# Gorilla-Lab-SCUT/DCL-Net

Measured on AMD Instinct MI355X. Metric: frames/sec DCL_Net.forward @ YCB-V bs32, higher is better.
Workload: dtype f32 (exact 3xbf16-split products on the bf16 MFMA, f32 accumulate)

## Files before the change

### dcl-net_amd/csrc/dense.hip

```cpp
#include "common.h"
#include <atomic>
#include <math.h>

namespace {

typedef float f32x16 __attribute__((ext_vector_type(16)));

constexpr int kKPitch = 68;
constexpr float kThr = 20.0f;

__device__ __forceinline__ int rowmap(int e, int h) { return (e & 3) + 8 * (e >> 2) + 4 * h; }

#ifdef DCL_DIAG
template <int NVT>
__global__ __launch_bounds__(256, 1) void k_cross_attn(
    int nq, int nk, const float *__restrict__ Q, int ldq, const float *__restrict__ K, int ldk,
    const float *__restrict__ V1, int dv1, int ldv1, float *__restrict__ O1, int ldo1,
    const float *__restrict__ V2, int dv2, int ldv2, float *__restrict__ O2, int ldo2) {
  constexpr int T = 256;
  constexpr int DV = NVT * 32;
  constexpr int KT = 32 * kKPitch;
  constexpr int TILE = KT + 32 * DV;
  constexpr int NVS = (32 * (DV / 4) + T - 1) / T;
  extern __shared__ float attn_lds[];
// ... 326 lines not shown
  auto load_k = [&](int kb) {
    int key, c4;
    k_slot(0, key, c4);
    knext0 = *reinterpret_cast<const float4 *>(K + (krow0 + min(kb + key, last_key)) * ldk + c4);
    if (KPT > 1) {
      k_slot(1, key, c4);
      knext1 = *reinterpret_cast<const float4 *>(K + (krow0 + min(kb + key, last_key)) * ldk + c4);
    }
  };
  auto store_k = [&]() {
    int key, c4;
    k_slot(0, key, c4);
    *reinterpret_cast<float4 *>(Ks + key * kKPitch + c4) = knext0;
    if (KPT > 1) {
      k_slot(1, key, c4);
      *reinterpret_cast<float4 *>(Ks + key * kKPitch + c4) = knext1;
    }
  };

  f32x16 O[NVT];
#pragma unroll
  for (int t = 0; t < NVT; ++t)
#pragma unroll
    for (int e = 0; e < 16; ++e) O[t][e] = 0.0f;
  float m_ref = -INFINITY, l_part = 0.0f;

  const int ntiles = (nk + 31) >> 5;
  const int kb_begin = (int)((long long)blockIdx.z * ntiles / gridDim.z) * 32;
  const int kb_end = min((int)((long long)(blockIdx.z + 1) * ntiles / gridDim.z) * 32, nk);
  load_k(kb_begin);
  store_k();
  dma_v(kb_begin, 0);
  int cur = 0;
  for (int kb = kb_begin; kb < kb_end; kb += 32) {
    const bool more = kb + 32 < kb_end;
    __builtin_amdgcn_s_waitcnt(0x0F70);
    __syncthreads();
    if (more) dma_v(kb + 32, cur ^ 1);

    f32x16 S;
#pragma unroll
    for (int e = 0; e < 16; ++e) S[e] = 0.0f;
    {
      const float *krow = Ks + r * kKPitch + 32 * h;
      const float *qrow = Qs + r * kKPitch + 32 * h;
#pragma unroll
      for (int i = 0; i < 8; ++i) {
        const float4 a = *reinterpret_cast<const float4 *>(krow + 4 * i);
        const float4 qv = *reinterpret_cast<const float4 *>(qrow + 4 * i);
        S = __builtin_amdgcn_mfma_f32_32x32x2f32(a.x, qv.x, S, 0, 0, 0);
        S = __builtin_amdgcn_mfma_f32_32x32x2f32(a.y, qv.y, S, 0, 0, 0);
        S = __builtin_amdgcn_mfma_f32_32x32x2f32(a.z, qv.z, S, 0, 0, 0);
        S = __builtin_amdgcn_mfma_f32_32x32x2f32(a.w, qv.w, S, 0, 0, 0);
      }
    }
    __builtin_amdgcn_s_waitcnt(0xC07F);
    __builtin_amdgcn_s_barrier();
    if (more) load_k(kb + 32);

    float m_tile = -INFINITY;
#pragma unroll
    for (int e = 0; e < 16; ++e) {
      if (kb + rowmap(e, h) >= nk) S[e] = -INFINITY;
      m_tile = fmaxf(m_tile, S[e]);
    }
    m_tile = fmaxf(m_tile, __shfl_xor(m_tile, 32, 64));
    if (__ballot(m_tile > m_ref + kThr) != 0ull) {
      const float m_new = fmaxf(m_ref, m_tile);
      const float f = __expf(m_ref - m_new);
      l_part *= f;
#pragma unroll
      for (int t = 0; t < NVT; ++t)
#pragma unroll
        for (int e = 0; e < 16; ++e) O[t][e] *= f;
      m_ref = m_new;
    }
#pragma unroll
    for (int e = 0; e < 16; ++e) {
      S[e] = __expf(S[e] - m_ref);
      l_part += S[e];
    }

    const float *v1b = V1s + cur * V1T + 4 * h * 256 + r;
    const float *v2b = V2s + cur * V2T + 4 * h * 64 + r;
#pragma unroll
    for (int t = 0; t < NVT; ++t) {
#pragma unroll
      for (int e = 0; e < 16; ++e) {
        const int krow = (e & 3) + 8 * (e >> 2);
        const float a = t < 8 ? v1b[krow * 256 + t * 32] : v2b[krow * 64 + (t - 8) * 32];
        O[t] = __builtin_amdgcn_mfma_f32_32x32x2f32(a, S[e], O[t], 0, 0, 0);
      }
    }
    if (more) store_k();
    cur ^= 1;
  }

  asm volatile("s_nop 15\n\ts_nop 7" ::: "memory");
  const float l_tot = l_part + __shfl_xor(l_part, 32, 64);
  if (qlive && gridDim.z > 1) {
    const size_t rows = (size_t)gridDim.y * nq;
    float *P = part + ((size_t)blockIdx.z * rows + (size_t)b * nq + q) * kAttnPartPitch;
#pragma unroll
    for (int t = 0; t < NVT; ++t)
#pragma unroll
      for (int g = 0; g < 4; ++g)
        *reinterpret_cast<float4 *>(P + t * 32 + 8 * g + 4 * h) =
            make_float4(O[t][4 * g], O[t][4 * g + 1], O[t][4 * g + 2], O[t][4 * g + 3]);
    if (h == 0) { P[320] = m_ref; P[321] = l_tot; }
  } else if (qlive) {
    const size_t row = (size_t)b * nq + q;
#pragma unroll
    for (int t = 0; t < NVT; ++t)
#pragma unroll
      for (int g = 0; g < 4; ++g) {
        const int c = t * 32 + 8 * g + 4 * h;
        float4 v;
        v.x = O[t][4 * g] / l_tot; v.y = O[t][4 * g + 1] / l_tot;
        v.z = O[t][4 * g + 2] / l_tot; v.w = O[t][4 * g + 3] / l_tot;
        if (c < 256) *reinterpret_cast<float4 *>(O1 + row * ldo1 + c) = v;
        else *reinterpret_cast<float4 *>(O2 + row * ldo2 + (c - 256)) = v;
      }
  }
}

typedef __bf16 at_bf16x2 __attribute__((ext_vector_type(2)));
typedef __bf16 at_bf16x8 __attribute__((ext_vector_type(8)));
typedef float at_f32x2 __attribute__((ext_vector_type(2)));
typedef unsigned at_u32x4 __attribute__((ext_vector_type(4)));
constexpr int kAttnHalfBytes = 3 * 320 * 2 * 16;
constexpr int kAttnKTileBytes = 3 * 32 * 128;
constexpr int kAttnTileBytes = 2 * kAttnHalfBytes + kAttnKTileBytes;

__device__ __forceinline__ unsigned at_cvt2(float a, float b) {
  const at_f32x2 v = {a, b};
  return __builtin_bit_cast(unsigned, __builtin_convertvector(v, at_bf16x2));
}
__device__ __forceinline__ void at_split2(float x0, float x1, unsigned &h, unsigned &m, unsigned &l) {
  h = at_cvt2(x0, x1);
  float r0 = x0 - __uint_as_float(h << 16);
  asm volatile("" : "+v"(r0));
  float r1 = x1 - __uint_as_float(h & 0xffff0000u);
  asm volatile("" : "+v"(r1));
  m = at_cvt2(r0, r1);
  float s0 = r0 - __uint_as_float(m << 16);
  asm volatile("" : "+v"(s0));
  float s1 = r1 - __uint_as_float(m & 0xffff0000u);
  asm volatile("" : "+v"(s1));
  l = at_cvt2(s0, s1);
}
__device__ __forceinline__ at_bf16x8 at_bf(at_u32x4 v) { return __builtin_bit_cast(at_bf16x8, v); }

__global__ __launch_bounds__(256) void k_attn_split_v(int nk, int nht, const float *__restrict__ V1, int ldv1, const float *__restrict__ V2,
                                                      int ldv2, unsigned *__restrict__ planes, long long total, int c_begin) {
  const int nc = 320 - c_begin;
  for (long long i = blockIdx.x * 256ll + threadIdx.x; i < total; i += (long long)gridDim.x * 256) {
    const int hs = (int)(i & 1);
    const long long q = i >> 1;
    const int c = c_begin + (int)(q % nc);
    const long long cht = q / nc;
    const int ht = (int)(cht % nht), crop = (int)(cht / nht);
    const int h = hs ^ ((c >> 3) & 1);
    const float *col = c < 256 ? V1 + c : V2 + (c - 256);
    const int ld = c < 256 ? ldv1 : ldv2;
    float v[8];
#pragma unroll
    for (int e = 0; e < 8; ++e) {
      const int key = 16 * ht + (e & 3) + 8 * (e >> 2) + 4 * h;
      v[e] = key < nk ? col[((size_t)crop * nk + key) * ld] : 0.0f;
    }
    unsigned ph[4], pm[4], pl[4];
#pragma unroll
    for (int e = 0; e < 4; ++e) at_split2(v[2 * e], v[2 * e + 1], ph[e], pm[e], pl[e]);
    unsigned *dst = planes + (size_t)cht * (kAttnHalfBytes / 4) + (size_t)(c * 2 + hs) * 4;
#pragma unroll
    for (int e = 0; e < 4; ++e) { dst[e] = ph[e]; dst[320 * 2 * 4 + e] = pm[e]; dst[2 * 320 * 2 * 4 + e] = pl[e]; }
  }
}

__global__ __launch_bounds__(256) void k_attn_split_k(int nk, int ntiles, const float *__restrict__ K, int ldk, unsigned *__restrict__ kplanes,
                                                      long long total) {
  for (long long i = blockIdx.x * 256ll + threadIdx.x; i < total; i += (long long)gridDim.x * 256) {
    const int ps = (int)(i & 7), key = (int)((i >> 3) & 31);
    const long long ct = i >> 8;
    const int tile = (int)(ct % ntiles), crop = (int)(ct / ntiles);
    const int p = ps ^ ((key >> 1) & 7), kk = tile * 32 + key;
    float4 a = make_float4(0.f, 0.f, 0.f, 0.f), b = a;
    if (kk < nk) {
      const float *row = K + ((size_t)crop * nk + kk) * ldk + 8 * p;
      a = *reinterpret_cast<const float4 *>(row);
      b = *reinterpret_cast<const float4 *>(row + 4);
    }
    unsigned ph[4], pm[4], pl[4];
    at_split2(a.x, a.y, ph[0], pm[0], pl[0]);
    at_split2(a.z, a.w, ph[1], pm[1], pl[1]);
    at_split2(b.x, b.y, ph[2], pm[2], pl[2]);
    at_split2(b.z, b.w, ph[3], pm[3], pl[3]);
    unsigned *dst = kplanes + (size_t)ct * (kAttnKTileBytes / 4) + (size_t)(key * 8 + ps) * 4;
#pragma unroll
    for (int e = 0; e < 4; ++e) { dst[e] = ph[e]; dst[32 * 32 + e] = pm[e]; dst[2 * 32 * 32 + e] = pl[e]; }
  }
}

__global__ __launch_bounds__(512, 2) void k_cross_attn_split(
    int nq, int nk, const float *__restrict__ Q, int ldq, const unsigned char *__restrict__ planes,
    const unsigned char *__restrict__ kplanes, float *__restrict__ O1, int ldo1, float *__restrict__ O2, int ldo2,
    float *__restrict__ part, int xcd_remap, int whatif) {
  constexpr int NVT = 10, WAVES = 8;
  constexpr int VT = 2 * kAttnHalfBytes;
  extern __shared__ float attn_lds[];
  unsigned char *Kp = reinterpret_cast<unsigned char *>(attn_lds);
  unsigned char *Vp = Kp + 2 * kAttnKTileBytes;
  int bx, b;
  {
    const int nwg = gridDim.x * gridDim.y, id = blockIdx.x + gridDim.x * blockIdx.y;
    const int xq = nwg >> 3, xr = nwg & 7, xcd = id & 7;
    const int swz = !xcd_remap ? id : (xcd < xr ? xcd * (xq + 1) : xr * (xq + 1) + (xcd - xr) * xq) + (id >> 3);
    bx = swz % (int)gridDim.x;
    b = swz / (int)gridDim.x;
  }
  const int tid = threadIdx.x;
  const int lane = tid & 63, wave = __builtin_amdgcn_readfirstlane(tid >> 6);
  const int grp = wave >> 2;
  const int r = lane & 31, h = lane >> 5;
  constexpr int QB = WAVES * 32;
  const int q = bx * QB + wave * 32 + r;
  const bool qlive = q < nq;
  const float *qrow = Q + ((size_t)b * nq + min(q, nq - 1)) * ldq + 8 * h;
  const int nht = 2 * ((nk + 31) >> 5);
  const unsigned char *vsrc = planes + (size_t)b * nht * kAttnHalfBytes;
  const unsigned char *ksrc = kplanes + (size_t)b * (nht >> 1) * kAttnKTileBytes;
  const unsigned lane16 = (unsigned)lane * 16u;
  const unsigned vp0 = lds_addr_of(reinterpret_cast<const float *>(Vp));
  const unsigned kp0 = lds_addr_of(reinterpret_cast<const float *>(Kp));
  auto dma_tile = [&](int tile, int buf) {
    const unsigned char *ks = ksrc + (size_t)tile * kAttnKTileBytes + wave * 1024;
    const unsigned kd = kp0 + (unsigned)(buf * kAttnKTileBytes + wave * 1024);
    glds16_s(lane16, ks, kd);
    if (wave < 4) glds16_s(lane16, ks + 8 * 1024, kd + 8 * 1024);
    const unsigned char *vs = vsrc + (size_t)tile * VT + wave * 1024;
    const unsigned vd = vp0 + (unsigned)(buf * VT + wave * 1024);
#pragma unroll
    for (int i = 0; i < 8; ++i)
      if (wave + 8 * i < 60) glds16_s(lane16, vs + i * 8192, vd + (unsigned)(i * 8192));
  };

  f32x16 O[NVT];
#pragma unroll
  for (int t = 0; t < NVT; ++t)
#pragma unroll
    for (int e = 0; e < 16; ++e) O[t][e] = 0.0f;
  float m_ref = -INFINITY, l_part = 0.0f;
  at_u32x4 pp[2][3];
#pragma unroll
  for (int hf = 0; hf < 2; ++hf)
#pragma unroll
    for (int p = 0; p < 3; ++p) pp[hf][p] = at_u32x4{0u, 0u, 0u, 0u};

  const int ntiles_all = (nk + 31) >> 5;
  const int t_begin = (int)((long long)blockIdx.z * ntiles_all / gridDim.z);
  const int t_end = (int)((long long)(blockIdx.z + 1) * ntiles_all / gridDim.z);
  const int T = t_end - t_begin;
  const unsigned char *vfrag = Vp + ((r * 2 + (h ^ ((r >> 3) & 1))) << 4);
  const unsigned char *kfrag = Kp + r * 128;
  const int ksw = (r >> 1) & 7;

  auto s_phase = [&](int tl) __attribute__((always_inline)) {
    const int buf = tl & 1, kb = (t_begin + tl) * 32;
    f32x16 S;
#pragma unroll
    for (int e = 0; e < 16; ++e) S[e] = 0.0f;
    const unsigned char *kfb = kfrag + buf * kAttnKTileBytes;
    float4 qn0 = *reinterpret_cast<const float4 *>(qrow), qn1 = *reinterpret_cast<const float4 *>(qrow + 4);
#pragma unroll
    for (int st = 0; st < 4; ++st) {
      const float4 qc0 = qn0, qc1 = qn1;
      if (st < 3) {
        qn0 = *reinterpret_cast<const float4 *>(qrow + 16 * (st + 1));
        qn1 = *reinterpret_cast<const float4 *>(qrow + 16 * (st + 1) + 4);
      }
      const unsigned char *kf = kfb + (((2 * st + h) ^ ksw) << 4);
      const at_u32x4 kh = *reinterpret_cast<const at_u32x4 *>(kf);
      const at_u32x4 km = *reinterpret_cast<const at_u32x4 *>(kf + 32 * 128);
      const at_u32x4 kl = *reinterpret_cast<const at_u32x4 *>(kf + 2 * 32 * 128);
      at_u32x4 qh, qm, ql;
      unsigned a0, a1, a2;
      at_split2(qc0.x, qc0.y, a0, a1, a2); qh[0] = a0; qm[0] = a1; ql[0] = a2;
      at_split2(qc0.z, qc0.w, a0, a1, a2); qh[1] = a0; qm[1] = a1; ql[1] = a2;
      at_split2(qc1.x, qc1.y, a0, a1, a2); qh[2] = a0; qm[2] = a1; ql[2] = a2;
      at_split2(qc1.z, qc1.w, a0, a1, a2); qh[3] = a0; qm[3] = a1; ql[3] = a2;
      S = __builtin_amdgcn_mfma_f32_32x32x16_bf16(at_bf(kl), at_bf(qh), S, 0, 0, 0);
      S = __builtin_amdgcn_mfma_f32_32x32x16_bf16(at_bf(kh), at_bf(ql), S, 0, 0, 0);
      S = __builtin_amdgcn_mfma_f32_32x32x16_bf16(at_bf(km), at_bf(qm), S, 0, 0, 0);
      S = __builtin_amdgcn_mfma_f32_32x32x16_bf16(at_bf(km), at_bf(qh), S, 0, 0, 0);
      S = __builtin_amdgcn_mfma_f32_32x32x16_bf16(at_bf(kh), at_bf(qm), S, 0, 0, 0);
      S = __builtin_amdgcn_mfma_f32_32x32x16_bf16(at_bf(kh), at_bf(qh), S, 0, 0, 0);
    }
    float m_tile = -INFINITY;
    if (kb + 32 > nk) {
#pragma unroll
      for (int e = 0; e < 16; ++e)
        if (kb + rowmap(e, h) >= nk) S[e] = -INFINITY;
    }
#pragma unroll
    for (int e = 0; e < 16; ++e) m_tile = fmaxf(m_tile, S[e]);
    m_tile = fmaxf(m_tile, __shfl_xor(m_tile, 32, 64));
    if (__ballot(m_tile > m_ref + kThr) != 0ull) {
      const float m_new = fmaxf(m_ref, m_tile);
      const float f = __expf(m_ref - m_new);
      l_part *= f;
#pragma unroll
      for (int t = 0; t < NVT; ++t)
#pragma unroll
        for (int e = 0; e < 16; ++e) O[t][e] *= f;
      m_ref = m_new;
    }
#pragma unroll
    for (int e = 0; e < 16; ++e) {
      S[e] = __expf(S[e] - m_ref);
      l_part += S[e];
    }
#pragma unroll
    for (int hf = 0; hf < 2; ++hf)
#pragma unroll
      for (int e = 0; e < 4; ++e) {
        unsigned ph, pm, pl;
        at_split2(S[8 * hf + 2 * e], S[8 * hf + 2 * e + 1], ph, pm, pl);
        pp[hf][0][e] = ph; pp[hf][1][e] = pm; pp[hf][2][e] = pl;
      }
  };
  auto pv_phase = [&](int tl) __attribute__((always_inline)) {
    const unsigned char *vbuf = vfrag + (tl & 1) * VT;
#pragma unroll
    for (int hf = 0; hf < 2; ++hf) {
      const unsigned char *vb = vbuf + hf * kAttnHalfBytes;
#pragma unroll
      for (int t = 0; t < NVT; ++t) {
        const at_u32x4 vh = *reinterpret_cast<const at_u32x4 *>(vb + t * 1024);
        const at_u32x4 vm = *reinterpret_cast<const at_u32x4 *>(vb + 320 * 32 + t * 1024);
        const at_u32x4 vl = *reinterpret_cast<const at_u32x4 *>(vb + 2 * 320 * 32 + t * 1024);
        O[t] = __builtin_amdgcn_mfma_f32_32x32x16_bf16(at_bf(vl), at_bf(pp[hf][0]), O[t], 0, 0, 0);
        O[t] = __builtin_amdgcn_mfma_f32_32x32x16_bf16(at_bf(vh), at_bf(pp[hf][2]), O[t], 0, 0, 0);
        O[t] = __builtin_amdgcn_mfma_f32_32x32x16_bf16(at_bf(vm), at_bf(pp[hf][1]), O[t], 0, 0, 0);
        O[t] = __builtin_amdgcn_mfma_f32_32x32x16_bf16(at_bf(vm), at_bf(pp[hf][0]), O[t], 0, 0, 0);
        O[t] = __builtin_amdgcn_mfma_f32_32x32x16_bf16(at_bf(vh), at_bf(pp[hf][1]), O[t], 0, 0, 0);
        O[t] = __builtin_amdgcn_mfma_f32_32x32x16_bf16(at_bf(vh), at_bf(pp[hf][0]), O[t], 0, 0, 0);
      }
    }
  };
  auto interval = [&](int iv) __attribute__((always_inline)) {
    __builtin_amdgcn_s_waitcnt(0x0F70);
    __syncthreads();
    if ((iv & 1) && (iv + 1) / 2 < T && !(whatif & 4)) dma_tile(t_begin + (iv + 1) / 2, ((iv + 1) / 2) & 1);
  };
  if (T > 0) dma_tile(t_begin, 0);
  if (grp == 0) {
    for (int tl = 0; tl < T; ++tl) {
      interval(2 * tl);
      if (!(whatif & 2)) s_phase(tl);
      interval(2 * tl + 1);
      if (!(whatif & 1)) pv_phase(tl);
    }
    interval(2 * T);
  } else {
    interval(0);
    for (int tl = 0; tl < T; ++tl) {
      interval(2 * tl + 1);
      if (!(whatif & 2)) s_phase(tl);
      interval(2 * tl + 2);
      if (!(whatif & 1)) pv_phase(tl);
    }
  }

  asm volatile("s_nop 15\n\ts_nop 7" ::: "memory");
  const float l_tot = l_part + __shfl_xor(l_part, 32, 64);
  if (qlive && gridDim.z > 1) {
    const size_t rows = (size_t)gridDim.y * nq;
    float *P = part + ((size_t)blockIdx.z * rows + (size_t)b * nq + q) * kAttnPartPitch;
#pragma unroll
    for (int t = 0; t < NVT; ++t)
#pragma unroll
      for (int g = 0; g < 4; ++g)
        *reinterpret_cast<float4 *>(P + t * 32 + 8 * g + 4 * h) =
            make_float4(O[t][4 * g], O[t][4 * g + 1], O[t][4 * g + 2], O[t][4 * g + 3]);
    if (h == 0) { P[320] = m_ref; P[321] = l_tot; }
  } else if (qlive) {
    const size_t row = (size_t)b * nq + q;
#pragma unroll
    for (int t = 0; t < NVT; ++t)
#pragma unroll
      for (int g = 0; g < 4; ++g) {
        const int c = t * 32 + 8 * g + 4 * h;
        float4 v;
        v.x = O[t][4 * g] / l_tot; v.y = O[t][4 * g + 1] / l_tot;
        v.z = O[t][4 * g + 2] / l_tot; v.w = O[t][4 * g + 3] / l_tot;
        if (c < 256) *reinterpret_cast<float4 *>(O1 + row * ldo1 + c) = v;
        else *reinterpret_cast<float4 *>(O2 + row * ldo2 + (c - 256)) = v;
      }
  }
}

__global__ void k_cross_attn_combine(int rows, int nsplit, const float *__restrict__ part, float *__restrict__ O1, int ldo1,
                                     float *__restrict__ O2, int ldo2) {
  const long long total = (long long)rows * 80;
  for (long long t = (long long)blockIdx.x * blockDim.x + threadIdx.x; t < total; t += (long long)gridDim.x * blockDim.x) {
    const size_t row = (size_t)(t / 80);
    const int c = (int)(t - (long long)row * 80) * 4;
    float m = -INFINITY;
    for (int z = 0; z < nsplit; ++z) m = fmaxf(m, part[((size_t)z * rows + row) * kAttnPartPitch + 320]);
    float4 num = make_float4(0.f, 0.f, 0.f, 0.f);
    float den = 0.0f;
    for (int z = 0; z < nsplit; ++z) {
      const float *P = part + ((size_t)z * rows + row) * kAttnPartPitch;
      const float f = __expf(P[320] - m);
      const float4 o = *reinterpret_cast<const float4 *>(P + c);
      num.x += f * o.x; num.y += f * o.y; num.z += f * o.z; num.w += f * o.w;
      den += f * P[321];
    }
    const float4 v = make_float4(num.x / den, num.y / den, num.z / den, num.w / den);
    if (c < 256) *reinterpret_cast<float4 *>(O1 + row * ldo1 + c) = v;
    else *reinterpret_cast<float4 *>(O2 + row * ldo2 + (c - 256)) = v;
  }
}

template <int NT>
__device__ __forceinline__ float conf_block_reduce(float v, float *red, int lane, int wave, bool is_max) {
  constexpr int NW = NT / 64;
#pragma unroll
  for (int d = 32; d >= 1; d >>= 1) v = is_max ? fmaxf(v, __shfl_xor(v, d, 64)) : v + __shfl_xor(v, d, 64);
  if (lane == 0) red[wave] = v;
  __syncthreads();
  float r;
  if (NW == 4) {
    r = is_max ? fmaxf(fmaxf(red[0], red[1]), fmaxf(red[2], red[3])) : (red[0] + red[1]) + (red[2] + red[3]);
  } else {
    float t[NW];
#pragma unroll
    for (int i = 0; i < NW; ++i) t[i] = red[i];
#pragma unroll
    for (int step = 1; step < NW; step <<= 1)
#pragma unroll
      for (int i = 0; i + step < NW; i += 2 * step) t[i] = is_max ? fmaxf(t[i], t[i + step]) : t[i] + t[i + step];
    r = t[0];
  }
  __syncthreads();
  return r;
}
template <int NT>
__global__ __launch_bounds__(NT) void k_conf_softmax(int n1, int n2, const float *__restrict__ logit1,
                                                     const float *__restrict__ logit2, float *__restrict__ conf,
                                                     float *__restrict__ w, float *__restrict__ wsum) {
  __shared__ float red[NT / 64];
  const int L = n1 + n2;
  const int b = blockIdx.x, tid = threadIdx.x;
  const int lane = tid & 63, wave = tid >> 6;
  float mx = -INFINITY;
  for (int j = tid; j < L; j += NT) {
    const float x = j < n1 ? logit1[(size_t)b * n1 + j] : logit2[(size_t)b * n2 + (j - n1)];
    const float s = 1.0f / (1.0f + expf(-x));
    conf[(size_t)b * L + j] = s;
    mx = fmaxf(mx, s);
  }
  mx = conf_block_reduce<NT>(mx, red, lane, wave, true);
  float sum = 0.0f;
  for (int j = tid; j < L; j += NT) {
    const float e = expf(conf[(size_t)b * L + j] - mx);
    w[(size_t)b * L + j] = e;
    sum += e;
  }
  sum = conf_block_reduce<NT>(sum, red, lane, wave, false);
  const float inv = 1.0f / sum;
  float w1 = 0.f, w2 = 0.f;
  for (int j = tid; j < L; j += NT) {
    const float v = w[(size_t)b * L + j] * inv;
    w[(size_t)b * L + j] = v;
    if (j < n1) w1 += v; else w2 += v;
  }
  w1 = conf_block_reduce<NT>(w1, red, lane, wave, false);
  w2 = conf_block_reduce<NT>(w2, red, lane, wave, false);
  if (tid == 0) { wsum[b * 2] = w1; wsum[b * 2 + 1] = w2; }
}

__global__ __launch_bounds__(256) void k_weighted_colsum(int c, int n1, int n2, int nslices, const float *__restrict__ w,
                                                         const float *__restrict__ F1, int ld1, float *__restrict__ part1,
                                                         const float *__restrict__ F2, int ld2, float *__restrict__ part2) {
  __shared__ float4 red[4][64];
  const int second = (int)blockIdx.y >= nslices ? 1 : 0;
  const int b = blockIdx.z, slice = blockIdx.y - second * nslices;
  const int n = second ? n2 : n1, ld = second ? ld2 : ld1, w_stride = n1 + n2, w_off = second ? n1 : 0;
  const float *__restrict__ F = second ? F2 : F1;
  float *__restrict__ part = second ? part2 : part1;
  const int lane = threadIdx.x & 63, wave = threadIdx.x >> 6;
  const int ch = blockIdx.x * 256 + lane * 4;
  const int per = (n + nslices - 1) / nslices;
  const int j0 = slice * per, j1 = min(n, j0 + per);
  float4 acc = make_float4(0.f, 0.f, 0.f, 0.f);
  if (ch < c) {
    const float *wp = w + (size_t)b * w_stride + w_off;
    const float *fp = F + (size_t)b * n * ld + ch;
    for (int j = j0 + wave; j < j1; j += 4) {
      const float wj = wp[j];
      const float4 f = *reinterpret_cast<const float4 *>(fp + (size_t)j * ld);
      acc.x = __fmaf_rn(f.x, wj, acc.x); acc.y = __fmaf_rn(f.y, wj, acc.y);
      acc.z = __fmaf_rn(f.z, wj, acc.z); acc.w = __fmaf_rn(f.w, wj, acc.w);
    }
  }
  red[wave][lane] = acc;
  __syncthreads();
  if (wave == 0 && ch < c) {
    float4 o;
    o.x = (red[0][lane].x + red[1][lane].x) + (red[2][lane].x + red[3][lane].x);
    o.y = (red[0][lane].y + red[1][lane].y) + (red[2][lane].y + red[3][lane].y);
    o.z = (red[0][lane].z + red[1][lane].z) + (red[2][lane].z + red[3][lane].z);
    o.w = (red[0][lane].w + red[1][lane].w) + (red[2][lane].w + red[3][lane].w);
    *reinterpret_cast<float4 *>(part + ((size_t)b * nslices + slice) * c + ch) = o;
  }
}

template <int EPT>
__global__ __launch_bounds__(256) void k_conf_pool_small(int c, int n1, int n2, int nslices, const float *__restrict__ logit1,
                                                         const float *__restrict__ logit2, float *__restrict__ conf,
                                                         float *__restrict__ wsum, const float *__restrict__ F1, int ld1,
                                                         float *__restrict__ part1, const float *__restrict__ F2, int ld2,
                                                         float *__restrict__ part2) {
  __shared__ float wl[256 * EPT];
  __shared__ float redf[4], r1[4], r2[4];
  __shared__ float4 red[4][64];
  const int L = n1 + n2;
  const int second = (int)blockIdx.y >= nslices ? 1 : 0;
  const int b = blockIdx.z, slice = blockIdx.y - second * nslices;
  const int tid = threadIdx.x, lane = tid & 63, wave = tid >> 6;
  const bool writer = blockIdx.x == 0 && blockIdx.y == 0;
  float sv[EPT];
  float mx = -INFINITY;
#pragma unroll
  for (int k = 0; k < EPT; ++k) {
    const int j = tid + 256 * k;
    if (j < L) {
      const float x = j < n1 ? logit1[(size_t)b * n1 + j] : logit2[(size_t)b * n2 + (j - n1)];
      sv[k] = 1.0f / (1.0f + expf(-x));
      if (writer) conf[(size_t)b * L + j] = sv[k];
      mx = fmaxf(mx, sv[k]);
    }
  }
#pragma unroll
  for (int d = 32; d >= 1; d >>= 1) mx = fmaxf(mx, __shfl_xor(mx, d, 64));
  if (lane == 0) redf[wave] = mx;
  __syncthreads();
  mx = fmaxf(fmaxf(redf[0], redf[1]), fmaxf(redf[2], redf[3]));
  __syncthreads();
  float sum = 0.0f;
#pragma unroll
// ... 61 lines not shown
    const float x = o9[i * 9 + c * 3], y = o9[i * 9 + c * 3 + 1], z = o9[i * 9 + c * 3 + 2];
    const float mag = sqrtf((x * x + y * y) + z * z) + 1e-8f;
    A[0][c] = (double)(x / mag); A[1][c] = (double)(y / mag); A[2][c] = (double)(z / mag);
#pragma unroll
    for (int r = 0; r < 3; ++r) V[r][c] = r == c ? 1.0 : 0.0;
  }
  for (int sweep = 0; sweep < 30; ++sweep) {
    double off = 0.0;
#pragma unroll
    for (int p = 0; p < 2; ++p)
#pragma unroll
      for (int q = p + 1; q < 3; ++q) {
        double alpha = 0, beta = 0, gamma = 0;
#pragma unroll
        for (int r = 0; r < 3; ++r) { alpha += A[r][p] * A[r][p]; beta += A[r][q] * A[r][q]; gamma += A[r][p] * A[r][q]; }
        off = fmax(off, fabs(gamma) / sqrt(alpha * beta + 1e-300));
        if (fabs(gamma) < 1e-300) continue;
        const double zeta = (beta - alpha) / (2.0 * gamma);
        const double t = (zeta >= 0 ? 1.0 : -1.0) / (fabs(zeta) + sqrt(1.0 + zeta * zeta));
        const double cs = 1.0 / sqrt(1.0 + t * t), sn = cs * t;
#pragma unroll
        for (int r = 0; r < 3; ++r) {
          const double ap = A[r][p], aq = A[r][q];
          A[r][p] = cs * ap - sn * aq; A[r][q] = sn * ap + cs * aq;
          const double vp = V[r][p], vq = V[r][q];
          V[r][p] = cs * vp - sn * vq; V[r][q] = sn * vp + cs * vq;
        }
      }
    if (off < 1e-15) break;
  }
  double a0[3] = {A[0][0], A[1][0], A[2][0]}, a1[3] = {A[0][1], A[1][1], A[2][1]}, a2[3] = {A[0][2], A[1][2], A[2][2]};
  double v0[3] = {V[0][0], V[1][0], V[2][0]}, v1[3] = {V[0][1], V[1][1], V[2][1]}, v2[3] = {V[0][2], V[1][2], V[2][2]};
  double s0 = sqrt(a0[0] * a0[0] + a0[1] * a0[1] + a0[2] * a0[2]);
  double s1 = sqrt(a1[0] * a1[0] + a1[1] * a1[1] + a1[2] * a1[2]);
  double s2 = sqrt(a2[0] * a2[0] + a2[1] * a2[1] + a2[2] * a2[2]);
#define DCL_SWAP_COLS(sa, sb, aa, ab, va, vb)                                  \
  if (sa < sb) {                                                               \
    double t_ = sa; sa = sb; sb = t_;                                          \
    for (int r_ = 0; r_ < 3; ++r_) {                                           \
      t_ = aa[r_]; aa[r_] = ab[r_]; ab[r_] = t_;                               \
      t_ = va[r_]; va[r_] = vb[r_]; vb[r_] = t_;                               \
    }                                                                          \
  }
  DCL_SWAP_COLS(s0, s1, a0, a1, v0, v1)
  DCL_SWAP_COLS(s1, s2, a1, a2, v1, v2)
  DCL_SWAP_COLS(s0, s1, a0, a1, v0, v1)
#undef DCL_SWAP_COLS
  double u1[3], u2[3], u3[3];
#pragma unroll
  for (int r = 0; r < 3; ++r) { u1[r] = a0[r] / s0; u2[r] = a1[r] / s1; }
  u3[0] = u1[1] * u2[2] - u1[2] * u2[1];
  u3[1] = u1[2] * u2[0] - u1[0] * u2[2];
  u3[2] = u1[0] * u2[1] - u1[1] * u2[0];
  const double detV = v0[0] * (v1[1] * v2[2] - v1[2] * v2[1]) - v0[1] * (v1[0] * v2[2] - v1[2] * v2[0]) +
                      v0[2] * (v1[0] * v2[1] - v1[1] * v2[0]);
#pragma unroll
  for (int r = 0; r < 3; ++r)
#pragma unroll
    for (int c = 0; c < 3; ++c)
      R[i * 9 + r * 3 + c] = (float)(u1[r] * v0[c] + u2[r] * v1[c] + detV * u3[r] * v2[c]);
}
__global__ void k_ortho9d(int b, const float *__restrict__ o9, float *__restrict__ R) {
  const int i = blockIdx.x * blockDim.x + threadIdx.x;
  if (i < b) ortho9d_one(o9, R, i);
}

}

DCL_HOOK_INT(g_attn_variant, 0);
DCL_HOOK_INT(g_attn_split, 0);
DCL_HOOK_INT(g_attn_xcd_remap, 1);
#ifdef DCL_DIAG
DCL_API void dcl_debug_attention_split(int n) { g_attn_split = n; }
DCL_API void dcl_debug_attention_xcd_remap(int on) { g_attn_xcd_remap = on; }
DCL_API void dcl_debug_attention_variant(int v) { g_attn_variant = v; }
#endif

DCL_API int dcl_cross_attention(int b, int nq, int nk, const float *Q, int ldq, const float *K, int ldk,
                                const float *V1, int dv1, int ldv1, float *O1, int ldo1, const float *V2, int dv2,
                                int ldv2, float *O2, int ldo2, dclStream_t stream) {
  return dcl_cross_attention_ws(b, nq, nk, Q, ldq, K, ldk, V1, dv1, ldv1, O1, ldo1, V2, dv2, ldv2, O2, ldo2, nullptr, 0,
                                stream);
}

DCL_HOOK_INT(g_attn_whatif, 0);
DCL_HOOK_INT(g_attn_bf16, 1);
static bool attn_split_big(long long blocks8, int nk) { return blocks8 >= 64 && blocks8 * dcl_div_up(nk, 32) >= 16384; }
DCL_HOOK_INT(g_attn_pair_split, 1);
static int attn_pair_full_crops(int b, int nq, int dv1, int dv2, int concurrent_launches, int nk = 0) {
  if (!g_attn_pair_split || g_attn_variant != 0 || concurrent_launches != 2 || dv1 != 256 || dv2 != 64 || nq <= 0) return 0;
  const int qb8 = dcl_div_up(nq, 256);
  if (nk > 0 && g_attn_bf16 && attn_split_big((long long)b * qb8, nk)) return 0;
  if (qb8 > 128 || 128 % qb8 != 0) return 0;
  const int per_round = 128 / qb8;
  const int full = b / per_round * per_round;
  return full > 0 && full < b ? full : 0;
}
#ifdef DCL_DIAG
DCL_API void dcl_debug_attention_pair_split(int on) { g_attn_pair_split = on; }
#endif

static int attn_small_split(int b, int nq, int ntiles) {
  const int forced = g_attn_split;
  if (forced > 0) return forced > 16 ? 16 : forced;
  const long long T = 2ll * b * dcl_div_up(nq, 128);
  const double tiles_us = 1.1 * ntiles;
  double best = 1e30;
  int nsplit = 1;
  for (int z = 1; z <= 16; z *= 2) {
    const double cost = (double)dcl_div_up(T * z, 256) * (tiles_us / z + 4.0) + (z > 1 ? 4.0 + 0.15 * z * (double)b * nq / 1024.0 : 0.0);
    if (cost < best - 1e-9) { best = cost; nsplit = z; }
  }
  if (nsplit > ntiles / 2) nsplit = ntiles / 2;
  return nsplit < 1 ? 1 : nsplit;
}

DCL_API int dcl_cross_attention_scratch_floats(int b, int nq, int64_t *floats_host) {
  DCL_CHECK_ARG(b >= 0 && nq >= 0 && floats_host);
  const long long per = (long long)b * nq * kAttnPartPitch;
  const long long blocks8 = (long long)b * dcl_div_up(nq > 0 ? nq : 1, 256);
  long long z = 1;
  if (blocks8 < 256) {
    for (int ntiles = 2; ntiles <= (1 << 16); ntiles *= 2) z = max(z, (long long)attn_small_split(b, nq, ntiles));
  } else {
    z = 1;
    double best = (double)dcl_div_up(blocks8, 256);
    for (int c = 2; c <= 8; c *= 2) {
      const double cost = (double)dcl_div_up(blocks8 * c, 256) / c;
      if (cost <= best - 0.2 && c * per <= (128ll << 20)) { best = cost; z = c; }
    }
  }
  long long need = z > 1 ? z * per : 0;
  const int full = attn_pair_full_crops(b, nq, 256, 64, 2);
  if (full) {
    int64_t rest = 0;
    const int rc = dcl_cross_attention_scratch_floats(b - full, nq, &rest);
    if (rc) return rc;
    if (rest > need) need = rest;
  }
  *floats_host = need;
  return 0;
}

DCL_API int dcl_cross_attention_ws(int b, int nq, int nk, const float *Q, int ldq, const float *K, int ldk,
                                   const float *V1, int dv1, int ldv1, float *O1, int ldo1, const float *V2, int dv2,
                                   int ldv2, float *O2, int ldo2, float *scratch, int64_t scratch_floats,
                                   dclStream_t stream) {
  return dcl_cross_attention_ws2(b, nq, nk, Q, ldq, K, ldk, V1, dv1, ldv1, O1, ldo1, V2, dv2, ldv2, O2, ldo2, scratch,
                                 scratch_floats, 1, stream);
}

static int attn_dispatch(int b, int nq, int nk, const float *Q, int ldq, const float *K, int ldk, const float *V1, int dv1, int ldv1,
                         float *O1, int ldo1, const float *V2, int dv2, int ldv2, float *O2, int ldo2, float *scratch,
                         int64_t scratch_floats, int concurrent_launches, void *planes, int64_t planes_bytes, dclStream_t stream);

static bool attn_takes_w8(int b, int nq, int nk, int concurrent_launches) {
  const long long blocks8 = (long long)b * dcl_div_up(nq, 256);
  const bool pair8 = concurrent_launches == 2 && 2 * blocks8 > 240 && 2 * blocks8 <= 256;
  return g_attn_variant == 3 || (g_attn_variant == 0 && (blocks8 >= 256 || pair8 || attn_split_big(blocks8, nk)));
}
#ifdef DCL_DIAG
DCL_API void dcl_debug_attention_bf16(int on) { g_attn_bf16 = on; }
DCL_API void dcl_debug_attention_whatif(int bits) { g_attn_whatif = bits; }
#endif

DCL_API int dcl_cross_attention_split_crops(int b, int nq, int nk, int concurrent_launches) {
  if (b <= 0 || nq <= 0 || nk <= 0 || !g_attn_bf16) return 0;
  int crops = b;
  const int full = attn_pair_full_crops(b, nq, 256, 64, concurrent_launches, nk);
  if (full) crops = full;
  return attn_takes_w8(crops, nq, nk, concurrent_launches) ? crops : 0;
}

DCL_API int64_t dcl_cross_attention_planes_bytes(int b, int nq, int nk, int concurrent_launches) {
  if (b <= 0 || nq <= 0 || nk <= 0 || !g_attn_bf16) return 0;
  int crops = b;
  const int full = attn_pair_full_crops(b, nq, 256, 64, concurrent_launches, nk);
  if (full) crops = full;
  if (!attn_takes_w8(crops, nq, nk, concurrent_launches)) return 0;
  return (int64_t)crops * dcl_div_up(nk, 32) * kAttnTileBytes;
}

DCL_API int dcl_cross_attention_ws2(int b, int nq, int nk, const float *Q, int ldq, const float *K, int ldk,
                                    const float *V1, int dv1, int ldv1, float *O1, int ldo1, const float *V2, int dv2,
                                    int ldv2, float *O2, int ldo2, float *scratch, int64_t scratch_floats,
                                    int concurrent_launches, dclStream_t stream) {
  return dcl_cross_attention_ws3(b, nq, nk, Q, ldq, K, ldk, V1, dv1, ldv1, O1, ldo1, V2, dv2, ldv2, O2, ldo2, scratch, scratch_floats,
                                 concurrent_launches, nullptr, 0, stream);
}

DCL_API int dcl_cross_attention_ws3(int b, int nq, int nk, const float *Q, int ldq, const float *K, int ldk,
                                    const float *V1, int dv1, int ldv1, float *O1, int ldo1, const float *V2, int dv2,
                                    int ldv2, float *O2, int ldo2, float *scratch, int64_t scratch_floats,
                                    int concurrent_launches, void *planes, int64_t planes_bytes, dclStream_t stream) {
  DCL_CHECK_ARG(concurrent_launches == 1 || concurrent_launches == 2);
  const int full = (b > 0 && Q && K && O1) ? attn_pair_full_crops(b, nq, dv1, dv2, concurrent_launches, planes ? nk : 0) : 0;
  DCL_CHECK_ARG(!(full && !V1));
  if (full) {
    int rc = attn_dispatch(full, nq, nk, Q, ldq, K, ldk, V1, dv1, ldv1, O1, ldo1, V2, dv2, ldv2, O2, ldo2, scratch, scratch_floats,
                           concurrent_launches, planes, planes_bytes, stream);
    if (rc) return rc;
    const size_t qo = (size_t)full * nq, ko = (size_t)full * nk;
    return attn_dispatch(b - full, nq, nk, Q + qo * ldq, ldq, K + ko * ldk, ldk, V1 + ko * ldv1, dv1, ldv1, O1 + qo * ldo1, ldo1,
                         V2 ? V2 + ko * ldv2 : nullptr, dv2, ldv2, O2 ? O2 + qo * ldo2 : nullptr, ldo2, scratch, scratch_floats,
                         concurrent_launches, nullptr, 0, stream);
  }
  return attn_dispatch(b, nq, nk, Q, ldq, K, ldk, V1, dv1, ldv1, O1, ldo1, V2, dv2, ldv2, O2, ldo2, scratch, scratch_floats,
                       concurrent_launches, planes, planes_bytes, stream);
}

static int attn_dispatch(int b, int nq, int nk, const float *Q, int ldq, const float *K, int ldk, const float *V1, int dv1, int ldv1,
                         float *O1, int ldo1, const float *V2, int dv2, int ldv2, float *O2, int ldo2, float *scratch,
                         int64_t scratch_floats, int concurrent_launches, void *planes, int64_t planes_bytes, dclStream_t stream) {
  DCL_CHECK_ARG(b >= 0 && nq >= 0 && nk > 0 && dv1 > 0 && dv1 % 32 == 0 && dv2 >= 0 && dv2 % 32 == 0);
  if (b == 0 || nq == 0) return 0;
  DCL_CHECK_ARG(Q && K && (V1 || planes) && O1 && (dv2 == 0 || (V2 && O2)) && b <= 65535);
  DCL_CHECK_ARG(ldq >= 64 && ldk >= 64 && ldv1 >= dv1 && ldo1 >= dv1 && (dv2 == 0 || (ldv2 >= dv2 && ldo2 >= dv2)));
  DCL_CHECK_ARG(ldq % 4 == 0 && ldk % 4 == 0 && ldv1 % 4 == 0 && ldo1 % 4 == 0 && ldv2 % 4 == 0 && ldo2 % 4 == 0);
  DCL_CHECK_ARG((((uintptr_t)Q | (uintptr_t)K | (uintptr_t)V1 | (uintptr_t)O1 | (uintptr_t)V2 | (uintptr_t)O2) & 15) == 0);
  const bool v1_in_planes = V1 == nullptr;
  const int nvt = (dv1 + dv2) / 32;
  DCL_CHECK_ARG(nvt == 1 || nvt == 2 || nvt == 4 || nvt == 8 || nvt == 10);
  hipStream_t s = (hipStream_t)stream;
  const long long blocks8 = (long long)b * dcl_div_up(nq, 256);
  if (dv1 == 256 && dv2 == 64 && (g_attn_variant == 0 || g_attn_variant == 3 || g_attn_variant == 4)) {
    const bool pair8 = concurrent_launches == 2 && 2 * blocks8 > 240 && 2 * blocks8 <= 256;
    const bool split_usable = planes && g_attn_bf16 && (((uintptr_t)planes) & 15) == 0 &&
                              planes_bytes >= (int64_t)b * dcl_div_up(nk, 32) * kAttnTileBytes;
    const bool w8 = g_attn_variant == 3 ||
                    (g_attn_variant == 0 && (blocks8 >= 256 || pair8 || (split_usable && attn_split_big(blocks8, nk))));
    const int W = w8 ? 8 : 4;
    const size_t lds = (size_t)(32 * kKPitch + 2 * 32 * 256 + 2 * 32 * 64 + W * 32 * kKPitch) * sizeof(float);
    if (w8) {
      int nsplit = 1;
      if (scratch && !(pair8 && g_attn_split == 0)) {
        if (g_attn_split > 0) {
          nsplit = g_attn_split;
        } else {
          double best = (double)dcl_div_up(blocks8, 256);
          for (int z = 2; z <= 8; z *= 2) {
            const double cost = (double)dcl_div_up(blocks8 * z, 256) / z;
            if (cost <= best - 0.2 && (long long)z * b * nq * kAttnPartPitch <= (128ll << 20)) { best = cost; nsplit = z; }
          }
        }
        const int ntiles = dcl_div_up(nk, 32);
        if (nsplit > 8) nsplit = 8;
        if (nsplit > ntiles / 2) nsplit = ntiles / 2;
        while (nsplit > 1 && (long long)nsplit * b * nq * kAttnPartPitch > scratch_floats) --nsplit;
        if (nsplit < 1) nsplit = 1;
      }
      const int nht = 2 * dcl_div_up(nk, 32);
      const int64_t planes_need = (int64_t)b * (nht / 2) * kAttnTileBytes;
      if (planes && planes_bytes >= planes_need && g_attn_bf16 && (((uintptr_t)planes) & 15) == 0) {
        const int c_begin = V1 ? 0 : 256;
        const long long total = (long long)b * nht * (320 - c_begin) * 2;
        hipLaunchKernelGGL(k_attn_split_v, dim3(dcl_grid_1d(total, 256)), dim3(256), 0, s, nk, nht, V1, ldv1, V2, ldv2,
                           (unsigned *)planes, total, c_begin);
        unsigned char *kplanes = (unsigned char *)planes + (size_t)b * nht * kAttnHalfBytes;
        const long long ktotal = (long long)b * (nht / 2) * 32 * 8;
        hipLaunchKernelGGL(k_attn_split_k, dim3(dcl_grid_1d(ktotal, 256)), dim3(256), 0, s, nk, nht / 2, K, ldk, (unsigned *)kplanes, ktotal);
        const size_t lds_sp = (size_t)2 * (2 * kAttnHalfBytes + kAttnKTileBytes);
        (void)hipFuncSetAttribute((const void *)k_cross_attn_split, hipFuncAttributeMaxDynamicSharedMemorySize, (int)lds_sp);
        hipLaunchKernelGGL(k_cross_attn_split, dim3(dcl_div_up(nq, 256), b, nsplit), dim3(512), lds_sp, s, nq, nk, Q, ldq,
                           (const unsigned char *)planes, (const unsigned char *)kplanes, O1, ldo1, O2, ldo2, scratch,
                           (int)g_attn_xcd_remap, (int)g_attn_whatif);
      } else {
        if (v1_in_planes) {
          dcl_set_error("dcl_cross_attention: V1 = NULL (pieces in `planes`) but this call does not take the split-bf16 kernel");
          return DCL_EINVAL;
        }
        (void)hipFuncSetAttribute((const void *)k_cross_attn_dma<8>, hipFuncAttributeMaxDynamicSharedMemorySize, (int)lds);
        hipLaunchKernelGGL(k_cross_attn_dma<8>, dim3(dcl_div_up(nq, 256), b, nsplit), dim3(512), lds, s, nq, nk, Q, ldq, K, ldk,
                           V1, ldv1, O1, ldo1, V2, ldv2, O2, ldo2, scratch, (int)g_attn_xcd_remap);
      }
      if (nsplit > 1)
        hipLaunchKernelGGL(k_cross_attn_combine, dim3(dcl_grid_1d((long long)b * nq * 80, 256)), dim3(256), 0, s, b * nq,
                           nsplit, scratch, O1, ldo1, O2, ldo2);
    } else {
      if (v1_in_planes) {
        dcl_set_error("dcl_cross_attention: V1 = NULL (pieces in `planes`) but this call does not take the split-bf16 kernel");
        return DCL_EINVAL;
      }
      int nsplit = 1;
      if (scratch) {
        nsplit = attn_small_split(b, nq, dcl_div_up(nk, 32));
        const int ntiles = dcl_div_up(nk, 32);
        if (nsplit > 16) nsplit = 16;
        if (nsplit > ntiles / 2) nsplit = ntiles / 2;
        while (nsplit > 1 && (long long)nsplit * b * nq * kAttnPartPitch > scratch_floats) --nsplit;
        if (nsplit < 1) nsplit = 1;
      }
      (void)hipFuncSetAttribute((const void *)k_cross_attn_dma<4>, hipFuncAttributeMaxDynamicSharedMemorySize, (int)lds);
      hipLaunchKernelGGL(k_cross_attn_dma<4>, dim3(dcl_div_up(nq, 128), b, nsplit), dim3(256), lds, s, nq, nk, Q, ldq, K,
                         ldk, V1, ldv1, O1, ldo1, V2, ldv2, O2, ldo2, scratch, (int)g_attn_xcd_remap);
      if (nsplit > 1)
        hipLaunchKernelGGL(k_cross_attn_combine, dim3(dcl_grid_1d((long long)b * nq * 80, 256)), dim3(256), 0, s, b * nq,
                           nsplit, scratch, O1, ldo1, O2, ldo2);
    }
  }
#ifdef DCL_DIAG
  else if ((blocks8 >= 256 && g_attn_variant != 2) || g_attn_variant == 1) {
    const size_t lds = (size_t)(32 * kKPitch + 32 * nvt * 32 + 8 * 32 * kKPitch) * sizeof(float);
#define ATT8(N)                                                                                                \
  do {                                                                                                         \
    (void)hipFuncSetAttribute((const void *)k_cross_attn_shared<8, N>, hipFuncAttributeMaxDynamicSharedMemorySize, \
                              (int)lds);                                                                       \
    hipLaunchKernelGGL((k_cross_attn_shared<8, N>), dim3(dcl_div_up(nq, 256), b), dim3(512), lds, s, nq, nk, Q, \
                       ldq, K, ldk, V1, dv1, ldv1, O1, ldo1, V2, dv2, ldv2, O2, ldo2);                         \
  } while (0)
    switch (nvt) {
      case 1: ATT8(1); break;
      case 2: ATT8(2); break;
      case 4: ATT8(4); break;
      case 8: ATT8(8); break;
      default: ATT8(10); break;
    }
#undef ATT8
  } else {
    const size_t lds = (size_t)2 * (32 * kKPitch + 32 * nvt * 32) * sizeof(float);
#define ATT(N)                                                                                                 \
  do {                                                                                                         \
    (void)hipFuncSetAttribute((const void *)k_cross_attn<N>, hipFuncAttributeMaxDynamicSharedMemorySize,       \
                              (int)lds);                                                                       \
    hipLaunchKernelGGL((k_cross_attn<N>), dim3(dcl_div_up(nq, 128), b), dim3(256), lds, s, nq, nk, Q, ldq, K,   \
                       ldk, V1, dv1, ldv1, O1, ldo1, V2, dv2, ldv2, O2, ldo2);                                 \
  } while (0)
    switch (nvt) {
      case 1: ATT(1); break;
      case 2: ATT(2); break;
      case 4: ATT(4); break;
      case 8: ATT(8); break;
      default: ATT(10); break;
    }
#undef ATT
  }
#else
  else {
    dcl_set_error("dcl_cross_attention: only dv1 = 256, dv2 = 64 is built into the product library (got %d, %d)", dv1, dv2);
    return DCL_EINVAL;
  }
#endif
  DCL_LAUNCH_CHECK();
  return 0;
}

DCL_API int dcl_conf_pool(int b, int c, int n1, int n2, const float *logit1, const float *logit2, const float *F1,
                          int ld1, const float *F2, int ld2, float *conf, float *w_scratch, int nslices,
                          float *part1, float *part2, float *wsum, dclStream_t stream) {
  DCL_CHECK_ARG(b >= 0 && c > 0 && c % 4 == 0 && n1 > 0 && n2 > 0 && ld1 >= c && ld2 >= c && ld1 % 4 == 0 &&
                ld2 % 4 == 0 && nslices >= 1);
  if (b == 0) return 0;
  DCL_CHECK_ARG(conf && w_scratch && part1 && part2 && wsum && logit1 && F1 && logit2 && F2 && b <= 65535 &&
                nslices <= 32767);
  hipStream_t s = (hipStream_t)stream;
  if (b <= 8 && n1 + n2 <= 256 * 8) {
    hipLaunchKernelGGL(k_conf_pool_small<8>, dim3(dcl_div_up(c, 256), 2 * nslices, b), dim3(256), 0, s, c, n1, n2, nslices, logit1,
                       logit2, conf, wsum, F1, ld1, part1, F2, ld2, part2);
    DCL_LAUNCH_CHECK();
    return 0;
  }
  hipLaunchKernelGGL(k_conf_softmax<256>, dim3(b), dim3(256), 0, s, n1, n2, logit1, logit2, conf, w_scratch, wsum);
  hipLaunchKernelGGL(k_weighted_colsum, dim3(dcl_div_up(c, 256), 2 * nslices, b), dim3(256), 0, s, c, n1, n2, nslices,
                     w_scratch, F1, ld1, part1, F2, ld2, part2);
  DCL_LAUNCH_CHECK();
  return 0;
}

__global__ void k_pool_finish(int c, int nslices1, int nslices2, const float *__restrict__ part1, const float *__restrict__ part2,
                              const float *__restrict__ wsum, const float *__restrict__ sA, const float *__restrict__ tA,
                              const float *__restrict__ sB, const float *__restrict__ tB, float *__restrict__ out) {
  const int b = blockIdx.y, ch = blockIdx.x * blockDim.x + threadIdx.x;
  if (ch >= c) return;
  float a1[4] = {0.f, 0.f, 0.f, 0.f}, a2[4] = {0.f, 0.f, 0.f, 0.f};
  const float *q1 = part1 + (size_t)b * nslices1 * c + ch, *q2 = part2 + (size_t)b * nslices2 * c + ch;
  int s = 0;
  for (; s + 4 <= nslices1; s += 4) {
#pragma unroll
    for (int j = 0; j < 4; ++j) a1[j] += q1[(size_t)(s + j) * c];
  }
  for (int j = 0; s < nslices1; ++s, ++j) a1[j] += q1[(size_t)s * c];
  for (s = 0; s + 4 <= nslices2; s += 4) {
#pragma unroll
    for (int j = 0; j < 4; ++j) a2[j] += q2[(size_t)(s + j) * c];
  }
  for (int j = 0; s < nslices2; ++s, ++j) a2[j] += q2[(size_t)s * c];
  const float p1 = (a1[0] + a1[1]) + (a1[2] + a1[3]), p2 = (a2[0] + a2[1]) + (a2[2] + a2[3]);
  const float w0 = wsum[2 * b], w1 = wsum[2 * b + 1];
  out[(size_t)b * c + ch] = ((sA[ch] * p1 + tA[ch] * w0) + sB[ch] * p2) + tB[ch] * w1;
}

DCL_API int dcl_pool_finish2(int b, int c, int nslices1, int nslices2, const float *part1, const float *part2, const float *wsum,
                             const float *scale1, const float *shift1, const float *scale2, const float *shift2,
                             float *out, dclStream_t stream) {
  DCL_CHECK_ARG(b >= 0 && c > 0 && nslices1 >= 1 && nslices2 >= 1);
  if (b == 0) return 0;
  DCL_CHECK_ARG(part1 && part2 && wsum && scale1 && shift1 && scale2 && shift2 && out && b <= 65535);
  hipLaunchKernelGGL(k_pool_finish, dim3(dcl_div_up(c, 256), b), dim3(256), 0, (hipStream_t)stream, c, nslices1, nslices2, part1,
                     part2, wsum, scale1, shift1, scale2, shift2, out);
  DCL_LAUNCH_CHECK();
  return 0;
}
DCL_API int dcl_pool_finish(int b, int c, int nslices, const float *part1, const float *part2, const float *wsum,
                            const float *scale1, const float *shift1, const float *scale2, const float *shift2,
                            float *out, dclStream_t stream) {
  return dcl_pool_finish2(b, c, nslices, nslices, part1, part2, wsum, scale1, shift1, scale2, shift2, out, stream);
}

DCL_API int dcl_conf_softmax(int b, int n1, int n2, const float *logit1, const float *logit2, float *conf, float *w, float *wsum,
                             dclStream_t stream) {
  DCL_CHECK_ARG(b >= 0 && n1 > 0 && n2 > 0);
  if (b == 0) return 0;
  DCL_CHECK_ARG(logit1 && logit2 && conf && w && wsum && b <= 65535);
  if (n1 + n2 > 4096) hipLaunchKernelGGL(k_conf_softmax<1024>, dim3(b), dim3(1024), 0, (hipStream_t)stream, n1, n2, logit1, logit2, conf, w, wsum);
  else hipLaunchKernelGGL(k_conf_softmax<256>, dim3(b), dim3(256), 0, (hipStream_t)stream, n1, n2, logit1, logit2, conf, w, wsum);
  DCL_LAUNCH_CHECK();
  return 0;
}

__global__ __launch_bounds__(256) void k_affine3_relu(long long rows, int c4, const float *__restrict__ xyz, const float *__restrict__ W,
                                                      const float4 *__restrict__ term, float4 *__restrict__ out) {
  const long long total = rows * c4;
  for (long long t = (long long)blockIdx.x * blockDim.x + threadIdx.x; t < total; t += (long long)gridDim.x * blockDim.x) {
    const long long row = t / c4;
    const int q = (int)(t - row * c4);
    const float x = xyz[row * 3], y = xyz[row * 3 + 1], z = xyz[row * 3 + 2];
    const float4 wx = reinterpret_cast<const float4 *>(W)[q], wy = reinterpret_cast<const float4 *>(W)[c4 + q],
                 wz = reinterpret_cast<const float4 *>(W)[2 * c4 + q];
    const float4 a = term[t];
    float4 o;
    o.x = fmaxf(__fmaf_rn(z, wz.x, __fmaf_rn(y, wy.x, x * wx.x)) + a.x, 0.f);
    o.y = fmaxf(__fmaf_rn(z, wz.y, __fmaf_rn(y, wy.y, x * wx.y)) + a.y, 0.f);
    o.z = fmaxf(__fmaf_rn(z, wz.z, __fmaf_rn(y, wy.z, x * wx.z)) + a.z, 0.f);
// ... 281 lines not shown
```

### dcl-net_amd/csrc/linear_split.hip

```cpp
#include <hip/hip_runtime.h>
#include "common.h"

namespace {

typedef float sp_f32x16 __attribute__((ext_vector_type(16)));
typedef float sp_f32x2 __attribute__((ext_vector_type(2)));
typedef __bf16 sp_bf16x2 __attribute__((ext_vector_type(2)));
typedef __bf16 sp_bf16x8 __attribute__((ext_vector_type(8)));
typedef unsigned sp_u32x4 __attribute__((ext_vector_type(4)));
typedef __attribute__((address_space(3))) void sp_lds_void_t;

constexpr int kSpKC = 16;
constexpr int kSpBM = 256, kSpBN = 128;
constexpr int kSpA = kSpBM * kSpKC * 4;
constexpr int kSpP = kSpBN * kSpKC * 2;
constexpr int kSpB = 3 * kSpP;
constexpr int kSpST = kSpA + kSpB;

__device__ __forceinline__ unsigned sp_lds_addr(const void *p) {
  return __builtin_amdgcn_readfirstlane((unsigned)(size_t)(sp_lds_void_t *)p);
}
__device__ __forceinline__ void sp_glds16(unsigned voff, const void *sbase, unsigned lds_byte_addr) {
  unsigned keep;
  asm volatile("s_mov_b32 %0, m0\n\ts_mov_b32 m0, %3\n\ts_nop 0\n\tglobal_load_lds_dwordx4 %1, %2\n\ts_mov_b32 m0, %0"
// ... 153 lines not shown
      __builtin_amdgcn_sched_barrier(0);
      if (!(whatif & 2)) {
#pragma unroll
        for (int part = 0; part < 4; ++part) split_a(0, part);
      } else {
#pragma unroll
        for (int p = 0; p < 3; ++p) ap[0][p] = sp_u32x4{__float_as_uint(av[0][0].x), __float_as_uint(av[0][0].y), __float_as_uint(av[0][1].x), __float_as_uint(av[0][1].y)};
      }
      read_b(1);
      __builtin_amdgcn_sched_barrier(0);
#pragma unroll
      for (int blk = 0; blk < 8; ++blk) {
        const int i = blk >> 2, j = blk & 3;
        acc[i][j] = __builtin_amdgcn_mfma_f32_32x32x16_bf16(sp_bf(ap[i][2]), sp_bf(bp[j][0]), acc[i][j], 0, 0, 0);
        acc[i][j] = __builtin_amdgcn_mfma_f32_32x32x16_bf16(sp_bf(ap[i][0]), sp_bf(bp[j][2]), acc[i][j], 0, 0, 0);
        acc[i][j] = __builtin_amdgcn_mfma_f32_32x32x16_bf16(sp_bf(ap[i][1]), sp_bf(bp[j][1]), acc[i][j], 0, 0, 0);
        acc[i][j] = __builtin_amdgcn_mfma_f32_32x32x16_bf16(sp_bf(ap[i][1]), sp_bf(bp[j][0]), acc[i][j], 0, 0, 0);
        acc[i][j] = __builtin_amdgcn_mfma_f32_32x32x16_bf16(sp_bf(ap[i][0]), sp_bf(bp[j][1]), acc[i][j], 0, 0, 0);
        acc[i][j] = __builtin_amdgcn_mfma_f32_32x32x16_bf16(sp_bf(ap[i][0]), sp_bf(bp[j][0]), acc[i][j], 0, 0, 0);
        if (blk < 4) {
          if (!(whatif & 2)) split_a(1, blk);
          else { ap[1][0][blk] = __float_as_uint(av[1][blk >> 1].x); ap[1][1][blk] = __float_as_uint(av[1][blk >> 1].y); ap[1][2][blk] = __float_as_uint(av[1][blk >> 1].z); }
        }
        if (blk < 2) read_b(blk + 2);
        __builtin_amdgcn_sched_barrier(0);
      }
      asm volatile("s_waitcnt vmcnt(0)" ::: "memory");
    }
    asm volatile("s_nop 15\n\ts_nop 7" ::: "memory");

    if constexpr (EPI == 0) {
      if (whatif & 4) continue;
      float *__restrict__ y = a.y;
      const bool whole = row0 + kSpBM <= a.M && col0 + kSpBN <= a.N;
      float bias[4];
#pragma unroll
      for (int j = 0; j < 4; ++j) {
        const int co = col0 + j * 32 + r;
        bias[j] = (a.bias && co < a.N) ? a.bias[co] : 0.0f;
      }
      if (whole) {
#pragma unroll
        for (int i = 0; i < 2; ++i)
#pragma unroll
          for (int j = 0; j < 4; ++j) {
            float *yp = y + (size_t)(row0 + wave * 64 + i * 32 + 4 * h) * a.ldy + (col0 + j * 32 + r);
#pragma unroll
            for (int e = 0; e < 16; ++e) {
              float v = acc[i][j][e] + bias[j];
              if (a.relu) v = fmaxf(v, 0.0f);
              __builtin_nontemporal_store(v, yp + (size_t)((e & 3) + 8 * (e >> 2)) * a.ldy);
            }
          }
      } else {
#pragma unroll
        for (int i = 0; i < 2; ++i)
#pragma unroll
          for (int j = 0; j < 4; ++j) {
            const int co = col0 + j * 32 + r;
#pragma unroll
            for (int e = 0; e < 16; ++e) {
              const int orow = row0 + wave * 64 + i * 32 + sp_rowmap(e, h);
              float v = acc[i][j][e] + bias[j];
              if (a.relu) v = fmaxf(v, 0.0f);
              if (orow < a.M && co < a.N) y[(size_t)orow * a.ldy + co] = v;
            }
          }
      }
    } else if constexpr (EPI == 3) {
      unsigned char *vp = reinterpret_cast<unsigned char *>(a.part);
      const int crop = row0 / a.rows_per_crop, key0 = row0 - crop * a.rows_per_crop;
#pragma unroll
      for (int j = 0; j < 4; ++j) {
        const int c = col0 + j * 32 + r;
        const float bias = (a.bias && c < a.N) ? a.bias[c] : 0.0f;
        const int hs = h ^ ((c >> 3) & 1);
#pragma unroll
        for (int i = 0; i < 2; ++i)
#pragma unroll
          for (int hf = 0; hf < 2; ++hf) {
            const long long ht = (long long)crop * a.ldp + ((key0 + wave * 64 + i * 32) >> 4) + hf;
            sp_u32x4 ph, pm, pl;
#pragma unroll
            for (int e = 0; e < 4; ++e) {
              float v0 = acc[i][j][8 * hf + 2 * e] + bias, v1 = acc[i][j][8 * hf + 2 * e + 1] + bias;
              if (a.relu) { v0 = fmaxf(v0, 0.0f); v1 = fmaxf(v1, 0.0f); }
              unsigned qh, qm, ql;
              sp_split2(v0, v1, qh, qm, ql);
              ph[e] = qh; pm[e] = qm; pl[e] = ql;
            }
            unsigned char *dst = vp + (size_t)ht * (3 * 320 * 32) + (size_t)(c * 2 + hs) * 16;
            if (c < a.N) {
              *reinterpret_cast<sp_u32x4 *>(dst) = ph;
              *reinterpret_cast<sp_u32x4 *>(dst + 320 * 32) = pm;
              *reinterpret_cast<sp_u32x4 *>(dst + 2 * 320 * 32) = pl;
            }
          }
      }
    } else if constexpr (EPI == 2) {
      float w3c[4], bias[4];
#pragma unroll
      for (int j = 0; j < 4; ++j) {
        const int co = col0 + j * 32 + r;
        bias[j] = (a.bias && co < a.N) ? a.bias[co] : 0.0f;
        w3c[j] = co < a.N ? a.roww[(size_t)co * a.w_stride] : 0.0f;
      }
      const float b3 = a.b3[0];
#pragma unroll
      for (int i = 0; i < 2; ++i)
#pragma unroll
        for (int e = 0; e < 16; ++e) {
          float sdot = 0.0f;
#pragma unroll
          for (int j = 0; j < 4; ++j) sdot = __fmaf_rn(fmaxf(acc[i][j][e] + bias[j], 0.0f), w3c[j], sdot);
#pragma unroll
          for (int d = 16; d >= 1; d >>= 1) sdot += __shfl_xor(sdot, d, 64);
          const int orow = row0 + wave * 64 + i * 32 + sp_rowmap(e, h);
          if (r == 0 && orow < a.M) a.part[orow] = sdot + b3;
        }
    } else {
      const float *wl = reinterpret_cast<const float *>(sp_lds + 2 * kSpST) + wave * 64 + 4 * h;
      float *red = reinterpret_cast<float *>(sp_lds + 2 * kSpST) + kSpBM;
#pragma unroll
      for (int j = 0; j < 4; ++j) {
        const int cl = j * 32 + r, co = col0 + cl;
        const float bias = (a.bias && co < a.N) ? a.bias[co] : 0.0f;
        float s = 0.0f;
#pragma unroll
        for (int i = 0; i < 2; ++i)
#pragma unroll
          for (int g4 = 0; g4 < 4; ++g4) {
            const float4 w4 = *reinterpret_cast<const float4 *>(wl + i * 32 + 8 * g4);
            const float wv[4] = {w4.x, w4.y, w4.z, w4.w};
#pragma unroll
            for (int q = 0; q < 4; ++q) {
              float v = acc[i][j][4 * g4 + q] + bias;
              if (a.relu) v = fmaxf(v, 0.0f);
              s = __fmaf_rn(v, wv[q], s);
            }
          }
        s += __shfl_xor(s, 32, 64);
        if (h == 0) red[wave * kSpBN + cl] = s;
      }
      dcl_lds_barrier();
      {
        const int pt = tid >> 7, cl = tid & 127;
        if (col0 + cl < a.N && row0 + pt * 128 < a.M)
          a.part[(size_t)(2 * tm + pt) * a.ldp + col0 + cl] = red[(2 * pt) * kSpBN + cl] + red[(2 * pt + 1) * kSpBN + cl];
      }
    }
  }
}

DCL_HOOK_INT(g_sp_xcd, 1);

template <int EPI>
int launch_linear_split(const LinSplitArgs &a, hipStream_t stream) {
  const long long tiles = (long long)((a.M + kSpBM - 1) / kSpBM) * ((a.N + kSpBN - 1) / kSpBN);
  if (tiles > 0x7fffffffll) {
    dcl_set_error("dcl_linear_split_fwd: too many tiles");
    return DCL_EINVAL;
  }
  constexpr size_t lds = (size_t)2 * kSpST + (EPI == 1 ? (kSpBM + 4 * kSpBN) * sizeof(float) : 0);
  static bool attr_set = false;
  if (!attr_set) {
    (void)hipFuncSetAttribute((const void *)k_linear_split<EPI>, hipFuncAttributeMaxDynamicSharedMemorySize, (int)lds);
    attr_set = true;
  }
  hipLaunchKernelGGL((k_linear_split<EPI>), dim3((unsigned)tiles), dim3(256), lds, stream, a);
  return 0;
}

bool lin_split_ok(const float *x, int64_t ldx, const void *planes, int K) {
  return K >= kSpKC && K % kSpKC == 0 && ldx % 4 == 0 && ((size_t)x & 15) == 0 && ((size_t)planes & 15) == 0;
}

}

#ifdef DCL_DIAG
DCL_API void dcl_debug_linear_split_xcd_remap(int on) { g_sp_xcd = ((int)g_sp_xcd & ~1) | (on & 1); }
DCL_API void dcl_debug_linear_split_whatif(int bits) { g_sp_xcd = ((int)g_sp_xcd & 1) | (bits << 1); }
#endif

DCL_API int64_t dcl_linear_split_weight_bytes(int K, int N) {
  if (K <= 0 || N <= 0 || K % kSpKC) return 0;
  return (int64_t)(K / kSpKC) * ((N + kSpBN - 1) / kSpBN) * kSpB;
}

DCL_API int dcl_linear_split_weight(const float *Wt, int64_t ldw, int K, int N, void *planes, dclStream_t stream) {
  DCL_CHECK_ARG(Wt && planes && K > 0 && N > 0 && K % kSpKC == 0 && ldw >= N && ((size_t)planes & 15) == 0);
  const long long pieces = (long long)(K / kSpKC) * ((N + kSpBN - 1) / kSpBN) * kSpBN * 2;
  const unsigned grid = (unsigned)((pieces + 255) / 256 > 4096 ? 4096 : (pieces + 255) / 256);
  hipLaunchKernelGGL(k_split_weight, dim3(grid), dim3(256), 0, (hipStream_t)stream, Wt, (long long)ldw, K, N, (unsigned *)planes);
  DCL_LAUNCH_CHECK();
  return 0;
}

DCL_API int dcl_linear_split_fwd(const float *x, int64_t ldx, const void *planes, const float *bias, float *y, int64_t ldy, int M, int N,
                                 int K, int relu, dclStream_t stream) {
  DCL_CHECK_ARG(M >= 0 && N > 0 && K > 0 && x && planes && y && ldx >= K && ldy >= N);
  DCL_CHECK_ARG(lin_split_ok(x, ldx, planes, K));
  if (M == 0) return 0;
  LinSplitArgs a{x, (const unsigned char *)planes, bias, y, ldx, ldy, M, N, K, relu, nullptr, 1, 0, nullptr, nullptr, 0, (int)g_sp_xcd};
  int rc = launch_linear_split<0>(a, (hipStream_t)stream);
  if (rc) return rc;
  DCL_LAUNCH_CHECK();
  return 0;
}

DCL_API int dcl_linear_split_pool_fwd(const float *x, int64_t ldx, const void *planes, const float *bias, const float *roww,
                                      int rows_per_crop, int64_t w_stride, float *part, int64_t ldp, int M, int N, int K, int relu,
                                      dclStream_t stream) {
  DCL_CHECK_ARG(M > 0 && N > 0 && K > 0 && x && planes && roww && part && ldx >= K && ldp >= N && rows_per_crop >= 1 && w_stride >= 0);
  DCL_CHECK_ARG(lin_split_ok(x, ldx, planes, K));
  LinSplitArgs a{x, (const unsigned char *)planes, bias, nullptr, ldx, 0, M, N, K, relu, roww, rows_per_crop, w_stride, part, nullptr, ldp,
                 (int)g_sp_xcd};
  int rc = launch_linear_split<1>(a, (hipStream_t)stream);
  if (rc) return rc;
  DCL_LAUNCH_CHECK();
  return 0;
}

DCL_API int dcl_linear_split_vpieces_fwd(const float *x, int64_t ldx, const void *planes, const float *bias, void *vplanes,
                                         int rows_per_crop, int M, int N, int K, int relu, dclStream_t stream) {
  DCL_CHECK_ARG(M > 0 && N > 0 && N <= 320 && N % 32 == 0 && K > 0 && x && planes && vplanes && ldx >= K && rows_per_crop > 0);
  DCL_CHECK_ARG(rows_per_crop % kSpBM == 0 && M % rows_per_crop == 0 && (((size_t)vplanes) & 15) == 0);
  DCL_CHECK_ARG(lin_split_ok(x, ldx, planes, K));
  LinSplitArgs a{x, (const unsigned char *)planes, bias, nullptr, ldx, 0, M, N, K, relu, nullptr, rows_per_crop, 0, (float *)vplanes, nullptr,
                 (long long)(rows_per_crop / 16), (int)g_sp_xcd};
  int rc = launch_linear_split<3>(a, (hipStream_t)stream);
  if (rc) return rc;
  DCL_LAUNCH_CHECK();
  return 0;
}

DCL_API int dcl_linear_split_rowdot_fwd(const float *x, int64_t ldx, const void *planes, const float *bias, const float *w3, int64_t ldw3,
                                        const float *b3, float *out, int M, int N, int K, dclStream_t stream) {
  DCL_CHECK_ARG(M >= 0 && N > 0 && N <= kSpBN && K > 0 && x && planes && w3 && b3 && out && ldx >= K && ldw3 >= 1);
  DCL_CHECK_ARG(lin_split_ok(x, ldx, planes, K));
  if (M == 0) return 0;
  LinSplitArgs a{x, (const unsigned char *)planes, bias, nullptr, ldx, 0, M, N, K, 1, w3, 1, ldw3, out, b3, 0, (int)g_sp_xcd};
  int rc = launch_linear_split<2>(a, (hipStream_t)stream);
  if (rc) return rc;
  DCL_LAUNCH_CHECK();
  return 0;
}
```

### dcl-net_amd/models/DCL_Net.py

```python
from functools import partial

import numpy as np
import torch
import torch.nn as nn

from .. import ops
from .. import spconv
from ..libs.pointgroup_ops.functions import pointgroup_ops
from .losses import losses
from .Modules import (Aligner, Backbone_SPCONV, BasicBlock_3DCONV, Head_MultiLayerPerceptron,
                      Ops_GetPointFeat_spconv)

HOST_TIMES = None
_QUEUE_SHIMS = []
SIDE_STREAM_PRIORITY = -1
_SIDE_STREAMS = {}
SCALE_LISTS = [2, 4, 6, 8]
VOXEL_NUM_LIMIT = [64, 64, 64]


def normalize_vector(v):
    return v / (torch.sqrt(v.pow(2).sum(1, keepdim=True)) + 1e-8)


# ... 6 lines not shown
    ones = torch.ones(m.shape[0], dtype=m.dtype)
    sigma = torch.diag_embed(torch.stack([ones, ones, torch.det(U @ Vh)], dim=1))
    return (U @ sigma @ Vh).to(dev)


def _mlp3(dims):
    return Head_MultiLayerPerceptron(dims, ["relu", "relu", "none"], [False] * 3, [0.0] * 3)


def _fuser():
    return Head_MultiLayerPerceptron([512, 512, 512, 1024], ["relu"] * 3, [True] * 3, [0.0] * 3)


class Network(nn.Module):
    def __init__(self, cfg, mode="train", fused=True, graph_max_batch=8, async_inputs=False, graph_max_points=98304,
                 single_stream=False, pipeline_chunks=1, capture_graph=True, pair_features=None):
        super().__init__()
        self.single_stream = bool(single_stream)
        self._pair_features = pair_features
        self.pipeline_chunks = int(pipeline_chunks)
        self.capture_graph = bool(capture_graph)
        self.graph_max_batch = int(graph_max_batch)
        self.graph_max_points = int(graph_max_points)
        self.async_inputs = bool(async_inputs)
        self.voxelization_mode = cfg.voxelization_mode
        self.unit_voxel_extent = np.array(cfg.unit_voxel_extent)
        self.mode = mode
        self.fused = fused
        self.n_inp = cfg.n_inp
        self.n_tmp = cfg.n_tmp
        self.backbone_dims = [7, 16, 32, 32, 64, 64, 128, 128, 256]
        self.backbone_stride_layers = [1, 3, 5]
        self.backbone_inp = Backbone_SPCONV(self.backbone_dims, self.backbone_stride_layers, cfg.backbone)
        self.backbone_tmp = Backbone_SPCONV(self.backbone_dims, self.backbone_stride_layers, cfg.backbone)
        self.stage1_get_point_feats = Ops_GetPointFeat_spconv(SCALE_LISTS, self.unit_voxel_extent, VOXEL_NUM_LIMIT)
        block = partial(BasicBlock_3DCONV, size=1, bias=False, stride=1, padding=0, norm=True, act="relu", drop=0.0)
        for grp in ("1", "2"):
            for side in ("Xc", "Yo"):
                for kind, d_out in (("p", 256), ("m", 64)):
                    setattr(self, "disengage_%s_%s%s" % (side, kind, grp),
                            nn.Sequential(block(dim_in=480, dim_out=256), block(dim_in=256, dim_out=d_out)))
        self.neck_cross_att = Aligner()
        self.regressor_Xo = _mlp3([256, 256, 128, 3])
        self.regressor_Yc = _mlp3([256, 256, 128, 3])
        self.regressor_conf = _mlp3([128, 128, 128, 1])
        self.regressor_conf_bi = _mlp3([128, 128, 128, 1])
        self.neck_fuser = _fuser()
        self.neck_fuser_bi = _fuser()
        self.regressor_rot = _mlp3([1024, 512, 128, 9])
        self.regressor_trans = _mlp3([1024, 512, 128, 3])
        self._folded = None

    @property
    def pair_features(self):
        return self.single_stream if self._pair_features is None else bool(self._pair_features)

    @staticmethod
    def _drop_graph(ent):
        if ent is not None:
            if ent.get("graph") is not None and torch.cuda.is_available():
                torch.cuda.synchronize()
            ent["body"] = None
            ent.clear()

    def _invalidate(self):
        self._folded = None
        for ent in (self.__dict__.pop("_graphs", None) or {}).values():
            self._drop_graph(ent)
        self.__dict__.pop("_graph_seen", None)
        self.__dict__.pop("_vlist", None)

    def train(self, mode=True):
        self._invalidate()
        return super().train(mode)

    def _apply(self, fn, *a, **k):
        self._invalidate()
        return super()._apply(fn, *a, **k)

    def load_state_dict(self, *a, **k):
        self._invalidate()
        return super().load_state_dict(*a, **k)

    def __getstate__(self):
        state = dict(self.__dict__)
        for k in ("_side", "_graphs", "_graph_seen", "_crop_id_cache", "_vlist", "_counts_host"):
            state.pop(k, None)
        state["_folded"] = None
        return state

    @staticmethod
    def _bn_affine(bn):
        s = bn.weight / torch.sqrt(bn.running_var + bn.eps)
        return s, bn.bias - bn.running_mean * s

    def _fold(self):
        from .refiner import _param_version
        ver = _param_version(self)
        if self._folded is not None and self.__dict__.get("_fold_version") != ver:
            self._invalidate()
        if self._folded is not None:
            return self._folded
        self.__dict__["_fold_version"] = ver
        f = {}
        with torch.no_grad():
            for bb in ("backbone_inp", "backbone_tmp"):
                layers = []
                for m in range(1, 5):
                    for blk in getattr(getattr(self, bb), "module%d" % m):
                        conv, bn = blk.layers[0], blk.layers[1]
                        s, t = self._bn_affine(bn)
                        W = conv.weight.reshape(-1, conv.in_channels, conv.out_channels).contiguous()
                        layers.append((W, s.contiguous(), t.contiguous(), conv.subm))
                f[bb] = layers
                f[bb + "_ptrs"] = (ops._ptr_array([l[0] for l in layers]), ops._ptr_array([l[1] for l in layers]),
                                   ops._ptr_array([l[2] for l in layers]))
            for side in ("Xc", "Yo"):
                W1, t1, second = [], [], []
                for tag in ("p1", "m1", "p2", "m2"):
                    seq = getattr(self, "disengage_%s_%s" % (side, tag))
                    c0, b0 = seq[0].layers[0], seq[0].layers[1]
                    s, t = self._bn_affine(b0)
                    W1.append(c0.weight.reshape(c0.out_channels, c0.in_channels) * s[:, None])
                    t1.append(t)
                    c1, b1 = seq[1].layers[0], seq[1].layers[1]
                    s, t = self._bn_affine(b1)
                    second.append(((c1.weight.reshape(c1.out_channels, c1.in_channels) * s[:, None]).t().contiguous(),
                                   t.contiguous()))
                f["dis_" + side] = (torch.cat(W1, 0).t().contiguous(), torch.cat(t1, 0).contiguous(), second)
            for name in ("regressor_conf", "regressor_conf_bi", "regressor_rot", "regressor_trans", "regressor_Xo",
                         "regressor_Yc"):
                L = getattr(self, name).layers
                dense = name in ("regressor_rot", "regressor_trans")
                pad = (lambda w: w.contiguous()) if dense else ops.pad_linear_weight
                f[name] = [(pad(L[i].weight[:, :, 0].t()), L[i].bias.contiguous()) for i in (0, 2, 4)]
                if dense:
                    f[name + "_padded"] = [(ops.pad_linear_weight(Wt), bv) for Wt, bv in f[name]]
            for name in ("neck_fuser", "neck_fuser_bi"):
                L = getattr(self, name).layers
                out, s_prev, t_prev = [], None, None
                for ci, bi in ((0, 2), (3, 5), (6, 8)):
                    W, bvec = L[ci].weight[:, :, 0], L[ci].bias
                    if s_prev is not None:
                        bvec = bvec + W @ t_prev
                        W = W * s_prev[None, :]
                    out.append((W.t().contiguous(), bvec.contiguous()))
                    s_prev, t_prev = self._bn_affine(L[bi])
                f[name] = (out, s_prev.contiguous(), t_prev.contiguous())
            for side in ("Xc", "Yo"):
                W1t, _, second = f["dis_" + side]
                ops.prepare_linear(W1t)
                for Wt, _ in second:
                    ops.prepare_linear(Wt)
            for name in ("regressor_conf", "regressor_conf_bi", "regressor_Xo", "regressor_Yc"):
                for Wt, _ in f[name][:2]:
                    ops.prepare_linear(Wt)
            for name in ("neck_fuser", "neck_fuser_bi"):
                for Wt, _ in f[name][0]:
                    ops.prepare_linear(Wt)
        self._folded = f
        return f

    @staticmethod
    def _lin_relu(x, Wt, bias):
        return ops.linear(x, Wt, bias, True)

    def _mlp(self, x, layers):
        x = self._lin_relu(x, *layers[0])
        x = self._lin_relu(x, *layers[1])
        return ops.linear(x, layers[2][0], layers[2][1], False)

    def _side_stream(self, dev, which=0):
        if self.single_stream:
            return torch.cuda.current_stream(dev)
        key = (dev.index if dev.index is not None else torch.cuda.current_device(), which)
        if key not in _SIDE_STREAMS:
            _SIDE_STREAMS[key] = torch.cuda.Stream(dev, priority=SIDE_STREAM_PRIORITY)
        return _SIDE_STREAMS[key]

    def _pipeline_chunks(self, b):
        k = self.pipeline_chunks
        while k > 1 and (b % k != 0 or b // k < 4):
            k -= 1
        return max(k, 1)

    def _forward_fused(self, data):
        import time as _t
        mark = (lambda lbl: HOST_TIMES.append((lbl, _t.perf_counter()))) if HOST_TIMES is not None else (lambda lbl: None)
        mark("start")
        f = self._fold()
        dev = self.regressor_rot.layers[0].weight.device
        if dev.type != "cuda":
            raise RuntimeError("dcl-net_amd.Network runs on the GPU only: call .cuda() first (no CPU fallback)")
        b = int(data["batch_offsets"].size(0)) - 1
        S = int(np.asarray(data["voxel_num_limit"]).astype(np.int64)[0])
        main = torch.cuda.current_stream(dev)
        sstream = {"inp": self._side_stream(dev, 0), "tmp": self._side_stream(dev, 1)}
        single = sstream["inp"] is main
        K = self._pipeline_chunks(b)
        bc = b // K
        on_device = all(data[s][k].is_cuda for s in ("inp", "tmp") for k in ("feats", "v2p_maps", "occupied_voxels"))
        decoupled = self.async_inputs and on_device and not single
        for st in sstream.values():
            if not decoupled:
                st.wait_stream(main)
            elif data.get("ready_event") is not None:
                st.wait_event(data["ready_event"])
        npts = {"inp": self.n_inp, "tmp": self.n_tmp}
        side_in, runs, geo, vox, pb4, pf, pts = {}, {}, {}, {}, {}, {}, {}
        occ = {}
        counts_host = self._counts_pinned(K)
        def geometry(s):
            with torch.cuda.stream(sstream[s]):
                occ[s] = data[s]["occupied_voxels"].to(dev, non_blocking=True).int().contiguous()
                for c in range(K):
                    runs[s, c] = ops.BackboneRun(occ[s], bc, S, batch_lo=c * bc, counts_dev=counts_host[s][8 * c:8 * c + 8])
                geo[s] = torch.cuda.Event()
                geo[s].record(sstream[s])
        def stage(s):
            with torch.cuda.stream(sstream[s]):
                d = data[s]
                side_in[s] = (d["feats"].to(dev, non_blocking=True).float().contiguous(),
                              d["v2p_maps"].to(dev, non_blocking=True).int().contiguous(), occ[s])
                pb4[s] = torch.cat([self._crop_ids(dev, b, bc, npts[s]), side_in[s][0][:, 4:7]], 1)
                vox[s] = ops.voxelize_fp(side_in[s][0], side_in[s][1], self.voxelization_mode)
                pf[s] = torch.empty((b * npts[s], 480), dtype=torch.float32, device=dev)
            if not single:
                pf[s].record_stream(main)
                side_in[s][0].record_stream(main)
            pts[s] = side_in[s][0][:, 4:7].reshape(b, npts[s], 3)
        mark("geometry issued")
        unit = self.unit_voxel_extent
        assert unit[0] == unit[1] == unit[2], "anisotropic voxels: use fused=False"
        off = float(np.float32(-0.5 * unit[0] * VOXEL_NUM_LIMIT[0]))
        extents = [float(np.float32(unit[0] * sc)) for sc in SCALE_LISTS]
        done = {}
        if self.pair_features and K == 1:
            staged = {}
            for side in ("inp", "tmp"):
                geometry(side)
                stage(side)
                staged[side] = torch.cuda.Event()
                staged[side].record(sstream[side])
            for side in ("inp", "tmp"):
                geo[side].synchronize()
                runs[side, 0].set_counts(counts_host[side].tolist()[:8])
            mark("counts read back")
            s_inp, s_tmp = sstream["inp"], sstream["tmp"]
            with torch.cuda.stream(s_inp):
                if not single:
                    s_inp.wait_event(staged["tmp"])
                    for t in (vox["tmp"], runs["tmp", 0].ws):
                        t.record_stream(s_inp)
                ops.backbone_features_pair(runs["inp", 0], vox["inp"], f["backbone_inp_ptrs"],
                                           runs["tmp", 0], vox["tmp"], f["backbone_tmp_ptrs"])
                feat_done = torch.cuda.Event()
                feat_done.record(s_inp)
                if not single:
                    for t in runs["tmp", 0].levels:
                        t.record_stream(s_tmp)
                runs["inp", 0].point_features(pb4["inp"], extents, off, out=pf["inp"])
                done["inp", 0] = torch.cuda.Event()
                done["inp", 0].record(s_inp)
            with torch.cuda.stream(s_tmp):
                if not single:
                    s_tmp.wait_event(feat_done)
                runs["tmp", 0].point_features(pb4["tmp"], extents, off, out=pf["tmp"])
                done["tmp", 0] = torch.cuda.Event()
                done["tmp", 0].record(s_tmp)
        paired = bool(done)
        both_first = (self.HEAD_ORDER == 1 if self.HEAD_ORDER is not None else b * max(self.n_inp, self.n_tmp) <= 65536) and not paired
        if both_first:
            for side in ("inp", "tmp"):
                geometry(side)
                stage(side)
        for side, bb in (() if paired else (("inp", "backbone_inp"), ("tmp", "backbone_tmp"))):
            n = npts[side]
            if not both_first:
                geometry(side)
                stage(side)
            geo[side].synchronize()
            counts = counts_host[side].tolist()
            mark("counts read back " + side)
            for c in range(K):
                runs[side, c].set_counts(counts[8 * c:8 * c + 8])
            with torch.cuda.stream(sstream[side]):
                for c in range(K):
                    rows = slice(c * bc * n, (c + 1) * bc * n)
                    runs[side, c].features(vox[side], *f[bb + "_ptrs"])
                    runs[side, c].point_features(pb4[side][rows], extents, off, out=pf[side][rows])
                    done[side, c] = torch.cuda.Event()
                    done[side, c].record(sstream[side])
        act = {}
        tail_par = (not self.single_stream and not self.async_inputs and self._tail_parallel(b, launch_by_launch=True))
        for side, key in (("Xc", "inp"), ("Yo", "tmp")):
            act.update(self._disengage_buffers(side, b * npts[key], dev, fuse=(b, 2 if tail_par else 1) if K == 1 else None))
        mark("sparse issued")
        for c in range(K):
            for side, key in (("Xc", "inp"), ("Yo", "tmp")):
                main.wait_event(done[key, c])
                rows = slice(c * bc * npts[key], (c + 1) * bc * npts[key])
                self._disengage(f, side, pf[key][rows], act, rows)
        for st in sstream.values():
            main.wait_stream(st)
        tail_side = sstream["inp"] if tail_par else None
        prediction = self._dense_tail(f, act, b, dev, side=tail_side)
        mark("dense issued")
        if self.mode != "test":
            prediction["sym_flag"] = data["flags"].to(dev)
        data["labels"]["points_tmp"] = pts["tmp"]
        data["labels"]["points_inp"] = pts["inp"]
        return prediction

    def _counts_pinned(self, K):
        cache = self.__dict__.setdefault("_counts_host", {})
        if K not in cache:
            cache[K] = {s: torch.zeros(8 * K, dtype=torch.int32).pin_memory() for s in ("inp", "tmp")}
        assert all(t.is_pinned() for t in cache[K].values()), "level-size buffers must be pinned host memory"
        return cache[K]

    def _crop_ids(self, dev, b, bc, n):
        cache = self.__dict__.setdefault("_crop_id_cache", {})
        key = (str(dev), b, bc, n)
        if key not in cache:
            if len(cache) > 16:
                cache.clear()
            cache[key] = (torch.arange(b, device=dev) % bc).float().repeat_interleave(n).unsqueeze(1)
            torch.cuda.current_stream(dev).synchronize()
        return cache[key]

    _DIS_TAGS = (("p1", 256), ("m1", 64), ("p2", 256), ("m2", 64))
    POSE_HEADS_MAX = 128
    CONF_MLP_ROWS = 16384
    POSE_PARTS_MAX = 8
    PAR_TAIL = None
    GROUP_ROWS = 2 * 1024
    HEAD_ORDER = None
    GRAPH_TRIES = 5
    MAX_GRAPHS = 8
    GRAPH_ADMIT = 3

    def _disengage_buffers(self, side, rows, dev, fuse=None):
        new = lambda c: torch.empty((rows, c), dtype=torch.float32, device=dev)
        fuse_buf, conf_in = new(512), new(128)
        planes, fused = None, False
        if fuse is not None and self.mode == "test":
            b, par = fuse
            nk = self.n_inp if side == "Xc" else self.n_tmp
            nq = self.n_tmp if side == "Xc" else self.n_inp
            if rows == b * nk and nk % 256 == 0:
                planes, whole = ops.attention_planes(b, nq, nk, par, dev)
                fused = planes is not None and whole
        v1 = None if fused else new(256)
        if side == "Xc":
            return {"fuse1": fuse_buf, "conf_in1": conf_in, "Xcp1": fuse_buf[:, :256], "Xcm1": conf_in[:, :64],
                    "Xcp2": v1, "Xcm2": new(64), "planes2": planes}
        return {"fuse2": fuse_buf, "conf_in2": conf_in, "Yop2": fuse_buf[:, 256:], "Yom2": conf_in[:, 64:],
                "Yop1": v1, "Yom1": new(64), "planes1": planes}

    def _disengage(self, f, side, pf_rows, act, rows=slice(None)):
        W1t, t1, second = f["dis_" + side]
        H = self._lin_relu(pf_rows, W1t, t1)
        if pf_rows.shape[0] <= self.GROUP_ROWS:
            ops.linear_group([(H[:, 256 * j:256 * (j + 1)], second[j][0], second[j][1], True, act[side + tag][rows])
                              for j, (tag, _) in enumerate(self._DIS_TAGS)])
            return
        for j, (tag, _) in enumerate(self._DIS_TAGS):
            Wt, bias = second[j]
            Hj = H[:, 256 * j:256 * (j + 1)]
            if act[side + tag] is None:
                sw = ops.prepared_linear(Wt, Hj)
                planes = act["planes2" if side == "Xc" else "planes1"]
                all_rows = act[side + ("m2" if side == "Xc" else "m1")].shape[0]
                if sw is not None and pf_rows.shape[0] == all_rows:
                    ops.linear_split_vpieces(Hj, sw, bias, planes, self.n_inp if side == "Xc" else self.n_tmp, relu=True)
                    continue
                act[side + tag] = torch.empty((all_rows, 256), dtype=torch.float32, device=H.device)
            ops.linear(Hj, Wt, bias, True, out=act[side + tag][rows])

    def _dense(self, f, pf_inp, pf_tmp, b, dev):
        act = {}
        for side, pfs in (("Xc", pf_inp), ("Yo", pf_tmp)):
            act.update(self._disengage_buffers(side, pfs.shape[0], dev, fuse=(b, 1)))
            self._disengage(f, side, pfs, act)
        return self._dense_tail(f, act, b, dev)

    def _dense_tail(self, f, act, b, dev, side=None):
        main = torch.cuda.current_stream(dev)

        class _Both(object):
            def __enter__(self_inner):
                if side is not None:
                    side.wait_stream(main)
                    self_inner.ctx = torch.cuda.stream(side)
                    self_inner.ctx.__enter__()

            def __exit__(self_inner, *a):
                if side is not None:
                    self_inner.ctx.__exit__(*a)
        second = _Both()
        par = 2 if side is not None else 1

        def join():
            if side is not None:
                main.wait_stream(side)
        fuse1, conf_in1, fuse2, conf_in2 = act["fuse1"], act["conf_in1"], act["fuse2"], act["conf_in2"]
        (l1, sA, tA), (l2, sB, tB) = f["neck_fuser"], f["neck_fuser_bi"]
        def conf_and_fuser(conf_in, fuse, conf_layers, fuser_layers):
            F = fuse
            for Wt, bias in fuser_layers:
                F = self._lin_relu(F, Wt, bias)
            return conf_logits(conf_in, conf_layers), F
        def conf_logits(conf_in, conf_layers):
            if conf_in.shape[0] <= self.CONF_MLP_ROWS:
                return ops.mlp128_to1(conf_in, conf_layers)
            (W1t, b1), (W2t, b2), (W3t, b3) = conf_layers
            return ops.linear_rowdot(self._lin_relu(conf_in, W1t, b1), W2t, b2, W3t, b3)
        fused_pool = (b > self.POSE_PARTS_MAX and self.n_inp % ops.LINEAR_POOL_TILE == 0 and
                      self.n_tmp % ops.LINEAR_POOL_TILE == 0)
        if fused_pool:
            with second:
                ops.cross_attention(b, act["Yom2"], act["Xcm2"], act["Xcp2"], fuse2[:, :256], act["Xcm2"], conf_in2[:, :64], concurrent=par,
                                    planes=act.get("planes2"))
                logit2 = conf_logits(conf_in2, f["regressor_conf_bi"])
                if side is not None:
                    logit2.record_stream(main)
            ops.cross_attention(b, act["Xcm1"], act["Yom1"], act["Yop1"], fuse1[:, 256:], act["Yom1"], conf_in1[:, 64:], concurrent=par,
                                planes=act.get("planes1"))
            logit1 = conf_logits(conf_in1, f["regressor_conf"])
            join()
            conf, w, wsum = ops.conf_softmax(b, logit1.reshape(-1), logit2.reshape(-1))
            L = self.n_inp + self.n_tmp
            with second:
                if side is not None:
                    w.record_stream(side)
                H = self._lin_relu(self._lin_relu(fuse2, *l2[0]), *l2[1])
                part2 = ops.linear_pool(H, l2[2][0], l2[2][1], w.view(-1)[self.n_inp:], relu=True, rows_per_crop=self.n_tmp, w_stride=L)
                if side is not None:
                    part2.record_stream(main)
            H = self._lin_relu(self._lin_relu(fuse1, *l1[0]), *l1[1])
            part1 = ops.linear_pool(H, l1[2][0], l1[2][1], w.view(-1), relu=True, rows_per_crop=self.n_inp, w_stride=L)
            join()
            F_p_wei = ops.pool_finish2(part1, part2, wsum, (sA, tA, sB, tB))
        else:
            with second:
                ops.cross_attention(b, act["Yom2"], act["Xcm2"], act["Xcp2"], fuse2[:, :256], act["Xcm2"], conf_in2[:, :64], concurrent=par,
                                    planes=act.get("planes2"))
                logit2, Fp2 = conf_and_fuser(conf_in2, fuse2, f["regressor_conf_bi"], l2)
                if side is not None:
                    logit2.record_stream(main); Fp2.record_stream(main)
            ops.cross_attention(b, act["Xcm1"], act["Yom1"], act["Yop1"], fuse1[:, 256:], act["Yom1"], conf_in1[:, 64:], concurrent=par,
                                planes=act.get("planes1"))
            logit1, Fp1 = conf_and_fuser(conf_in1, fuse1, f["regressor_conf"], l1)
            join()
            if b <= self.POSE_PARTS_MAX:
                conf, parts = ops.conf_pool(b, logit1.reshape(-1), logit2.reshape(-1), Fp1, Fp2, affine=(sA, tA, sB, tB), finish=False)
                o9, trans_pred, rot_pred = ops.pose_heads_parts(parts, (sA, tA, sB, tB), f["regressor_rot"], f["regressor_trans"],
                                                                with_rotation=True)
                F_p_wei = None
            else:
                conf, F_p_wei = ops.conf_pool(b, logit1.reshape(-1), logit2.reshape(-1), Fp1, Fp2, affine=(sA, tA, sB, tB))
        if F_p_wei is None:
            pass
        elif b <= self.POSE_HEADS_MAX:
            o9, trans_pred, rot_pred = ops.pose_heads(F_p_wei, f["regressor_rot"], f["regressor_trans"], with_rotation=True)
        else:
            with second:
                trans_pred = self._mlp(F_p_wei, f["regressor_trans_padded"])
                if side is not None:
                    trans_pred.record_stream(main)
            o9 = self._mlp(F_p_wei, f["regressor_rot_padded"])
            rot_pred = ops.ortho9d_to_matrix(o9)
            join()
        F_Xo_p = fuse1[:, 256:].reshape(b, self.n_inp, 256).transpose(1, 2)
        prediction = {"trans_pred": trans_pred, "rot_pred": rot_pred, "conf": conf, "F_Xo_p": F_Xo_p}
        if self.mode != "test":
            F_Yc_p = fuse2[:, :256]
            prediction["Xo_pred"] = self._mlp(fuse1[:, 256:], f["regressor_Xo"]).reshape(b, self.n_inp, 3)
            prediction["Yc_pred"] = self._mlp(F_Yc_p, f["regressor_Yc"]).reshape(b, self.n_tmp, 3)
        return prediction


    def _tail_parallel(self, b, launch_by_launch=False):
        if self.PAR_TAIL is not None:
            return bool(self.PAR_TAIL)
        if launch_by_launch and b < 3:
            return False
        blocks = max(b * -(-self.n_inp // 256), b * -(-self.n_tmp // 256))
        if blocks < 256:
            return True
        rounds = -(-blocks // 256)
        return (rounds - blocks / 256.0) / rounds >= 0.1

    def _stage_done(self, name, stream):
        """called behind every stage of the two branches while the whole-forward graph is laid out (name, the stage's stream);
        does nothing -- a measuring tool may replace it on an instance to enqueue a marker there"""

    def forward_graphed(self, data):
        assert not self.training and self.fused
        f = self._fold()
        dev = self.regressor_rot.layers[0].weight.device
        b = int(data["batch_offsets"].size(0)) - 1
        S = int(np.asarray(data["voxel_num_limit"]).astype(np.int64)[0])
        need_ma = {s: int(data[s]["v2p_maps"].shape[1]) - 1 for s in ("inp", "tmp")}
        key = (b, self.n_inp, self.n_tmp, S)
        cache = self.__dict__.setdefault("_graphs", {})
        ent = cache.pop(key, None)
        if ent is None or any(need_ma[s] > ent["ma"][s] for s in ("inp", "tmp")):
            self._drop_graph(ent)
            ent = None
            while len(cache) >= self.MAX_GRAPHS:
                self._drop_graph(cache.pop(next(iter(cache))))
            ent = self._capture(f, dev, b, S, {s: max(32, 2 * need_ma[s]) for s in ("inp", "tmp")})
        cache[key] = ent
        def stageable(t, dtypes):
            return t.is_cuda and t.dim() == 2 and t.stride(1) == 1 and t.dtype in dtypes
        on_dev = all(stageable(data[s]["feats"], (torch.float32,)) and stageable(data[s]["v2p_maps"], (torch.int32,)) and
                     stageable(data[s]["occupied_voxels"], (torch.int32, torch.int64)) for s in ("inp", "tmp"))
        if on_dev:
            jobs = []
            for s in ("inp", "tmp"):
                st, d = ent[s], data[s]
                v0 = d["v0_dev"].view(1, 1) if "v0_dev" in d else int(d["occupied_voxels"].shape[0])
                jobs += [(st["feats"], d["feats"]), (st["occ"], d["occupied_voxels"]), (st["v2p"], d["v2p_maps"]),
                         (st["v0"].view(1, 1) if torch.is_tensor(v0) else st["v0"], v0),
                         (st["pb4"][:, 1:4], d["feats"][:, 4:7])]
            ops.pad_copy_many(jobs)
        else:
            assert "v0_dev" not in data["inp"], "capacity-form crops must be resident, dense CUDA tensors"
            for s, n in (("inp", self.n_inp), ("tmp", self.n_tmp)):
                st, d = ent[s], data[s]
                v0 = int(d["occupied_voxels"].shape[0])
                st["feats"].copy_(d["feats"], non_blocking=True)
                st["pb4"][:, 1:4].copy_(st["feats"][:, 4:7])
                st["occ"][:v0].copy_(d["occupied_voxels"], non_blocking=True)
                st["v2p"].zero_()
                st["v2p"][:v0, :need_ma[s] + 1].copy_(d["v2p_maps"], non_blocking=True)
                st["v0"].fill_(v0)
        if ent.pop("fresh", False) and ent["graph"] is not None and self.GRAPH_TRIES > 0 and not self.single_stream:
            ent = cache[key] = self._select_capture(ent, f, dev, b, S)
        if ent["graph"] is None:
            with torch.no_grad():
                ent["out"] = ent["body"]()
        else:
            ent["graph"].replay()
        o = ent["out"]
        F = o["F_Xo_p"].transpose(1, 2)
        res = {"trans_pred": torch.empty_like(o["trans_pred"]), "rot_pred": torch.empty_like(o["rot_pred"]),
               "conf": torch.empty_like(o["conf"]), "F": torch.empty((b, self.n_inp, 256), dtype=torch.float32, device=dev),
               "pts_tmp": torch.empty((b, self.n_tmp, 3), dtype=torch.float32, device=dev),
               "pts_inp": torch.empty((b, self.n_inp, 3), dtype=torch.float32, device=dev)}
        ops.pad_copy_many([(res["trans_pred"], o["trans_pred"]), (res["rot_pred"], o["rot_pred"].reshape(b, 9)),
                           (res["conf"], o["conf"]), (res["F"], F.reshape(b * self.n_inp, 256)),
                           (res["pts_tmp"].view(b * self.n_tmp, 3), ent["tmp"]["feats"][:, 4:7]),
                           (res["pts_inp"].view(b * self.n_inp, 3), ent["inp"]["feats"][:, 4:7])])
        out = {"trans_pred": res["trans_pred"], "rot_pred": res["rot_pred"], "conf": res["conf"],
               "F_Xo_p": res["F"].transpose(1, 2)}
        for k in o:
            if k not in out:
                out[k] = o[k].clone()
        if self.mode != "test":
            out["sym_flag"] = data["flags"].to(dev)
        data["labels"]["points_tmp"] = res["pts_tmp"]
        data["labels"]["points_inp"] = res["pts_inp"]
        if "vi_info" in data["inp"]:
            out["crop_overflow"] = data["inp"]["vi_info"][2:3]
        return out

    def _select_capture(self, ent, f, dev, b, S):
        import time

        def timed(e):
            for _ in range(3):
                e["graph"].replay()
            torch.cuda.synchronize(dev)
            t0 = time.perf_counter()
            for _ in range(6):
                e["graph"].replay()
            torch.cuda.synchronize(dev)
            return (time.perf_counter() - t0) / 6

        def capture(one_stream, src):
            keep, keep_pf = self.single_stream, self._pair_features
            self._pair_features = self.pair_features
            self.single_stream = bool(one_stream) or keep
            try:
                cand = self._capture(f, dev, b, S, ma)
            finally:
                self.single_stream, self._pair_features = keep, keep_pf
            cand.pop("fresh", None)
            for sd in ("inp", "tmp"):
                for k in ("feats", "occ", "v2p", "v0", "pb4"):
                    cand[sd][k].copy_(src[sd][k])
            return cand
        ma = dict(ent["ma"])
        best, t_best = ent, timed(ent)
        seen = [("two branches", t_best)]
        ref = capture(True, best)
        t_ref = timed(ref)
        seen.append(("one stream", t_ref))
        tries = 1
        while t_best > 1.03 * t_ref and tries < self.GRAPH_TRIES:
            if tries % 2 == 1 and len(_QUEUE_SHIMS) < 16:
                _QUEUE_SHIMS.append(torch.cuda.Stream(dev))
            cand = capture(False, best)
# ... 188 lines not shown
```

### dcl-net_amd/ops.py

```python
import ctypes as C
import threading

import weakref

import torch

from . import _native as N

_c_int = C.c_int
_c_float = C.c_float

PROFILE_EVENTS = None


def _i32_ptr_or_null(t):
    return N.ptr(t) if t is not None else N.vp(0)


def voxelize_idx(coords, batch_size, mode=4):
    if coords.is_cuda:
        raise RuntimeError("voxelize_idx is a host (DataLoader-side) op: pass a CPU tensor")
    assert coords.is_contiguous() and coords.dtype == torch.int64 and coords.dim() == 2
    n, ncol = coords.shape
    input_map = torch.zeros(n, dtype=torch.int32)
# ... 462 lines not shown
        n = points_b4.shape[0]
        ve = (C.c_float * 4)(*[float(v) for v in voxel_extents])
        N.check(N.lib().dcl_point_neighbours_cap(n, N.ptr(points_b4), self.batch, self.S, self.V0, N.ptr(self.ws), ve,
                                                 _c_float(offset), N.ptr(dist2), N.ptr(idx), N.stream()),
                "point_neighbours_cap")

    def point_interpolate(self, dist2, idx, out):
        n = idx.shape[1]
        N.check(N.lib().dcl_point_interpolate(n, self.caps, self.chan, self.level_ptrs, N.ptr(dist2), N.ptr(idx),
                                              N.ptr(out), out.stride(0), N.stream()), "point_interpolate")
        return out


def three_nn_sp(unknown, known, known_seg=None):
    N.need_cuda(unknown, known)
    assert unknown.is_contiguous() and known.is_contiguous()
    assert unknown.shape[1] == 4 and known.shape[1] == 4
    n, m = unknown.shape[0], known.shape[0]
    dist2 = torch.empty((n, 3), dtype=torch.float32, device=unknown.device)
    idx = torch.empty((n, 3), dtype=torch.int32, device=unknown.device)
    nb = 0 if known_seg is None else known_seg.numel() - 1
    N.check(N.lib().dcl_three_nn_sp(n, m, N.ptr(unknown), N.ptr(known), N.ptr(dist2), N.ptr(idx),
                                    _i32_ptr_or_null(known_seg), nb, N.stream()), "three_nn_sp")
    return dist2, idx


def three_interpolate_sp(features, idx, weight, out=None, from_dist2=False):
    N.need_cuda(features, idx, weight)
    assert features.is_contiguous() and idx.is_contiguous() and weight.is_contiguous()
    m, c = features.shape
    n = idx.shape[0]
    if out is None:
        out = torch.empty((n, c), dtype=torch.float32, device=features.device)
    assert out.shape == (n, c) and out.stride(1) == 1
    fn = N.lib().dcl_three_interpolate_dist2_sp if from_dist2 else N.lib().dcl_three_interpolate_sp
    N.check(fn(c, m, n, N.ptr(features), N.ptr(idx), N.ptr(weight), N.ptr(out), out.stride(0) if n > 1 else c,
               N.stream()), "three_interpolate_sp")
    return out


def voxel_centres(aset_or_indices, ve, off, n=None):
    ind = aset_or_indices
    n = ind.shape[0] if n is None else n
    out = torch.empty((max(n, 1), 4), dtype=torch.float32, device=ind.device)
    N.check(N.lib().dcl_voxel_centres(N.ptr(ind), N.vp(0), int(n), _c_float(ve), _c_float(off), N.ptr(out), N.stream()),
            "voxel_centres")
    return out[:n]


def ball_query(radius, nsample, xyz, new_xyz):
    N.need_cuda(xyz, new_xyz)
    assert xyz.is_contiguous() and new_xyz.is_contiguous()
    B, n, _ = xyz.shape
    m = new_xyz.shape[1]
    idx = torch.empty((B, m, nsample), dtype=torch.int32, device=xyz.device)
    N.check(N.lib().dcl_ball_query(B, n, m, _c_float(radius), int(nsample), N.ptr(new_xyz), N.ptr(xyz), N.ptr(idx),
                                   N.stream()), "ball_query")
    return idx


def group_points(features, idx, out=None):
    N.need_cuda(features, idx, out)
    assert features.is_contiguous() and idx.is_contiguous() and idx.dtype == torch.int32
    B, c, n = features.shape
    _, npoint, ns = idx.shape
    if out is None:
        out = torch.empty((B, c, npoint, ns), dtype=torch.float32, device=features.device)
    assert out.shape == (B, c, npoint, ns) and out.stride(3) == 1 and out.stride(2) == ns and out.stride(1) == npoint * ns
    oc = out.stride(0) // (npoint * ns) if B > 1 else c
    assert B == 1 or out.stride(0) == oc * npoint * ns
    N.check(N.lib().dcl_group_points_into(B, c, n, npoint, ns, N.ptr(features), N.ptr(idx), N.ptr(out), int(oc),
                                          N.stream()), "group_points")
    return out


def gather_points(features, idx):
    N.need_cuda(features, idx)
    assert features.is_contiguous() and idx.is_contiguous() and idx.dtype == torch.int32
    B, c, n = features.shape
    m = idx.shape[1]
    out = torch.empty((B, c, m), dtype=torch.float32, device=features.device)
    N.check(N.lib().dcl_gather_points(B, c, n, m, N.ptr(features), N.ptr(idx), N.ptr(out), N.stream()), "gather_points")
    return out


def furthest_point_sampling(xyz, npoint):
    N.need_cuda(xyz)
    assert xyz.is_contiguous()
    B, n, _ = xyz.shape
    temp = torch.full((B, n), 1e10, dtype=torch.float32, device=xyz.device)
    idx = torch.empty((B, npoint), dtype=torch.int32, device=xyz.device)
    N.check(N.lib().dcl_furthest_point_sampling(B, n, int(npoint), N.ptr(xyz), N.ptr(temp), N.ptr(idx), N.stream()),
            "furthest_point_sampling")
    return idx


def knn(k, unknown, known):
    N.need_cuda(unknown, known)
    assert unknown.is_contiguous() and known.is_contiguous()
    B, n, _ = unknown.shape
    m = known.shape[1]
    if k <= 3:
        d2, idx = three_nn(unknown, known)
        return d2[:, :, :k].contiguous(), idx[:, :, :k].contiguous()
    dist2 = torch.empty((B, n, k), dtype=torch.float32, device=unknown.device)
    idx = torch.empty((B, n, k), dtype=torch.int32, device=unknown.device)
    N.check(N.lib().dcl_knn(B, n, m, int(k), N.ptr(unknown), N.ptr(known), N.ptr(dist2), N.ptr(idx), N.stream()), "knn")
    return dist2, idx


def three_nn(unknown, known):
    N.need_cuda(unknown, known)
    assert unknown.is_contiguous() and known.is_contiguous()
    B, n, _ = unknown.shape
    m = known.shape[1]
    dist2 = torch.empty((B, n, 3), dtype=torch.float32, device=unknown.device)
    idx = torch.empty((B, n, 3), dtype=torch.int32, device=unknown.device)
    N.check(N.lib().dcl_three_nn(B, n, m, N.ptr(unknown), N.ptr(known), N.ptr(dist2), N.ptr(idx), N.stream()),
            "three_nn")
    return dist2, idx


def three_interpolate(features, idx, weight):
    N.need_cuda(features, idx, weight)
    assert features.is_contiguous() and idx.is_contiguous() and weight.is_contiguous()
    B, c, m = features.shape
    n = idx.shape[1]
    out = torch.empty((B, c, n), dtype=torch.float32, device=features.device)
    N.check(N.lib().dcl_three_interpolate(B, c, m, n, N.ptr(features), N.ptr(idx), N.ptr(weight), N.ptr(out),
                                          N.stream()), "three_interpolate")
    return out


def _ld(t):
    assert t.dim() == 2 and t.stride(1) == 1
    return t.stride(0) if t.shape[0] > 1 else t.shape[1]


ATTENTION_SPLIT = True


def attention_planes(b, nq, nk, concurrent=1, device=None):
    if not ATTENTION_SPLIT:
        return None, False
    lib = N.lib()
    lib.dcl_cross_attention_planes_bytes.restype = C.c_int64
    pb = int(lib.dcl_cross_attention_planes_bytes(int(b), int(nq), int(nk), int(concurrent)))
    if not pb:
        return None, False
    whole = int(lib.dcl_cross_attention_split_crops(int(b), int(nq), int(nk), int(concurrent))) == int(b)
    return torch.empty(pb, dtype=torch.uint8, device=device if device is not None else torch.device("cuda")), whole


def cross_attention(b, Q, K, V1, O1, V2=None, O2=None, concurrent=1, planes=None):
    N.need_cuda(Q, K, V1, O1, V2, O2)
    nq, nk = Q.shape[0] // b, K.shape[0] // b
    assert Q.shape[1] == 64 and K.shape[1] == 64 and O1.shape[0] == Q.shape[0]
    assert V1 is not None or planes is not None, "V1 = None: its pieces are expected in `planes` (attention_planes, linear_split_vpieces)"
    assert V1 is None or V1.shape[0] == K.shape[0]
    dv1 = 256 if V1 is None else V1.shape[1]
    dv2 = 0 if V2 is None else V2.shape[1]
    ev = None
    if PROFILE_EVENTS is not None:
        ev = (torch.cuda.Event(enable_timing=True), torch.cuda.Event(enable_timing=True))
        ev[0].record()
    scratch = None
    if dv1 == 256 and dv2 == 64:
        need = C.c_int64(0)
        N.check(N.lib().dcl_cross_attention_scratch_floats(b, nq, C.byref(need)), "cross_attention_scratch_floats")
        if need.value:
            scratch = torch.empty(need.value, dtype=torch.float32, device=Q.device)
    if planes is None and dv1 == 256 and dv2 == 64:
        planes, _ = attention_planes(b, nq, nk, concurrent, Q.device)
    N.check(N.lib().dcl_cross_attention_ws3(b, nq, nk, N.ptr(Q), _ld(Q), N.ptr(K), _ld(K), N.ptr(V1), dv1, 256 if V1 is None else _ld(V1),
                                            N.ptr(O1), _ld(O1), N.ptr(V2), dv2, 0 if V2 is None else _ld(V2), N.ptr(O2),
                                            0 if O2 is None else _ld(O2), N.ptr(scratch),
                                            C.c_int64(0 if scratch is None else scratch.numel()), int(concurrent), N.ptr(planes),
                                            C.c_int64(0 if planes is None else planes.numel()), N.stream()),
            "cross_attention")
    if ev is not None:
        ev[1].record()
        PROFILE_EVENTS.append(("cross_attention", ev[0], ev[1]))
    return O1, O2


def conf_pool(b, logit1, logit2, F1, F2, affine=None, finish=True):
    N.need_cuda(logit1, logit2, F1, F2)
    n1, n2 = F1.shape[0] // b, F2.shape[0] // b
    c = F1.shape[1]
    assert logit1.is_contiguous() and logit2.is_contiguous() and logit1.numel() == b * n1 and logit2.numel() == b * n2
    dev = F1.device
    nslices = max(1, min(64, 2048 // max(1, b * ((c + 255) // 256))))
    conf = torch.empty((b, n1 + n2), dtype=torch.float32, device=dev)
    w = torch.empty((b, n1 + n2), dtype=torch.float32, device=dev)
    part1 = torch.empty((b, nslices, c), dtype=torch.float32, device=dev)
    part2 = torch.empty((b, nslices, c), dtype=torch.float32, device=dev)
    ws = torch.empty((b, 2), dtype=torch.float32, device=dev)
    N.check(N.lib().dcl_conf_pool(b, c, n1, n2, N.ptr(logit1), N.ptr(logit2), N.ptr(F1), _ld(F1), N.ptr(F2), _ld(F2),
                                  N.ptr(conf), N.ptr(w), nslices, N.ptr(part1), N.ptr(part2), N.ptr(ws), N.stream()),
            "conf_pool")
    if affine is not None:
        s1, t1, s2, t2 = affine
        N.need_cuda(s1, t1, s2, t2)
        assert all(t.is_contiguous() and t.numel() == c and t.dtype == torch.float32 for t in affine)
        if not finish:
            return conf, (nslices, part1, part2, ws)
        out = torch.empty((b, c), dtype=torch.float32, device=dev)
        N.check(N.lib().dcl_pool_finish(b, c, nslices, N.ptr(part1), N.ptr(part2), N.ptr(ws), N.ptr(s1), N.ptr(t1),
                                        N.ptr(s2), N.ptr(t2), N.ptr(out), N.stream()), "pool_finish")
        return conf, out
    return conf, part1.sum(dim=1), part2.sum(dim=1), ws


def affine3_relu(xyz, W3, term):
    N.need_cuda(xyz, W3, term)
    assert xyz.is_contiguous() and W3.is_contiguous() and term.is_contiguous() and xyz.shape[1] == 3
    rows, c = term.shape
    assert tuple(W3.shape) == (3, c) and xyz.shape[0] == rows
    out = torch.empty_like(term)
    N.check(N.lib().dcl_affine3_relu(C.c_int64(rows), int(c), N.ptr(xyz), N.ptr(W3), N.ptr(term), N.ptr(out), N.stream()),
            "affine3_relu")
    return out


def pose_heads(pooled, rot_layers, trans_layers, with_rotation=False):
    N.need_cuda(pooled)
    pooled = pooled.contiguous()
    b, dev = pooled.shape[0], pooled.device
    assert pooled.shape[1] == 1024 and tuple(rot_layers[0][0].shape) == (1024, 512) and tuple(rot_layers[2][0].shape) == (128, 9)
    assert tuple(trans_layers[1][0].shape) == (512, 128) and tuple(trans_layers[2][0].shape) == (128, 3)
    flat = lambda layers: _ptr_array([t for pair in layers for t in pair])
    assert all(t.is_contiguous() and t.dtype == torch.float32 for layers in (rot_layers, trans_layers) for p in layers for t in p)
    h1 = torch.empty((2, b, 512), dtype=torch.float32, device=dev)
    o9 = torch.empty((b, 9), dtype=torch.float32, device=dev)
    trans = torch.empty((b, 3), dtype=torch.float32, device=dev)
    R = torch.empty((b, 3, 3), dtype=torch.float32, device=dev) if with_rotation else None
    N.check(N.lib().dcl_pose_heads(b, N.ptr(pooled), flat(rot_layers), flat(trans_layers), N.ptr(h1), N.ptr(o9), N.ptr(trans),
                                   N.ptr(R), N.stream()), "pose_heads")
    return (o9, trans, R) if with_rotation else (o9, trans)


def pose_heads_parts(parts, affine, rot_layers, trans_layers, with_rotation=False):
    nslices, part1, part2, ws = parts
    s1, t1, s2, t2 = affine
    b, dev = part1.shape[0], part1.device
    assert part1.shape[2] == 1024 and tuple(rot_layers[0][0].shape) == (1024, 512) and tuple(rot_layers[2][0].shape) == (128, 9)
    assert tuple(trans_layers[1][0].shape) == (512, 128) and tuple(trans_layers[2][0].shape) == (128, 3)
    flat = lambda layers: _ptr_array([t for pair in layers for t in pair])
    assert all(t.is_contiguous() and t.dtype == torch.float32 for layers in (rot_layers, trans_layers) for p in layers for t in p)
    h1 = torch.empty((2, b, 512), dtype=torch.float32, device=dev)
    o9 = torch.empty((b, 9), dtype=torch.float32, device=dev)
    trans = torch.empty((b, 3), dtype=torch.float32, device=dev)
    R = torch.empty((b, 3, 3), dtype=torch.float32, device=dev) if with_rotation else None
    N.check(N.lib().dcl_pose_heads_parts(b, int(nslices), N.ptr(part1), N.ptr(part2), N.ptr(ws), N.ptr(s1), N.ptr(t1), N.ptr(s2),
                                         N.ptr(t2), flat(rot_layers), flat(trans_layers), N.ptr(h1), N.ptr(o9), N.ptr(trans),
                                         N.ptr(R), N.stream()), "pose_heads_parts")
    return (o9, trans, R) if with_rotation else (o9, trans)


VENDOR_GEMM = False


def linear(x, Wt, bias=None, relu=False, out=None):
    if not VENDOR_GEMM and x.is_cuda and Wt.is_cuda and x.dim() == 2 and Wt.dim() == 2:
        sw = prepared_linear(Wt, x)
        if sw is not None:
            return linear_split(x, sw, bias, relu, out)
        if linear_dma_ok(x, Wt):
            return linear_dma(x, Wt, bias, relu, out)
    return linear_lt(x, Wt, bias, relu, out)


def linear_lt(x, Wt, bias=None, relu=False, out=None):
    N.need_cuda(x, Wt)
    assert x.dim() == 2 and Wt.dim() == 2 and x.shape[1] == Wt.shape[0] and x.dtype == Wt.dtype == torch.float32
    M, K = x.shape
    n = Wt.shape[1]
    if out is None:
        out = torch.empty((M, n), dtype=torch.float32, device=x.device)
    assert out.shape == (M, n) and out.dtype == torch.float32 and out.is_cuda
    for t in (x, Wt, out):
        assert t.stride(1) == 1 or t.shape[1] == 1, "rows must be dense"
    if bias is not None:
        assert bias.is_cuda and bias.dtype == torch.float32 and bias.numel() == n and bias.is_contiguous()
    pitch = lambda t: int(t.stride(0)) if t.shape[0] > 1 else max(int(t.stride(0)), int(t.shape[1]))
    N.check(N.lib().dcl_linear_fwd(N.ptr(x), C.c_int64(pitch(x)), N.ptr(Wt), C.c_int64(pitch(Wt)), N.ptr(bias), N.ptr(out),
                                   C.c_int64(pitch(out)), int(M), int(n), int(K), int(bool(relu)), None,
                                   C.c_int64(0), N.stream()), "linear_fwd")
    return out


def linear_dma_ok(x, Wt):
    K, n = Wt.shape
    pw = int(Wt.stride(0)) if K > 1 else n
    px = int(x.stride(0)) if x.shape[0] > 1 else K
    return (K >= 32 and K % 32 == 0 and px % 4 == 0 and pw % 4 == 0 and x.data_ptr() % 16 == 0 and Wt.data_ptr() % 16 == 0 and
            pw >= (n + 3) // 4 * 4)


def linear_dma(x, Wt, bias=None, relu=False, out=None):
    N.need_cuda(x, Wt)
    assert x.dim() == 2 and Wt.dim() == 2 and x.shape[1] == Wt.shape[0] and x.dtype == Wt.dtype == torch.float32
    M, K = x.shape
    n = Wt.shape[1]
    if out is None:
        out = torch.empty((M, n), dtype=torch.float32, device=x.device)
    assert out.shape == (M, n) and out.dtype == torch.float32 and out.is_cuda
    for t in (x, Wt, out):
        assert t.stride(1) == 1 or t.shape[1] == 1, "rows must be dense"
    if bias is not None:
        assert bias.is_cuda and bias.dtype == torch.float32 and bias.numel() == n and bias.is_contiguous()
    pitch = lambda t: int(t.stride(0)) if t.shape[0] > 1 else max(int(t.stride(0)), int(t.shape[1]))
    N.check(N.lib().dcl_linear_dma_fwd(N.ptr(x), C.c_int64(pitch(x)), N.ptr(Wt), C.c_int64(pitch(Wt)), N.ptr(bias), N.ptr(out),
                                       C.c_int64(pitch(out)), int(M), int(n), int(K), int(bool(relu)), N.stream()), "linear_dma_fwd")
    return out


GEMM_SPLIT = True
SPLIT_MIN_TILES = 192
_PREPARED = {}


def prepare_linear(Wt):
    K, n = Wt.shape
    if not Wt.is_cuda or n <= 64 or K % 16 or K < 16:
        return None
    ent = _PREPARED.get(id(Wt))
    if ent is not None and ent[0]() is Wt:
        return ent[1]
    sw = SplitWeight(Wt)
    sw.Wt = None
    key = id(Wt)
    _PREPARED[key] = (weakref.ref(Wt, lambda _r, key=key: _PREPARED.pop(key, None)), sw)
    return sw


def prepared_linear(Wt, x):
    if not GEMM_SPLIT:
        return None
    ent = _PREPARED.get(id(Wt))
    if ent is None or ent[0]() is not Wt:
        return None
    sw = ent[1]
    M = x.shape[0]
    if ((M + 255) // 256) * ((sw.n + 127) // 128) < SPLIT_MIN_TILES or not linear_split_ok(x, sw.K):
        return None
    return sw


LINEAR_POOL_TILE = 128


def linear_pool(x, Wt, bias, roww, relu=True, part=None, rows_per_crop=None, w_stride=0):
    N.need_cuda(x, Wt, roww)
    sw = prepared_linear(Wt, x)
    if sw is not None:
        return linear_split_pool(x, sw, bias, roww, relu, part, rows_per_crop, w_stride)
    M, K = x.shape
    n = Wt.shape[1]
    if rows_per_crop is None:
        rows_per_crop, w_stride = M, 0
        assert roww.is_contiguous() and roww.numel() == M
    assert roww.dtype == torch.float32 and M % rows_per_crop == 0
    tiles = (M + LINEAR_POOL_TILE - 1) // LINEAR_POOL_TILE
    if part is None:
        part = torch.empty((tiles, n), dtype=torch.float32, device=x.device)
    assert part.shape == (tiles, n) and part.stride(1) == 1
    pitch = lambda t: int(t.stride(0)) if t.shape[0] > 1 else max(int(t.stride(0)), int(t.shape[1]))
    N.check(N.lib().dcl_linear_pool_fwd(N.ptr(x), C.c_int64(pitch(x)), N.ptr(Wt), C.c_int64(pitch(Wt)), N.ptr(bias), N.ptr(roww),
                                        int(rows_per_crop), C.c_int64(int(w_stride)), N.ptr(part), C.c_int64(pitch(part)), int(M),
                                        int(n), int(K), int(bool(relu)), N.stream()), "linear_pool_fwd")
    return part


def linear_rowdot(x, Wt, bias, w3, b3, out=None):
    N.need_cuda(x, Wt, w3, b3)
    sw = prepared_linear(Wt, x)
    if sw is not None:
        return linear_split_rowdot(x, sw, bias, w3, b3, out)
    M, K = x.shape
    n = Wt.shape[1]
    assert n <= 128 and w3.shape == (n, 1) and b3.numel() == 1 and bias.numel() == n
    if out is None:
        out = torch.empty((M, 1), dtype=torch.float32, device=x.device)
    assert out.is_contiguous() and out.numel() == M
    pitch = lambda t: int(t.stride(0)) if t.shape[0] > 1 else max(int(t.stride(0)), int(t.shape[1]))
    N.check(N.lib().dcl_linear_rowdot_fwd(N.ptr(x), C.c_int64(pitch(x)), N.ptr(Wt), C.c_int64(pitch(Wt)), N.ptr(bias), N.ptr(w3),
                                          C.c_int64(int(w3.stride(0))), N.ptr(b3), N.ptr(out), int(M), int(n), int(K), N.stream()),
            "linear_rowdot_fwd")
    return out


class SplitWeight:
    __slots__ = ("Wt", "planes", "K", "n")

    def __init__(self, Wt):
        N.need_cuda(Wt)
        assert Wt.dim() == 2 and Wt.dtype == torch.float32 and (Wt.stride(1) == 1 or Wt.shape[1] == 1)
        self.Wt, (self.K, self.n) = Wt, Wt.shape
        lib = N.lib()
        lib.dcl_linear_split_weight_bytes.restype = C.c_int64
        nbytes = int(lib.dcl_linear_split_weight_bytes(int(self.K), int(self.n)))
        assert nbytes > 0, "split-bf16 GEMM core: K must be a multiple of 16"
        self.planes = torch.empty(nbytes, dtype=torch.uint8, device=Wt.device)
        pw = int(Wt.stride(0)) if self.K > 1 else self.n
        N.check(lib.dcl_linear_split_weight(N.ptr(Wt), C.c_int64(pw), int(self.K), int(self.n), N.ptr(self.planes), N.stream()),
                "linear_split_weight")


def linear_split_ok(x, K):
    px = int(x.stride(0)) if x.shape[0] > 1 else K
    return K >= 16 and K % 16 == 0 and px % 4 == 0 and x.data_ptr() % 16 == 0


def linear_split(x, sw, bias=None, relu=False, out=None):
    N.need_cuda(x)
    assert x.dim() == 2 and x.shape[1] == sw.K and x.dtype == torch.float32 and (x.stride(1) == 1 or x.shape[1] == 1)
    M, K, n = x.shape[0], sw.K, sw.n
    if out is None:
        out = torch.empty((M, n), dtype=torch.float32, device=x.device)
    assert out.shape == (M, n) and out.dtype == torch.float32 and out.is_cuda and (out.stride(1) == 1 or n == 1)
    if bias is not None:
        assert bias.is_cuda and bias.dtype == torch.float32 and bias.numel() == n and bias.is_contiguous()
    pitch = lambda t: int(t.stride(0)) if t.shape[0] > 1 else max(int(t.stride(0)), int(t.shape[1]))
    N.check(N.lib().dcl_linear_split_fwd(N.ptr(x), C.c_int64(pitch(x)), N.ptr(sw.planes), N.ptr(bias), N.ptr(out), C.c_int64(pitch(out)),
                                         int(M), int(n), int(K), int(bool(relu)), N.stream()), "linear_split_fwd")
    return out


def linear_split_pool(x, sw, bias, roww, relu=True, part=None, rows_per_crop=None, w_stride=0):
    N.need_cuda(x, roww)
    M, K, n = x.shape[0], sw.K, sw.n
    assert x.shape[1] == K
    if rows_per_crop is None:
        rows_per_crop, w_stride = M, 0
        assert roww.is_contiguous() and roww.numel() == M
    assert roww.dtype == torch.float32 and M % rows_per_crop == 0
    tiles = (M + LINEAR_POOL_TILE - 1) // LINEAR_POOL_TILE
    if part is None:
        part = torch.empty((tiles, n), dtype=torch.float32, device=x.device)
    assert part.shape == (tiles, n) and part.stride(1) == 1
    pitch = lambda t: int(t.stride(0)) if t.shape[0] > 1 else max(int(t.stride(0)), int(t.shape[1]))
    N.check(N.lib().dcl_linear_split_pool_fwd(N.ptr(x), C.c_int64(pitch(x)), N.ptr(sw.planes), N.ptr(bias), N.ptr(roww), int(rows_per_crop),
                                              C.c_int64(int(w_stride)), N.ptr(part), C.c_int64(pitch(part)), int(M), int(n), int(K),
                                              int(bool(relu)), N.stream()), "linear_split_pool_fwd")
    return part


def linear_split_vpieces(x, sw, bias, vplanes, rows_per_crop, relu=True):
    N.need_cuda(x, vplanes)
    M, K, n = x.shape[0], sw.K, sw.n
    assert x.shape[1] == K and n <= 320 and n % 32 == 0 and rows_per_crop % 256 == 0 and M % rows_per_crop == 0
    pitch = lambda t: int(t.stride(0)) if t.shape[0] > 1 else max(int(t.stride(0)), int(t.shape[1]))
    N.check(N.lib().dcl_linear_split_vpieces_fwd(N.ptr(x), C.c_int64(pitch(x)), N.ptr(sw.planes), N.ptr(bias), N.ptr(vplanes),
                                                 int(rows_per_crop), int(M), int(n), int(K), int(bool(relu)), N.stream()),
            "linear_split_vpieces_fwd")
    return vplanes


def linear_split_rowdot(x, sw, bias, w3, b3, out=None):
    N.need_cuda(x, w3, b3)
    M, K, n = x.shape[0], sw.K, sw.n
    assert x.shape[1] == K and n <= 128 and w3.shape == (n, 1) and b3.numel() == 1 and bias.numel() == n
    if out is None:
        out = torch.empty((M, 1), dtype=torch.float32, device=x.device)
    assert out.is_contiguous() and out.numel() == M
    pitch = lambda t: int(t.stride(0)) if t.shape[0] > 1 else max(int(t.stride(0)), int(t.shape[1]))
    N.check(N.lib().dcl_linear_split_rowdot_fwd(N.ptr(x), C.c_int64(pitch(x)), N.ptr(sw.planes), N.ptr(bias), N.ptr(w3),
                                                C.c_int64(int(w3.stride(0))), N.ptr(b3), N.ptr(out), int(M), int(n), int(K), N.stream()),
            "linear_split_rowdot_fwd")
    return out


def conf_softmax(b, logit1, logit2):
    N.need_cuda(logit1, logit2)
    assert logit1.is_contiguous() and logit2.is_contiguous() and logit1.numel() % b == 0 and logit2.numel() % b == 0
    n1, n2 = logit1.numel() // b, logit2.numel() // b
    dev = logit1.device
    conf = torch.empty((b, n1 + n2), dtype=torch.float32, device=dev)
    w = torch.empty((b, n1 + n2), dtype=torch.float32, device=dev)
    ws = torch.empty((b, 2), dtype=torch.float32, device=dev)
    N.check(N.lib().dcl_conf_softmax(b, n1, n2, N.ptr(logit1), N.ptr(logit2), N.ptr(conf), N.ptr(w), N.ptr(ws), N.stream()),
            "conf_softmax")
    return conf, w, ws


def pool_finish2(part1, part2, ws, affine):
    b, c = ws.shape[0], part1.shape[1]
    s1, t1, s2, t2 = affine
    assert part1.is_contiguous() and part2.is_contiguous() and part1.shape[0] % b == 0 and part2.shape[0] % b == 0
    out = torch.empty((b, c), dtype=torch.float32, device=part1.device)
    N.check(N.lib().dcl_pool_finish2(b, c, part1.shape[0] // b, part2.shape[0] // b, N.ptr(part1), N.ptr(part2), N.ptr(ws),
                                     N.ptr(s1), N.ptr(t1), N.ptr(s2), N.ptr(t2), N.ptr(out), N.stream()), "pool_finish2")
    return out


class _LinearJob(C.Structure):
    _fields_ = [("x", C.c_void_p), ("ldx", C.c_int64), ("Wt", C.c_void_p), ("ldw", C.c_int64), ("bias", C.c_void_p),
                ("y", C.c_void_p), ("ldy", C.c_int64), ("M", C.c_int32), ("N", C.c_int32), ("K", C.c_int32), ("relu", C.c_int32)]

# ... 222 lines not shown
```

### include/dclnet_hip.h

```cpp
#ifndef DCLNET_HIP_H_
#define DCLNET_HIP_H_

#include <stdint.h>

#ifdef __cplusplus
extern "C" {
#endif

#define DCL_EINVAL (-1)
typedef void *dclStream_t;

const char *dcl_last_error(void);
#define DCL_ABI_VERSION 2
int dcl_abi_version(void);

int dcl_voxelize_idx_count(const int64_t *coords_host, int n, int ncol, int batch_size, int mode,
                           int32_t *input_map_host, int32_t *n_active_host, int32_t *max_active_host);
int dcl_voxelize_idx_fill(const int64_t *coords_host, int n, int ncol, const int32_t *input_map_host,
                          int n_active, int max_active, int64_t *output_coords_host,
                          int32_t *output_map_host);
int dcl_voxelize_idx_fill_mode(const int64_t *coords_host, int n, int ncol, const int32_t *input_map_host,
                               int n_active, int max_active, int mode, int64_t *output_coords_host,
                               int32_t *output_map_host);

// ... 25 lines not shown
                        int batch, int S_in, int ksize, int stride, int padding, int32_t *nbr, int cap,
                        dclStream_t stream);

int dcl_rulebook_conv(const int32_t *in_indices, const int32_t *n_in_dev, int n_in_host,
                      const uint32_t *in_mask, const int32_t *in_wprefix, const int32_t *in_perm,
                      int batch, int S_in, int ksize, int stride, int padding,
                      uint32_t *out_mask, int32_t *out_wprefix, int32_t *out_indices,
                      int32_t *n_out_dev, int32_t *nbr, int cap_out, int32_t *scratch,
                      dclStream_t stream);

int dcl_rulebook_subm(const int32_t *indices, const int32_t *n_dev, int n_host,
                      const uint32_t *mask, const int32_t *wprefix, const int32_t *perm,
                      int batch, int S, int ksize, int32_t *nbr, int cap, dclStream_t stream);

int dcl_rulebook_to_pairs(const int32_t *nbr, int cap, const int32_t *n_out_dev, int n_out_host,
                          int kvol, int32_t *indice_pairs, int n_in_cap, int32_t *indice_num,
                          dclStream_t stream);

int dcl_rulebook_from_pairs(const int32_t *indice_pairs, int pair_stride, const int32_t *indice_num_dev, int kvol,
                            int n_in, int n_out, int32_t *nbr, int cap, int32_t *bad_pairs_dev, dclStream_t stream);
int dcl_indice_summary_rf(const int32_t *indice_pairs, int pair_stride, const int32_t *indice_num_dev, int kvol,
                          int n_out, int32_t *rf, dclStream_t stream);

int dcl_sparse_conv_fwd(const float *feat, const int32_t *nbr, int cap, const int32_t *n_out_dev,
                        int n_out_host, const float *W, int cin, int cout, int kvol, int subm,
                        const float *scale, const float *shift, int relu, float *out,
                        dclStream_t stream);

int dcl_sparse_conv_fwd_ws(const float *feat, const int32_t *nbr, int cap, const int32_t *n_out_dev,
                           int n_out_host, const float *W, int cin, int cout, int kvol, int subm,
                           const float *scale, const float *shift, int relu, float *out, float *scratch,
                           int64_t scratch_floats, dclStream_t stream);

int dcl_order_rows_ws_bytes(int cap, int64_t *bytes_host);
int dcl_order_rows(const int32_t *out_indices, const int32_t *n_out_dev, int n_out_host, int cap, const uint32_t *in_mask,
                   int S_in, int subm, void *ws, int64_t ws_bytes, int32_t *order, int32_t *bal, uint32_t *smask,
                   dclStream_t stream);
int dcl_sparse_conv_fwd_ordered(const float *feat, const int32_t *nbr, int cap, const int32_t *n_out_dev, int n_out_host,
                                const float *W, int cin, int cout, int kvol, int subm, const float *scale,
                                const float *shift, int relu, float *out, float *scratch, int64_t scratch_floats,
                                const int32_t *order, const int32_t *bal, const uint32_t *smask, dclStream_t stream);
int dcl_sparse_conv_scratch_floats(int rows_cap, int cout, int64_t *floats_host);

int dcl_sparse_avgpool_fwd(const float *feat, const int32_t *nbr, int cap, const int32_t *n_out_dev,
                           int n_out_host, int c, int kvol, float *out, int32_t *rf,
                           dclStream_t stream);

int dcl_sparse_avgpool_fwd_rf(const float *feat, const int32_t *nbr, int cap, const int32_t *n_out_dev,
                              int n_out_host, int c, int kvol, const int32_t *summaryrf, float *out,
                              dclStream_t stream);

#define DCL_PAD_COPY_MAX_JOBS 12
typedef struct {
  void *dst;
  const void *src;
  int32_t rows_dst, cols_dst, rows_src, cols_src, src_pitch, src_is_i64, fill_value, dst_pitch ;
} DclPadCopyJob;
int dcl_pad_copy_many(const DclPadCopyJob *jobs_host, int njobs, dclStream_t stream);

int dcl_backbone_ws_bytes(int batch, int S, int V0, int64_t *bytes_host);
int dcl_backbone_geometry(const int32_t *occ, int V0, int batch, int S, void *ws, int64_t ws_bytes,
                          int32_t *counts_dev , dclStream_t stream);
int dcl_backbone_geometry_window(const int32_t *occ, int V0, int batch_lo, int batch, int S, void *ws, int64_t ws_bytes,
                                 int32_t *counts_dev, dclStream_t stream);
int dcl_backbone_ws2_bytes(const int32_t *counts_host, const int32_t *channels_host, int64_t *bytes_host);
int dcl_backbone_features(const int32_t *occ, int V0, int batch, int S, void *ws, const int32_t *counts_host,
                          const int32_t *channels_host, const float *vox_feats,
                          const float *const *weights_host, const float *const *scales_host,
                          const float *const *shifts_host, void *ws2, int64_t ws2_bytes,
                          float *const *level_out_host, dclStream_t stream);
int dcl_backbone_caps(int batch, int S, int V0_cap, int32_t *caps_host );
int dcl_backbone_geometry_cap(const int32_t *occ, const int32_t *V0_dev, int V0_cap, int batch, int S, void *ws,
                              int64_t ws_bytes, int32_t *counts_dev, dclStream_t stream);
int dcl_backbone_geometry_cap_vox(const int32_t *occ, const int32_t *V0_dev, int V0_cap, int batch, int S, void *ws,
                                  int64_t ws_bytes, int32_t *counts_dev, const float *feats, const int32_t *rules,
                                  float *vox_out, int rows, int max_active, int planes, int average, dclStream_t stream);
int dcl_backbone_features_cap(const int32_t *occ, int V0_cap, int batch, int S, void *ws, const int32_t *counts_dev,
                              const int32_t *channels_host, const float *vox_feats, const float *const *weights_host,
                              const float *const *scales_host, const float *const *shifts_host, void *ws2,
                              int64_t ws2_bytes, float *const *level_out_host, dclStream_t stream);
int dcl_backbone_features_pair(int batch, int S, const int32_t *channels_host, const int32_t *V0, void *const *ws,
                               const int32_t *const *counts_host, const int32_t *const *counts_dev,
                               const float *const *vox_feats, const float *const *const *weights,
                               const float *const *const *scales, const float *const *const *shifts, void *const *ws2,
                               const int64_t *ws2_bytes, float *const *const *level_out, dclStream_t stream);
int dcl_point_features_cap(int n, const float *points_b4, int batch, int S, int V0_cap, void *ws,
                           const int32_t *counts_dev, const int32_t *channels_host,
                           const float *const *level_feats_host, const float *voxel_extent_host, float offset,
                           float *out, int ld, void *tmp, int64_t tmp_bytes, dclStream_t stream);

int dcl_backbone_level_info(int batch, int S, int V0, int level, int64_t *indices_off_host,
                            int64_t *wprefix_off_host, int32_t *S_level_host);
int dcl_point_features(int n, const float *points_b4, int batch, int S, int V0, void *ws,
                       const int32_t *counts_host, const int32_t *channels_host,
                       const float *const *level_feats_host, const float *voxel_extent_host, float offset,
                       float *out, int ld, void *tmp, int64_t tmp_bytes, dclStream_t stream);
int dcl_point_neighbours(int n, const float *points_b4, int batch, int S, int V0, void *ws, const int32_t *counts_host,
                         const float *voxel_extent_host, float offset, float *dist2, int32_t *idx, dclStream_t stream);
int dcl_point_neighbours_cap(int n, const float *points_b4, int batch, int S, int V0_cap, void *ws,
                             const float *voxel_extent_host, float offset, float *dist2, int32_t *idx,
                             dclStream_t stream);
int dcl_point_interpolate(int n, const int32_t *counts_host, const int32_t *channels_host,
                          const float *const *level_feats_host, const float *dist2, const int32_t *idx, float *out,
                          int ld, dclStream_t stream);

int dcl_three_nn_sp(int n, int m, const float *unknown, const float *known, float *dist2,
                    int32_t *idx, const int32_t *known_seg, int nbatch, dclStream_t stream);

int dcl_three_interpolate_sp(int c, int m, int n, const float *points, const int32_t *idx,
                             const float *weight, float *out, int out_stride, dclStream_t stream);

int dcl_three_interpolate_dist2_sp(int c, int m, int n, const float *points, const int32_t *idx,
                                   const float *dist2, float *out, int out_stride,
                                   dclStream_t stream);

int dcl_voxel_centres(const int32_t *indices, const int32_t *n_dev, int n_host, float ve, float off,
                      float *centres, dclStream_t stream);

int dcl_ball_query(int b, int n, int m, float radius, int nsample, const float *new_xyz,
                   const float *xyz, int32_t *idx, dclStream_t stream);
int dcl_group_points(int b, int c, int n, int npoints, int nsample, const float *points,
                     const int32_t *idx, float *out, dclStream_t stream);
int dcl_group_points_into(int b, int c, int n, int npoints, int nsample, const float *points, const int32_t *idx,
                          float *out, int out_batch_channels, dclStream_t stream);
int dcl_gather_points(int b, int c, int n, int npoints, const float *points, const int32_t *idx,
                      float *out, dclStream_t stream);
int dcl_furthest_point_sampling(int b, int n, int m, const float *dataset, float *temp,
                                int32_t *idxs, dclStream_t stream);
int dcl_knn(int b, int n, int m, int k, const float *unknown, const float *known, float *dist2,
            int32_t *idx, dclStream_t stream);
int dcl_three_nn(int b, int n, int m, const float *unknown, const float *known, float *dist2,
                 int32_t *idx, dclStream_t stream);
int dcl_three_interpolate(int b, int c, int m, int n, const float *points, const int32_t *idx,
                          const float *weight, float *out, dclStream_t stream);

int dcl_cross_attention(int b, int nq, int nk, const float *Q, int ldq, const float *K, int ldk,
                        const float *V1, int dv1, int ldv1, float *O1, int ldo1, const float *V2,
                        int dv2, int ldv2, float *O2, int ldo2, dclStream_t stream);
int dcl_cross_attention_ws(int b, int nq, int nk, const float *Q, int ldq, const float *K, int ldk,
                           const float *V1, int dv1, int ldv1, float *O1, int ldo1,
                           const float *V2, int dv2, int ldv2, float *O2, int ldo2,
                           float *scratch, int64_t scratch_floats, dclStream_t stream);
int dcl_cross_attention_ws2(int b, int nq, int nk, const float *Q, int ldq, const float *K, int ldk,
                            const float *V1, int dv1, int ldv1, float *O1, int ldo1,
                            const float *V2, int dv2, int ldv2, float *O2, int ldo2,
                            float *scratch, int64_t scratch_floats, int concurrent_launches, dclStream_t stream);
int64_t dcl_cross_attention_planes_bytes(int b, int nq, int nk, int concurrent_launches);
int dcl_cross_attention_split_crops(int b, int nq, int nk, int concurrent_launches);
int dcl_cross_attention_ws3(int b, int nq, int nk, const float *Q, int ldq, const float *K, int ldk,
                            const float *V1, int dv1, int ldv1, float *O1, int ldo1, const float *V2, int dv2,
                            int ldv2, float *O2, int ldo2, float *scratch, int64_t scratch_floats,
                            int concurrent_launches, void *planes, int64_t planes_bytes, dclStream_t stream);
int dcl_cross_attention_scratch_floats(int b, int nq, int64_t *floats_host);

int dcl_conf_pool(int b, int c, int n1, int n2, const float *logit1, const float *logit2,
                  const float *F1, int ld1, const float *F2, int ld2, float *conf, float *w_scratch,
                  int nslices, float *part1, float *part2, float *wsum, dclStream_t stream);
int dcl_pool_finish(int b, int c, int nslices, const float *part1, const float *part2, const float *wsum,
                    const float *scale1, const float *shift1, const float *scale2, const float *shift2, float *out,
                    dclStream_t stream);

int dcl_affine3_relu(int64_t rows, int c, const float *xyz, const float *W3, const float *term, float *out,
                     dclStream_t stream);
int dcl_mlp128_to1(const float *x, int64_t ldx, int M, const float *W1t, const float *b1, const float *W2t,
                   const float *b2, const float *w3, int64_t ldw3, const float *b3, float *out, dclStream_t stream);
int dcl_pose_heads(int b, const float *pooled, const float *const *rot_layers, const float *const *trans_layers,
                   float *h1_scratch, float *o9, float *trans, float *R, dclStream_t stream);
int dcl_pose_heads_parts(int b, int nslices, const float *part1, const float *part2, const float *wsum,
                         const float *scale1, const float *shift1, const float *scale2, const float *shift2,
                         const float *const *rot_layers, const float *const *trans_layers, float *h1_scratch, float *o9,
                         float *trans, float *R, dclStream_t stream);

int dcl_linear_fwd(const float *x, int64_t ldx, const float *Wt, int64_t ldw, const float *bias, float *y, int64_t ldy,
                   int M, int N, int K, int relu, void *workspace, int64_t workspace_bytes, dclStream_t stream);

int dcl_linear_dma_fwd(const float *x, int64_t ldx, const float *Wt, int64_t ldw, const float *bias, float *y, int64_t ldy,
                       int M, int N, int K, int relu, dclStream_t stream);
int dcl_linear_pool_fwd(const float *x, int64_t ldx, const float *Wt, int64_t ldw, const float *bias, const float *roww,
                        int rows_per_crop, int64_t w_stride, float *part, int64_t ldp, int M, int N, int K, int relu,
                        dclStream_t stream);
int dcl_linear_rowdot_fwd(const float *x, int64_t ldx, const float *Wt, int64_t ldw, const float *bias, const float *w3,
                          int64_t ldw3, const float *b3, float *out, int M, int N, int K, dclStream_t stream);
int64_t dcl_linear_split_weight_bytes(int K, int N);
int dcl_linear_split_weight(const float *Wt, int64_t ldw, int K, int N, void *planes, dclStream_t stream);
int dcl_linear_split_fwd(const float *x, int64_t ldx, const void *planes, const float *bias, float *y, int64_t ldy, int M, int N,
                         int K, int relu, dclStream_t stream);
int dcl_linear_split_pool_fwd(const float *x, int64_t ldx, const void *planes, const float *bias, const float *roww,
                              int rows_per_crop, int64_t w_stride, float *part, int64_t ldp, int M, int N, int K, int relu,
                              dclStream_t stream);
int dcl_linear_split_vpieces_fwd(const float *x, int64_t ldx, const void *planes, const float *bias, void *vplanes,
                                 int rows_per_crop, int M, int N, int K, int relu, dclStream_t stream);
int dcl_linear_split_rowdot_fwd(const float *x, int64_t ldx, const void *planes, const float *bias, const float *w3, int64_t ldw3,
                                const float *b3, float *out, int M, int N, int K, dclStream_t stream);
int dcl_conf_softmax(int b, int n1, int n2, const float *logit1, const float *logit2, float *conf, float *w, float *wsum,
                     dclStream_t stream);
int dcl_pool_finish2(int b, int c, int nslices1, int nslices2, const float *part1, const float *part2, const float *wsum,
                     const float *scale1, const float *shift1, const float *scale2, const float *shift2, float *out,
                     dclStream_t stream);

#define DCL_LINEAR_MAX_JOBS 8
typedef struct DclLinearJob {
  const float *x; int64_t ldx;
  const float *Wt; int64_t ldw;
  const float *bias;
  float *y; int64_t ldy;
  int M, N, K, relu;
} DclLinearJob;
int dcl_linear_group_fwd(const DclLinearJob *jobs, int njobs, dclStream_t stream);

int dcl_ortho9d_to_matrix(int b, const float *o9, float *R, dclStream_t stream);

int dcl_rulebook_transpose(const int32_t *nbr, int cap_out, const int32_t *n_out_dev, int n_out_host, int kvol,
                           int32_t *inv, int cap_in, dclStream_t stream);
int dcl_sparse_conv_wgrad_splits(int n_out, int32_t *splits_host);
int dcl_sparse_conv_wgrad(const float *feat, const int32_t *nbr, int cap, int n_out, const float *dout, int cin, int cout,
                          int kvol, float *partial, float *dW, dclStream_t stream);
int dcl_sparse_avgpool_bwd(const float *dout, const int32_t *inv, int cap_in, int n_in, const int32_t *rf, int c, int kvol,
                           float *din, dclStream_t stream);
int dcl_three_interpolate_grad_sp(int c, int n, int m, const float *grad_out, const int32_t *idx, const float *weight,
                                  float *grad_points_zeroed, dclStream_t stream);
int dcl_voxelize_bp(const float *d_out, const int32_t *rules, float *d_feats_zeroed, int n_rows, int max_active, int c,
                    int average, dclStream_t stream);

int dcl_crop_points_ws_ints(int n_inst, int cap, int64_t *ints_host);
int dcl_crop_points(const uint16_t *depth, const int32_t *label, const uint8_t *rgb, int H, int W, int rgb_channels,
                    int n_inst, const int32_t *boxes, const int32_t *obj_ids, const float *cam_host,
                    const double *rgb_mean_host, const float *half_extent_host, int min_valid, int always_filter, int cap,
                    float *raw_xyz, float *raw_rgb, float *out_xyz, float *out_rgb, float *centroid,
                    int32_t *counts, int32_t *ws, dclStream_t stream);
int dcl_crop_sample(int n_inst, int npoint, int cap, const float *xyz, const float *rgb, const int64_t *sample_idx,
                    const int32_t *counts, int min_valid, float half_extent0, const float *unit_host, int voxel_limit,
                    float *feats, int64_t *coords, dclStream_t stream);

int dcl_add_s(int b, int P, const float *cld, const int32_t *cls, const float *R_pred, const float *t_pred,
              const float *R_gt, const float *t_gt, float *partial_scratch, float *out, dclStream_t stream);

int dcl_add(int b, int P, const float *cld, const int32_t *cls, const float *R_pred, const float *t_pred,
            const float *R_gt, const float *t_gt, float *partial_scratch, float *out, dclStream_t stream);
int dcl_add_by_symmetry(int b, int P, const float *cld, const int32_t *cls, const int32_t *sym_flag,
                        const float *R_pred, const float *t_pred, const float *R_gt, const float *t_gt,
                        float *partial_scratch, float *out, dclStream_t stream);

int dcl_legacy_permutation_heads(uint32_t *key624, int32_t *pos_io, const int32_t *m, int k, int n, int64_t *out,
                                 int32_t *scratch);

int dcl_profile_conv_begin(void);
int dcl_profile_conv_end(double *ms_total_host, int32_t *calls_host);
int dcl_profile_conv_end_calls(double *ms_total_host, int32_t *calls_host, float *ms_per_call_host, int32_t *what_per_call_host,
                               int32_t cap);

#ifdef DCL_DIAG
void dcl_debug_force_valu_conv(int on);
void dcl_debug_attention_variant(int v);
void dcl_debug_attention_split(int n);
void dcl_debug_attention_xcd_remap(int on);
int dcl_debug_geometry_chain(int mode);
void dcl_debug_order_min_batch(int n);
void dcl_debug_order_min_level(int m);
void dcl_debug_three_nn_grid(int mode);
void dcl_debug_nn_batched_mode(int mode);
void dcl_debug_nn_qpt(int q);
unsigned long long dcl_debug_nn_tests_executed(int reset);
void dcl_debug_conv_split(int n);
void dcl_debug_conv_few_chunks(int n);
void dcl_debug_conv_few_tiles(int on);
void dcl_debug_conv_wlds(int on);
void dcl_debug_linear_tile(int t);
void dcl_debug_linear_xcd_remap(int on);
void dcl_debug_linear_persist(int rounds);
int dcl_debug_linear_candidates(int M, int N, int K, int ncand, float *ms_out, long long *ws_out, int *found_out);
long long dcl_debug_linear_plan_workspace(int M, int N, int K);
void dcl_debug_attention_pair_split(int on);
void dcl_debug_attention_bf16(int on);
void dcl_debug_linear_split_xcd_remap(int on);
void dcl_debug_linear_split_whatif(int bits);
void dcl_debug_attention_whatif(int bits);
void dcl_debug_geometry_small_batch(int n);
int dcl_debug_geometry_small_stamps(unsigned long long *host32);
int dcl_debug_stamp(unsigned long long *slot_dev, dclStream_t stream);
void dcl_debug_conv_few_cap(int rows);
void dcl_debug_conv_few_hint(int rows);
void dcl_debug_conv_slots(int n);
void dcl_debug_conv_order_mode(int mode);
int dcl_debug_order_stamps(unsigned long long *host16);
void dcl_debug_conv_xcd_remap(int on);
void dcl_debug_group_points_cfg(int cc, int xb, int threads, int nontemporal);
void dcl_debug_launch_census_reset(void);
long long dcl_debug_launch_census(char *buf, long long cap);
#endif

#ifdef __cplusplus
}
#endif
#endif
```

Measured before the change: 2096.

## Emit pre-split bf16 Q and K/V2 pieces from 64-wide linear epilogues for attention

Adds a 64-output split-bf16 linear kernel whose epilogue can write the attention's Q operand, or the K and V2 operands, directly as hi/mid/lo bf16 planes in the layout the attention kernel loads. The attention sweep gains a templated path that reads pre-split Q pieces instead of splitting Q in its inner loop. A KV2 flag skips the separate K and V2 split kernels. This removes per-tile Q splitting inside the attention inner loop and separate split passes, at the cost of extra plane buffers and more code paths.

```diff
diff --git a/dcl-net_amd/csrc/dense.hip b/dcl-net_amd/csrc/dense.hip
--- a/dcl-net_amd/csrc/dense.hip
+++ b/dcl-net_amd/csrc/dense.hip
@@ -502,8 +502,8 @@
 __device__ __forceinline__ at_bf16x8 at_bf(at_u32x4 v) { return __builtin_bit_cast(at_bf16x8, v); }
 
 __global__ __launch_bounds__(256) void k_attn_split_v(int nk, int nht, const float *__restrict__ V1, int ldv1, const float *__restrict__ V2,
-                                                      int ldv2, unsigned *__restrict__ planes, long long total, int c_begin) {
-  const int nc = 320 - c_begin;
+                                                      int ldv2, unsigned *__restrict__ planes, long long total, int c_begin, int c_end) {
+  const int nc = c_end - c_begin;
   for (long long i = blockIdx.x * 256ll + threadIdx.x; i < total; i += (long long)gridDim.x * 256) {
     const int hs = (int)(i & 1);
     const long long q = i >> 1;
@@ -552,8 +552,35 @@
   }
 }
 
-__global__ __launch_bounds__(512, 2) void k_cross_attn_split(
-    int nq, int nk, const float *__restrict__ Q, int ldq, const unsigned char *__restrict__ planes,
+constexpr int kAttnQBlockBytes = 4 * 3 * 64 * 16;
+__global__ __launch_bounds__(256) void k_attn_split_q(int nq, int nqb, const float *__restrict__ Q, int ldq, unsigned *__restrict__ qpieces,
+                                                      long long total) {
+  for (long long i = blockIdx.x * 256ll + threadIdx.x; i < total; i += (long long)gridDim.x * 256) {
+    const int lane = (int)(i & 63), st = (int)((i >> 6) & 3);
+    const long long cb = i >> 8;
+    const int crop = (int)(cb / nqb), q = (int)(cb - (long long)crop * nqb) * 32 + (lane & 31);
+    float4 a = make_float4(0.f, 0.f, 0.f, 0.f), b = a;
+    if (q < nq) {
+      const float *row = Q + ((size_t)crop * nq + q) * ldq + 16 * st + 8 * (lane >> 5);
+      a = *reinterpret_cast<const float4 *>(row);
+      b = *reinterpret_cast<const float4 *>(row + 4);
+    }
+    at_u32x4 ph, pm, pl;
+    unsigned a0, a1, a2;
+    at_split2(a.x, a.y, a0, a1, a2); ph[0] = a0; pm[0] = a1; pl[0] = a2;
+    at_split2(a.z, a.w, a0, a1, a2); ph[1] = a0; pm[1] = a1; pl[1] = a2;
+    at_split2(b.x, b.y, a0, a1, a2); ph[2] = a0; pm[2] = a1; pl[2] = a2;
+    at_split2(b.z, b.w, a0, a1, a2); ph[3] = a0; pm[3] = a1; pl[3] = a2;
+    unsigned *dst = qpieces + (size_t)(cb * 4 + st) * (3 * 64 * 4) + lane * 4;
+    *reinterpret_cast<at_u32x4 *>(dst) = ph;
+    *reinterpret_cast<at_u32x4 *>(dst + 64 * 4) = pm;
+    *reinterpret_cast<at_u32x4 *>(dst + 2 * 64 * 4) = pl;
+  }
+}
+
+template <bool QP>
+__device__ __forceinline__ void attn_split_sweep(
+    int nq, int nk, const float *__restrict__ Q, int ldq, const unsigned char *__restrict__ qpieces, const unsigned char *__restrict__ planes,
     const unsigned char *__restrict__ kplanes, float *__restrict__ O1, int ldo1, float *__restrict__ O2, int ldo2,
     float *__restrict__ part, int xcd_remap, int whatif) {
   constexpr int NVT = 10, WAVES = 8;
@@ -576,7 +603,9 @@
   constexpr int QB = WAVES * 32;
   const int q = bx * QB + wave * 32 + r;
   const bool qlive = q < nq;
-  const float *qrow = Q + ((size_t)b * nq + min(q, nq - 1)) * ldq + 8 * h;
+  const float *qrow = QP ? nullptr : Q + ((size_t)b * nq + min(q, nq - 1)) * ldq + 8 * h;
+  const int nqb = (nq + 31) >> 5;
+  const unsigned char *qsrc = QP ? qpieces + ((size_t)b * nqb + min(bx * WAVES + wave, nqb - 1)) * kAttnQBlockBytes + lane * 16 : nullptr;
   const int nht = 2 * ((nk + 31) >> 5);
   const unsigned char *vsrc = planes + (size_t)b * nht * kAttnHalfBytes;
   const unsigned char *ksrc = kplanes + (size_t)b * (nht >> 1) * kAttnKTileBytes;
@@ -621,6 +650,29 @@
 #pragma unroll
     for (int e = 0; e < 16; ++e) S[e] = 0.0f;
     const unsigned char *kfb = kfrag + buf * kAttnKTileBytes;
+    if constexpr (QP) {
+      at_u32x4 qn[3];
+#pragma unroll
+      for (int p = 0; p < 3; ++p) qn[p] = *reinterpret_cast<const at_u32x4 *>(qsrc + p * 1024);
+#pragma unroll
+      for (int st = 0; st < 4; ++st) {
+        const at_u32x4 qh = qn[0], qm = qn[1], ql = qn[2];
+        if (st < 3) {
+#pragma unroll
+          for (int p = 0; p < 3; ++p) qn[p] = *reinterpret_cast<const at_u32x4 *>(qsrc + ((st + 1) * 3 + p) * 1024);
+        }
+        const unsigned char *kf = kfb + (((2 * st + h) ^ ksw) << 4);
+        const at_u32x4 kh = *reinterpret_cast<const at_u32x4 *>(kf);
+        const at_u32x4 km = *reinterpret_cast<const at_u32x4 *>(kf + 32 * 128);
+        const at_u32x4 kl = *reinterpret_cast<const at_u32x4 *>(kf + 2 * 32 * 128);
+        S = __builtin_amdgcn_mfma_f32_32x32x16_bf16(at_bf(kl), at_bf(qh), S, 0, 0, 0);
+        S = __builtin_amdgcn_mfma_f32_32x32x16_bf16(at_bf(kh), at_bf(ql), S, 0, 0, 0);
+        S = __builtin_amdgcn_mfma_f32_32x32x16_bf16(at_bf(km), at_bf(qm), S, 0, 0, 0);
+        S = __builtin_amdgcn_mfma_f32_32x32x16_bf16(at_bf(km), at_bf(qh), S, 0, 0, 0);
+        S = __builtin_amdgcn_mfma_f32_32x32x16_bf16(at_bf(kh), at_bf(qm), S, 0, 0, 0);
+        S = __builtin_amdgcn_mfma_f32_32x32x16_bf16(at_bf(kh), at_bf(qh), S, 0, 0, 0);
+      }
+    } else {
     float4 qn0 = *reinterpret_cast<const float4 *>(qrow), qn1 = *reinterpret_cast<const float4 *>(qrow + 4);
 #pragma unroll
     for (int st = 0; st < 4; ++st) {
@@ -646,6 +698,7 @@
       S = __builtin_amdgcn_mfma_f32_32x32x16_bf16(at_bf(kh), at_bf(qm), S, 0, 0, 0);
       S = __builtin_amdgcn_mfma_f32_32x32x16_bf16(at_bf(kh), at_bf(qh), S, 0, 0, 0);
     }
+    }
     float m_tile = -INFINITY;
     if (kb + 32 > nk) {
 #pragma unroll
@@ -748,6 +801,19 @@
         else *reinterpret_cast<float4 *>(O2 + row * ldo2 + (c - 256)) = v;
       }
   }
+}
+
+__global__ __launch_bounds__(512, 2) void k_cross_attn_split(
+    int nq, int nk, const float *__restrict__ Q, int ldq, const unsigned char *__restrict__ planes,
+    const unsigned char *__restrict__ kplanes, float *__restrict__ O1, int ldo1, float *__restrict__ O2, int ldo2,
+    float *__restrict__ part, int xcd_remap, int whatif) {
+  attn_split_sweep<false>(nq, nk, Q, ldq, nullptr, planes, kplanes, O1, ldo1, O2, ldo2, part, xcd_remap, whatif);
+}
+__global__ __launch_bounds__(512, 2) void k_cross_attn_split_q(
+    int nq, int nk, const unsigned char *__restrict__ qpieces, const unsigned char *__restrict__ planes,
+    const unsigned char *__restrict__ kplanes, float *__restrict__ O1, int ldo1, float *__restrict__ O2, int ldo2,
+    float *__restrict__ part, int xcd_remap, int whatif) {
+  attn_split_sweep<true>(nq, nk, nullptr, 0, qpieces, planes, kplanes, O1, ldo1, O2, ldo2, part, xcd_remap, whatif);
 }
 
 __global__ void k_cross_attn_combine(int rows, int nsplit, const float *__restrict__ part, float *__restrict__ O1, int ldo1,
@@ -1115,7 +1181,8 @@
 
 static int attn_dispatch(int b, int nq, int nk, const float *Q, int ldq, const float *K, int ldk, const float *V1, int dv1, int ldv1,
                          float *O1, int ldo1, const float *V2, int dv2, int ldv2, float *O2, int ldo2, float *scratch,
-                         int64_t scratch_floats, int concurrent_launches, void *planes, int64_t planes_bytes, dclStream_t stream);
+                         int64_t scratch_floats, int concurrent_launches, void *planes, int64_t planes_bytes, void *qpieces, int flags,
+                         dclStream_t stream);
 
 static bool attn_takes_w8(int b, int nq, int nk, int concurrent_launches) {
   const long long blocks8 = (long long)b * dcl_div_up(nq, 256);
@@ -1156,27 +1223,50 @@
                                     const float *V1, int dv1, int ldv1, float *O1, int ldo1, const float *V2, int dv2,
                                     int ldv2, float *O2, int ldo2, float *scratch, int64_t scratch_floats,
                                     int concurrent_launches, void *planes, int64_t planes_bytes, dclStream_t stream) {
+  return dcl_cross_attention_ws4(b, nq, nk, Q, ldq, K, ldk, V1, dv1, ldv1, O1, ldo1, V2, dv2, ldv2, O2, ldo2, scratch, scratch_floats,
+                                 concurrent_launches, planes, planes_bytes, nullptr, 0, stream);
+}
+
+DCL_API int64_t dcl_cross_attention_qpieces_bytes(int b, int nq) {
+  if (b <= 0 || nq <= 0) return 0;
+  return (int64_t)b * dcl_div_up(nq, 32) * kAttnQBlockBytes;
+}
+
+DCL_API int dcl_cross_attention_ws4(int b, int nq, int nk, const float *Q, int ldq, const float *K, int ldk,
+                                    const float *V1, int dv1, int ldv1, float *O1, int ldo1, const float *V2, int dv2,
+                                    int ldv2, float *O2, int ldo2, float *scratch, int64_t scratch_floats,
+                                    int concurrent_launches, void *planes, int64_t planes_bytes, void *qpieces, int flags,
+                                    dclStream_t stream) {
   DCL_CHECK_ARG(concurrent_launches == 1 || concurrent_launches == 2);
+  DCL_CHECK_ARG((flags & ~(DCL_ATTN_Q_PIECES | DCL_ATTN_KV2_PIECES)) == 0 && (qpieces || !(flags & DCL_ATTN_Q_PIECES)));
+  DCL_CHECK_ARG(((uintptr_t)qpieces & 15) == 0);
   const int full = (b > 0 && Q && K && O1) ? attn_pair_full_crops(b, nq, dv1, dv2, concurrent_launches, planes ? nk : 0) : 0;
-  DCL_CHECK_ARG(!(full && !V1));
+  DCL_CHECK_ARG(!(full && (!V1 || flags)));
   if (full) {
     int rc = attn_dispatch(full, nq, nk, Q, ldq, K, ldk, V1, dv1, ldv1, O1, ldo1, V2, dv2, ldv2, O2, ldo2, scratch, scratch_floats,
-                           concurrent_launches, planes, planes_bytes, stream);
+                           concurrent_launches, planes, planes_bytes, qpieces, 0, stream);
     if (rc) return rc;
     const size_t qo = (size_t)full * nq, ko = (size_t)full * nk;
     return attn_dispatch(b - full, nq, nk, Q + qo * ldq, ldq, K + ko * ldk, ldk, V1 + ko * ldv1, dv1, ldv1, O1 + qo * ldo1, ldo1,
                          V2 ? V2 + ko * ldv2 : nullptr, dv2, ldv2, O2 ? O2 + qo * ldo2 : nullptr, ldo2, scratch, scratch_floats,
-                         concurrent_launches, nullptr, 0, stream);
+                         concurrent_launches, nullptr, 0, nullptr, 0, stream);
   }
   return attn_dispatch(b, nq, nk, Q, ldq, K, ldk, V1, dv1, ldv1, O1, ldo1, V2, dv2, ldv2, O2, ldo2, scratch, scratch_floats,
-                       concurrent_launches, planes, planes_bytes, stream);
+                       concurrent_launches, planes, planes_bytes, qpieces, flags, stream);
 }
 
 static int attn_dispatch(int b, int nq, int nk, const float *Q, int ldq, const float *K, int ldk, const float *V1, int dv1, int ldv1,
                          float *O1, int ldo1, const float *V2, int dv2, int ldv2, float *O2, int ldo2, float *scratch,
-                         int64_t scratch_floats, int concurrent_launches, void *planes, int64_t planes_bytes, dclStream_t stream) {
+                         int64_t scratch_floats, int concurrent_launches, void *planes, int64_t planes_bytes, void *qpieces, int flags,
+                         dclStream_t stream) {
   DCL_CHECK_ARG(b >= 0 && nq >= 0 && nk > 0 && dv1 > 0 && dv1 % 32 == 0 && dv2 >= 0 && dv2 % 32 == 0);
   if (b == 0 || nq == 0) return 0;
+  const bool kv2_in_planes = flags & DCL_ATTN_KV2_PIECES;
+  if (kv2_in_planes) {
+    DCL_CHECK_ARG(planes && dv2 == 64 && O2);
+    if (!K) K = reinterpret_cast<const float *>(planes);
+    if (!V2) V2 = reinterpret_cast<const float *>(planes);
+  }
   DCL_CHECK_ARG(Q && K && (V1 || planes) && O1 && (dv2 == 0 || (V2 && O2)) && b <= 65535);
   DCL_CHECK_ARG(ldq >= 64 && ldk >= 64 && ldv1 >= dv1 && ldo1 >= dv1 && (dv2 == 0 || (ldv2 >= dv2 && ldo2 >= dv2)));
   DCL_CHECK_ARG(ldq % 4 == 0 && ldk % 4 == 0 && ldv1 % 4 == 0 && ldo1 % 4 == 0 && ldv2 % 4 == 0 && ldo2 % 4 == 0);
@@ -1215,20 +1305,38 @@
       const int nht = 2 * dcl_div_up(nk, 32);
       const int64_t planes_need = (int64_t)b * (nht / 2) * kAttnTileBytes;
       if (planes && planes_bytes >= planes_need && g_attn_bf16 && (((uintptr_t)planes) & 15) == 0) {
-        const int c_begin = V1 ? 0 : 256;
-        const long long total = (long long)b * nht * (320 - c_begin) * 2;
-        hipLaunchKernelGGL(k_attn_split_v, dim3(dcl_grid_1d(total, 256)), dim3(256), 0, s, nk, nht, V1, ldv1, V2, ldv2,
-                           (unsigned *)planes, total, c_begin);
+        const int c_begin = V1 ? 0 : 256, c_end = kv2_in_planes ? 256 : 320;
+        if (c_end > c_begin) {
+          const long long total = (long long)b * nht * (c_end - c_begin) * 2;
+          hipLaunchKernelGGL(k_attn_split_v, dim3(dcl_grid_1d(total, 256)), dim3(256), 0, s, nk, nht, V1, ldv1, V2, ldv2,
+                             (unsigned *)planes, total, c_begin, c_end);
+        }
         unsigned char *kplanes = (unsigned char *)planes + (size_t)b * nht * kAttnHalfBytes;
-        const long long ktotal = (long long)b * (nht / 2) * 32 * 8;
-        hipLaunchKernelGGL(k_attn_split_k, dim3(dcl_grid_1d(ktotal, 256)), dim3(256), 0, s, nk, nht / 2, K, ldk, (unsigned *)kplanes, ktotal);
+        if (!kv2_in_planes) {
+          const long long ktotal = (long long)b * (nht / 2) * 32 * 8;
+          hipLaunchKernelGGL(k_attn_split_k, dim3(dcl_grid_1d(ktotal, 256)), dim3(256), 0, s, nk, nht / 2, K, ldk, (unsigned *)kplanes,
+                             ktotal);
+        }
         const size_t lds_sp = (size_t)2 * (2 * kAttnHalfBytes + kAttnKTileBytes);
-        (void)hipFuncSetAttribute((const void *)k_cross_attn_split, hipFuncAttributeMaxDynamicSharedMemorySize, (int)lds_sp);
-        hipLaunchKernelGGL(k_cross_attn_split, dim3(dcl_div_up(nq, 256), b, nsplit), dim3(512), lds_sp, s, nq, nk, Q, ldq,
-                           (const unsigned char *)planes, (const unsigned char *)kplanes, O1, ldo1, O2, ldo2, scratch,
-                           (int)g_attn_xcd_remap, (int)g_attn_whatif);
+        if (qpieces) {
+          const int nqb = dcl_div_up(nq, 32);
+          if (!(flags & DCL_ATTN_Q_PIECES)) {
+            const long long qtotal = (long long)b * nqb * 4 * 64;
+            hipLaunchKernelGGL(k_attn_split_q, dim3(dcl_grid_1d(qtotal, 256)), dim3(256), 0, s, nq, nqb, Q, ldq, (unsigned *)qpieces,
+                               qtotal);
+          }
+          (void)hipFuncSetAttribute((const void *)k_cross_attn_split_q, hipFuncAttributeMaxDynamicSharedMemorySize, (int)lds_sp);
+          hipLaunchKernelGGL(k_cross_attn_split_q, dim3(dcl_div_up(nq, 256), b, nsplit), dim3(512), lds_sp, s, nq, nk,
+                             (const unsigned char *)qpieces, (const unsigned char *)planes, (const unsigned char *)kplanes, O1, ldo1,
+                             O2, ldo2, scratch, (int)g_attn_xcd_remap, (int)g_attn_whatif);
+        } else {
+          (void)hipFuncSetAttribute((const void *)k_cross_attn_split, hipFuncAttributeMaxDynamicSharedMemorySize, (int)lds_sp);
+          hipLaunchKernelGGL(k_cross_attn_split, dim3(dcl_div_up(nq, 256), b, nsplit), dim3(512), lds_sp, s, nq, nk, Q, ldq,
+                             (const unsigned char *)planes, (const unsigned char *)kplanes, O1, ldo1, O2, ldo2, scratch,
+                             (int)g_attn_xcd_remap, (int)g_attn_whatif);
+        }
       } else {
-        if (v1_in_planes) {
+        if (v1_in_planes || kv2_in_planes) {
           dcl_set_error("dcl_cross_attention: V1 = NULL (pieces in `planes`) but this call does not take the split-bf16 kernel");
           return DCL_EINVAL;
         }
@@ -1240,7 +1348,7 @@
         hipLaunchKernelGGL(k_cross_attn_combine, dim3(dcl_grid_1d((long long)b * nq * 80, 256)), dim3(256), 0, s, b * nq,
                            nsplit, scratch, O1, ldo1, O2, ldo2);
     } else {
-      if (v1_in_planes) {
+      if (v1_in_planes || kv2_in_planes) {
         dcl_set_error("dcl_cross_attention: V1 = NULL (pieces in `planes`) but this call does not take the split-bf16 kernel");
         return DCL_EINVAL;
       }
diff --git a/dcl-net_amd/csrc/linear_split.hip b/dcl-net_amd/csrc/linear_split.hip
--- a/dcl-net_amd/csrc/linear_split.hip
+++ b/dcl-net_amd/csrc/linear_split.hip
@@ -329,6 +329,210 @@
   }
 }
 
+constexpr int kS64BN = 64;
+constexpr int kS64P = kS64BN * kSpKC * 2;
+constexpr int kS64ST = kSpA + 3 * kS64P;
+constexpr int kS64Pitch = 68;
+constexpr int kAtHalfBytes = 3 * 320 * 32;
+constexpr int kAtKTileBytes = 3 * 32 * 128;
+constexpr int kAtQBlockBytes = 4 * 3 * 64 * 16;
+
+template <int FORM>
+__global__ __launch_bounds__(256, 2) void k_linear_split64(const LinSplitArgs a) {
+  extern __shared__ __attribute__((aligned(16))) unsigned char sp_lds[];
+  const int ntm = (a.M + kSpBM - 1) / kSpBM;
+  const int tid = threadIdx.x, lane = tid & 63, wave = __builtin_amdgcn_readfirstlane(tid >> 6);
+  const int r = lane & 31, h = lane >> 5;
+  const int nchunks = a.K / kSpKC;
+  const unsigned lds0 = sp_lds_addr(sp_lds);
+  const size_t bstep = (size_t)kSpB;
+  const int asw = (r >> 2) & 3;
+  const unsigned char *afrag = sp_lds + (wave * 64 + r) * 64;
+  const unsigned char *bfrag = sp_lds + kSpA + r * 32 + ((h ^ ((r >> 3) & 1)) << 4);
+  const unsigned boff0 = (unsigned)((tid >> 7) * 4096 + (tid & 127) * 16), boff1 = 2u * 4096u + (unsigned)tid * 16u;
+
+  for (int tm = blockIdx.x; tm < ntm; tm += gridDim.x) {
+    const int row0 = tm * kSpBM;
+    unsigned aoff[4];
+#pragma unroll
+    for (int i = 0; i < 4; ++i) {
+      const int row = wave * 64 + i * 16 + (lane >> 2);
+      const int p = (lane & 3) ^ ((row >> 2) & 3);
+      const int srow = min(row0 + row, a.M - 1) - row0;
+      aoff[i] = (unsigned)(((long long)srow * a.ldx + 4 * p) * 4);
+    }
+    const float *abase = a.x + (size_t)row0 * a.ldx;
+    const unsigned char *bbase = a.planes;
+    auto issue = [&](int stage) {
+      const unsigned s0 = lds0 + (unsigned)(stage * kS64ST);
+      sp_glds16(boff0, bbase, s0 + (unsigned)(kSpA + wave * 1024));
+      if (wave < 2) sp_glds16(boff1, bbase, s0 + (unsigned)(kSpA + 4096 + wave * 1024));
+#pragma unroll
+      for (int k = 0; k < 4; ++k) sp_glds16(aoff[k], abase, s0 + (unsigned)((wave * 64 + k * 16) * 64));
+      abase += kSpKC;
+      bbase += bstep;
+    };
+    sp_f32x16 acc[2][2];
+#pragma unroll
+    for (int i = 0; i < 2; ++i)
+#pragma unroll
+      for (int j = 0; j < 2; ++j)
+#pragma unroll
+        for (int e = 0; e < 16; ++e) acc[i][j][e] = 0.0f;
+
+    dcl_lds_barrier();
+    issue(0);
+    asm volatile("s_waitcnt vmcnt(0)" ::: "memory");
+    for (int c = 0; c < nchunks; ++c) {
+      const int st = c & 1;
+      asm volatile("s_waitcnt lgkmcnt(0)" ::: "memory");
+      __builtin_amdgcn_s_barrier();
+      const bool more = c + 1 < nchunks;
+      const unsigned char *sa = afrag + st * kS64ST, *sb = bfrag + st * kS64ST;
+      float4 av[2][2];
+      sp_u32x4 ap[2][3], bp[2][3];
+      auto read_a = [&](int i) {
+#pragma unroll
+        for (int q = 0; q < 2; ++q) av[i][q] = *reinterpret_cast<const float4 *>(sa + i * 32 * 64 + (((2 * h + q) ^ asw) << 4));
+      };
+      auto read_b = [&](int j) {
+#pragma unroll
+        for (int p = 0; p < 3; ++p) bp[j][p] = *reinterpret_cast<const sp_u32x4 *>(sb + p * kS64P + j * 32 * 32);
+      };
+      auto split_a = [&](int i, int part) {
+        unsigned ph, pm, pl;
+        const float4 v = av[i][part >> 1];
+        if (part & 1) sp_split2(v.z, v.w, ph, pm, pl); else sp_split2(v.x, v.y, ph, pm, pl);
+        ap[i][0][part] = ph; ap[i][1][part] = pm; ap[i][2][part] = pl;
+      };
+      read_a(0);
+      read_b(0);
+      read_a(1);
+      read_b(1);
+      if (more) issue(st ^ 1);
+      __builtin_amdgcn_sched_barrier(0);
+#pragma unroll
+      for (int part = 0; part < 4; ++part) split_a(0, part);
+      __builtin_amdgcn_sched_barrier(0);
+#pragma unroll
+      for (int blk = 0; blk < 4; ++blk) {
+        const int i = blk >> 1, j = blk & 1;
+        acc[i][j] = __builtin_amdgcn_mfma_f32_32x32x16_bf16(sp_bf(ap[i][2]), sp_bf(bp[j][0]), acc[i][j], 0, 0, 0);
+        acc[i][j] = __builtin_amdgcn_mfma_f32_32x32x16_bf16(sp_bf(ap[i][0]), sp_bf(bp[j][2]), acc[i][j], 0, 0, 0);
+        acc[i][j] = __builtin_amdgcn_mfma_f32_32x32x16_bf16(sp_bf(ap[i][1]), sp_bf(bp[j][1]), acc[i][j], 0, 0, 0);
+        acc[i][j] = __builtin_amdgcn_mfma_f32_32x32x16_bf16(sp_bf(ap[i][1]), sp_bf(bp[j][0]), acc[i][j], 0, 0, 0);
+        acc[i][j] = __builtin_amdgcn_mfma_f32_32x32x16_bf16(sp_bf(ap[i][0]), sp_bf(bp[j][1]), acc[i][j], 0, 0, 0);
+        acc[i][j] = __builtin_amdgcn_mfma_f32_32x32x16_bf16(sp_bf(ap[i][0]), sp_bf(bp[j][0]), acc[i][j], 0, 0, 0);
+        if (blk < 2) { split_a(1, 2 * blk); split_a(1, 2 * blk + 1); }
+        __builtin_amdgcn_sched_barrier(0);
+      }
+      asm volatile("s_waitcnt vmcnt(0)" ::: "memory");
+    }
+    asm volatile("s_nop 15\n\ts_nop 7" ::: "memory");
+
+    float bias[2];
+#pragma unroll
+    for (int j = 0; j < 2; ++j) {
+      const int co = j * 32 + r;
+      bias[j] = (a.bias && co < a.N) ? a.bias[co] : 0.0f;
+    }
+#pragma unroll
+    for (int i = 0; i < 2; ++i)
+#pragma unroll
+      for (int j = 0; j < 2; ++j)
+#pragma unroll
+        for (int e = 0; e < 16; ++e) {
+          float v = acc[i][j][e] + bias[j];
+          if (a.relu) v = fmaxf(v, 0.0f);
+          acc[i][j][e] = v;
+        }
+    if constexpr (FORM <= 1) {
+#pragma unroll
+      for (int i = 0; i < 2; ++i)
+#pragma unroll
+        for (int j = 0; j < 2; ++j) {
+          const int co = j * 32 + r;
+#pragma unroll
+          for (int e = 0; e < 16; ++e) {
+            const int orow = row0 + wave * 64 + i * 32 + sp_rowmap(e, h);
+            if (orow < a.M && co < a.N) __builtin_nontemporal_store(acc[i][j][e], a.y + (size_t)orow * a.ldy + co);
+          }
+        }
+    }
+    if constexpr (FORM >= 1) {
+      unsigned char *pc = reinterpret_cast<unsigned char *>(a.part);
+      const int crop = row0 / a.rows_per_crop, key0 = row0 - crop * a.rows_per_crop;
+      if constexpr (FORM == 2) {
+#pragma unroll
+        for (int j = 0; j < 2; ++j) {
+          const int c = 256 + j * 32 + r;
+          const int hs = h ^ ((c >> 3) & 1);
+#pragma unroll
+          for (int i = 0; i < 2; ++i)
+#pragma unroll
+            for (int hf = 0; hf < 2; ++hf) {
+              const long long ht = (long long)crop * a.ldp + ((key0 + wave * 64 + i * 32) >> 4) + hf;
+              sp_u32x4 ph, pm, pl;
+#pragma unroll
+              for (int e = 0; e < 4; ++e) {
+                unsigned qh, qm, ql;
+                sp_split2(acc[i][j][8 * hf + 2 * e], acc[i][j][8 * hf + 2 * e + 1], qh, qm, ql);
+                ph[e] = qh; pm[e] = qm; pl[e] = ql;
+              }
+              unsigned char *dst = pc + (size_t)ht * kAtHalfBytes + (size_t)(c * 2 + hs) * 16;
+              *reinterpret_cast<sp_u32x4 *>(dst) = ph;
+              *reinterpret_cast<sp_u32x4 *>(dst + 320 * 32) = pm;
+              *reinterpret_cast<sp_u32x4 *>(dst + 2 * 320 * 32) = pl;
+            }
+        }
+      }
+      float *stg = reinterpret_cast<float *>(sp_lds) + wave * 32 * kS64Pitch;
+#pragma unroll
+      for (int i = 0; i < 2; ++i) {
+        __syncthreads();
+#pragma unroll
+        for (int j = 0; j < 2; ++j)
+#pragma unroll
+          for (int e = 0; e < 16; ++e) stg[sp_rowmap(e, h) * kS64Pitch + j * 32 + r] = acc[i][j][e];
+        __syncthreads();
+        const int blk32 = (key0 + wave * 64 + i * 32) >> 5;
+        auto split8 = [&](const float *src, sp_u32x4 &ph, sp_u32x4 &pm, sp_u32x4 &pl) {
+          const float4 u = *reinterpret_cast<const float4 *>(src), w = *reinterpret_cast<const float4 *>(src + 4);
+          unsigned qh, qm, ql;
+          sp_split2(u.x, u.y, qh, qm, ql); ph[0] = qh; pm[0] = qm; pl[0] = ql;
+          sp_split2(u.z, u.w, qh, qm, ql); ph[1] = qh; pm[1] = qm; pl[1] = ql;
+          sp_split2(w.x, w.y, qh, qm, ql); ph[2] = qh; pm[2] = qm; pl[2] = ql;
+          sp_split2(w.z, w.w, qh, qm, ql); ph[3] = qh; pm[3] = qm; pl[3] = ql;
+        };
+        if constexpr (FORM == 1) {
+          unsigned char *qb = pc + ((size_t)crop * (a.rows_per_crop >> 5) + blk32) * kAtQBlockBytes + lane * 16;
+#pragma unroll
+          for (int s = 0; s < 4; ++s) {
+            sp_u32x4 ph, pm, pl;
+            split8(stg + r * kS64Pitch + 16 * s + 8 * h, ph, pm, pl);
+            *reinterpret_cast<sp_u32x4 *>(qb + (s * 3 + 0) * 1024) = ph;
+            *reinterpret_cast<sp_u32x4 *>(qb + (s * 3 + 1) * 1024) = pm;
+            *reinterpret_cast<sp_u32x4 *>(qb + (s * 3 + 2) * 1024) = pl;
+          }
+        } else {
+          const int crops = a.M / a.rows_per_crop;
+          unsigned char *kt = pc + (size_t)crops * a.ldp * kAtHalfBytes + ((size_t)crop * (a.ldp >> 1) + blk32) * kAtKTileBytes;
+#pragma unroll
+          for (int u = 0; u < 4; ++u) {
+            const int item = lane + 64 * u, key = item >> 3, ps = item & 7, g = ps ^ ((key >> 1) & 7);
+            sp_u32x4 ph, pm, pl;
+            split8(stg + key * kS64Pitch + 8 * g, ph, pm, pl);
+            unsigned char *dst = kt + (size_t)item * 16;
+            *reinterpret_cast<sp_u32x4 *>(dst) = ph;
+            *reinterpret_cast<sp_u32x4 *>(dst + 32 * 128) = pm;
+            *reinterpret_cast<sp_u32x4 *>(dst + 2 * 32 * 128) = pl;
+          }
+        }
+      }
+    }
+  }
+}
+
 DCL_HOOK_INT(g_sp_xcd, 1);
 
 template <int EPI>
@@ -422,3 +626,25 @@
   DCL_LAUNCH_CHECK();
   return 0;
 }
+
+DCL_API int dcl_linear_split64_fwd(const float *x, int64_t ldx, const void *planes, const float *bias, float *y, int64_t ldy, void *pieces,
+                                   int rows_per_crop, int M, int N, int K, int relu, int form, dclStream_t stream) {
+  DCL_CHECK_ARG(M >= 0 && N > 0 && N <= kS64BN && K > 0 && x && planes && ldx >= K && form >= 0 && form <= 2);
+  DCL_CHECK_ARG(form == 2 || (y && ldy >= N));
+  DCL_CHECK_ARG(form == 0 || (N == kS64BN && pieces && (((size_t)pieces) & 15) == 0 && rows_per_crop > 0 &&
+                              rows_per_crop % kSpBM == 0 && M % rows_per_crop == 0));
+  DCL_CHECK_ARG(lin_split_ok(x, ldx, planes, K));
+  if (M == 0) return 0;
+  LinSplitArgs a{x, (const unsigned char *)planes, bias, y, ldx, ldy, M, N, K, relu, nullptr, form ? rows_per_crop : 1, 0, (float *)pieces,
+                 nullptr, (long long)(form == 2 ? rows_per_crop / 16 : 0), 0};
+  const int tiles = (M + kSpBM - 1) / kSpBM;
+  const unsigned grid = (unsigned)(tiles < 2048 ? tiles : 2048);
+  constexpr size_t lds = (size_t)2 * kS64ST;
+  static_assert(4 * 32 * kS64Pitch * sizeof(float) <= lds, "epilogue staging fits the stage ring");
+  hipStream_t s = (hipStream_t)stream;
+  if (form == 0) hipLaunchKernelGGL(k_linear_split64<0>, dim3(grid), dim3(256), lds, s, a);
+  else if (form == 1) hipLaunchKernelGGL(k_linear_split64<1>, dim3(grid), dim3(256), lds, s, a);
+  else hipLaunchKernelGGL(k_linear_split64<2>, dim3(grid), dim3(256), lds, s, a);
+  DCL_LAUNCH_CHECK();
+  return 0;
+}
diff --git a/dcl-net_amd/models/DCL_Net.py b/dcl-net_amd/models/DCL_Net.py
--- a/dcl-net_amd/models/DCL_Net.py
+++ b/dcl-net_amd/models/DCL_Net.py
@@ -182,6 +182,7 @@
                 ops.prepare_linear(W1t)
                 for Wt, _ in second:
                     ops.prepare_linear(Wt)
+                    ops.prepare_linear64(Wt)
             for name in ("regressor_conf", "regressor_conf_bi", "regressor_Xo", "regressor_Yc"):
                 for Wt, _ in f[name][:2]:
                     ops.prepare_linear(Wt)
@@ -373,20 +374,27 @@
     def _disengage_buffers(self, side, rows, dev, fuse=None):
         new = lambda c: torch.empty((rows, c), dtype=torch.float32, device=dev)
         fuse_buf, conf_in = new(512), new(128)
-        planes, fused = None, False
+        planes, fused, qpieces = None, False, None
         if fuse is not None and self.mode == "test":
             b, par = fuse
-            nk = self.n_inp if side == "Xc" else self.n_tmp
-            nq = self.n_tmp if side == "Xc" else self.n_inp
-            if rows == b * nk and nk % 256 == 0:
-                planes, whole = ops.attention_planes(b, nq, nk, par, dev)
+            n_this, n_other = (self.n_inp, self.n_tmp) if side == "Xc" else (self.n_tmp, self.n_inp)
+            if rows == b * n_this and n_this % 256 == 0:
+                planes, whole = ops.attention_planes(b, n_other, n_this, par, dev)
                 fused = planes is not None and whole
+                if ops.attention_split_whole(b, n_this, n_other, par):
+                    qpieces = ops.attention_qpieces(b, n_this, dev)
         v1 = None if fused else new(256)
+        kv2 = None if fused and self._dis64(side) else new(64)
         if side == "Xc":
             return {"fuse1": fuse_buf, "conf_in1": conf_in, "Xcp1": fuse_buf[:, :256], "Xcm1": conf_in[:, :64],
-                    "Xcp2": v1, "Xcm2": new(64), "planes2": planes}
+                    "Xcp2": v1, "Xcm2": kv2, "planes2": planes, "qpieces1": qpieces if self._dis64(side) else None}
         return {"fuse2": fuse_buf, "conf_in2": conf_in, "Yop2": fuse_buf[:, 256:], "Yom2": conf_in[:, 64:],
-                "Yop1": v1, "Yom1": new(64), "planes1": planes}
+                "Yop1": v1, "Yom1": kv2, "planes1": planes, "qpieces2": qpieces if self._dis64(side) else None}
+
+    def _dis64(self, side):
+        f = getattr(self, "_folded", None)
+        return (ops.GEMM_SPLIT and f is not None and
+                all(ops.prepared64(f["dis_" + side][2][j][0]) is not None for j, (_, c) in enumerate(self._DIS_TAGS) if c == 64))
 
     def _disengage(self, f, side, pf_rows, act, rows=slice(None)):
         W1t, t1, second = f["dis_" + side]
@@ -395,17 +403,34 @@
             ops.linear_group([(H[:, 256 * j:256 * (j + 1)], second[j][0], second[j][1], True, act[side + tag][rows])
                               for j, (tag, _) in enumerate(self._DIS_TAGS)])
             return
-        for j, (tag, _) in enumerate(self._DIS_TAGS):
+        d_key, d_query = (2, 1) if side == "Xc" else (1, 2)
+        n_this = self.n_inp if side == "Xc" else self.n_tmp
+        q_tag = "m1" if side == "Xc" else "m2"
+        all_rows = act["conf_in%d" % d_query].shape[0]
+        whole = pf_rows.shape[0] == all_rows
+        for j, (tag, c) in enumerate(self._DIS_TAGS):
             Wt, bias = second[j]
             Hj = H[:, 256 * j:256 * (j + 1)]
             if act[side + tag] is None:
-                sw = ops.prepared_linear(Wt, Hj)
-                planes = act["planes2" if side == "Xc" else "planes1"]
-                all_rows = act[side + ("m2" if side == "Xc" else "m1")].shape[0]
-                if sw is not None and pf_rows.shape[0] == all_rows:
-                    ops.linear_split_vpieces(Hj, sw, bias, planes, self.n_inp if side == "Xc" else self.n_tmp, relu=True)
+                planes = act["planes%d" % d_key]
+                if c == 64:
+                    sw = ops.prepared_linear64(Wt, Hj)
+                    if sw is not None and whole:
+                        ops.linear_split64(Hj, sw, bias, pieces=planes, rows_per_crop=n_this, form=2)
+                        act["kv2_ready%d" % d_key] = True
+                        continue
+                else:
+                    sw = ops.prepared_linear(Wt, Hj)
+                    if sw is not None and whole:
+                        ops.linear_split_vpieces(Hj, sw, bias, planes, n_this, relu=True)
+                        continue
+                act[side + tag] = torch.empty((all_rows, c), dtype=torch.float32, device=H.device)
+            elif tag == q_tag and act.get("qpieces%d" % d_query) is not None and whole:
+                sw = ops.prepared_linear64(Wt, Hj)
+                if sw is not None:
+                    ops.linear_split64(Hj, sw, bias, out=act[side + tag], pieces=act["qpieces%d" % d_query], rows_per_crop=n_this, form=1)
+                    act["q_ready%d" % d_query] = True
                     continue
-                act[side + tag] = torch.empty((all_rows, 256), dtype=torch.float32, device=H.device)
             ops.linear(Hj, Wt, bias, True, out=act[side + tag][rows])
 
     def _dense(self, f, pf_inp, pf_tmp, b, dev):
@@ -435,6 +460,12 @@
             if side is not None:
                 main.wait_stream(side)
         fuse1, conf_in1, fuse2, conf_in2 = act["fuse1"], act["conf_in1"], act["fuse2"], act["conf_in2"]
+
+        def pieces(d):
+            flags = ((ops.ATTN_Q_PIECES if act.get("q_ready%d" % d) else 0) |
+                     (ops.ATTN_KV2_PIECES if act.get("kv2_ready%d" % d) else 0))
+            return dict(planes=act.get("planes%d" % d), qpieces=act.get("qpieces%d" % d), flags=flags,
+                        nk=self.n_inp if d == 2 else self.n_tmp)
         (l1, sA, tA), (l2, sB, tB) = f["neck_fuser"], f["neck_fuser_bi"]
         def conf_and_fuser(conf_in, fuse, conf_layers, fuser_layers):
             F = fuse
@@ -451,12 +482,12 @@
         if fused_pool:
             with second:
                 ops.cross_attention(b, act["Yom2"], act["Xcm2"], act["Xcp2"], fuse2[:, :256], act["Xcm2"], conf_in2[:, :64], concurrent=par,
-                                    planes=act.get("planes2"))
+                                    **pieces(2))
                 logit2 = conf_logits(conf_in2, f["regressor_conf_bi"])
                 if side is not None:
                     logit2.record_stream(main)
             ops.cross_attention(b, act["Xcm1"], act["Yom1"], act["Yop1"], fuse1[:, 256:], act["Yom1"], conf_in1[:, 64:], concurrent=par,
-                                planes=act.get("planes1"))
+                                **pieces(1))
             logit1 = conf_logits(conf_in1, f["regressor_conf"])
             join()
             conf, w, wsum = ops.conf_softmax(b, logit1.reshape(-1), logit2.reshape(-1))
@@ -475,12 +506,12 @@
         else:
             with second:
                 ops.cross_attention(b, act["Yom2"], act["Xcm2"], act["Xcp2"], fuse2[:, :256], act["Xcm2"], conf_in2[:, :64], concurrent=par,
-                                    planes=act.get("planes2"))
+                                    **pieces(2))
                 logit2, Fp2 = conf_and_fuser(conf_in2, fuse2, f["regressor_conf_bi"], l2)
                 if side is not None:
                     logit2.record_stream(main); Fp2.record_stream(main)
             ops.cross_attention(b, act["Xcm1"], act["Yom1"], act["Yop1"], fuse1[:, 256:], act["Yom1"], conf_in1[:, 64:], concurrent=par,
-                                planes=act.get("planes1"))
+                                **pieces(1))
             logit1, Fp1 = conf_and_fuser(conf_in1, fuse1, f["regressor_conf"], l1)
             join()
             if b <= self.POSE_PARTS_MAX:
diff --git a/dcl-net_amd/ops.py b/dcl-net_amd/ops.py
--- a/dcl-net_amd/ops.py
+++ b/dcl-net_amd/ops.py
@@ -638,14 +638,32 @@
     return torch.empty(pb, dtype=torch.uint8, device=device if device is not None else torch.device("cuda")), whole
 
 
-def cross_attention(b, Q, K, V1, O1, V2=None, O2=None, concurrent=1, planes=None):
+ATTN_Q_PIECES, ATTN_KV2_PIECES = 1, 2
+
+
+def attention_split_whole(b, nq, nk, concurrent=1):
+    if not ATTENTION_SPLIT:
+        return False
+    return int(N.lib().dcl_cross_attention_split_crops(int(b), int(nq), int(nk), int(concurrent))) == int(b)
+
+
+def attention_qpieces(b, nq, device=None):
+    lib = N.lib()
+    lib.dcl_cross_attention_qpieces_bytes.restype = C.c_int64
+    nbytes = int(lib.dcl_cross_attention_qpieces_bytes(int(b), int(nq)))
+    return torch.empty(nbytes, dtype=torch.uint8, device=device if device is not None else torch.device("cuda"))
+
+
+def cross_attention(b, Q, K, V1, O1, V2=None, O2=None, concurrent=1, planes=None, qpieces=None, flags=0, nk=None):
     N.need_cuda(Q, K, V1, O1, V2, O2)
-    nq, nk = Q.shape[0] // b, K.shape[0] // b
-    assert Q.shape[1] == 64 and K.shape[1] == 64 and O1.shape[0] == Q.shape[0]
+    kv2 = bool(flags & ATTN_KV2_PIECES)
+    assert not kv2 or (K is None and V2 is None and nk is not None and planes is not None and O2 is not None)
+    nq, nk = Q.shape[0] // b, (nk if kv2 else K.shape[0] // b)
+    assert Q.shape[1] == 64 and (kv2 or K.shape[1] == 64) and O1.shape[0] == Q.shape[0]
     assert V1 is not None or planes is not None, "V1 = None: its pieces are expected in `planes` (attention_planes, linear_split_vpieces)"
-    assert V1 is None or V1.shape[0] == K.shape[0]
+    assert V1 is None or V1.shape[0] == b * nk
     dv1 = 256 if V1 is None else V1.shape[1]
-    dv2 = 0 if V2 is None else V2.shape[1]
+    dv2 = 64 if kv2 else (0 if V2 is None else V2.shape[1])
     ev = None
     if PROFILE_EVENTS is not None:
         ev = (torch.cuda.Event(enable_timing=True), torch.cuda.Event(enable_timing=True))
@@ -658,11 +676,13 @@
             scratch = torch.empty(need.value, dtype=torch.float32, device=Q.device)
     if planes is None and dv1 == 256 and dv2 == 64:
         planes, _ = attention_planes(b, nq, nk, concurrent, Q.device)
-    N.check(N.lib().dcl_cross_attention_ws3(b, nq, nk, N.ptr(Q), _ld(Q), N.ptr(K), _ld(K), N.ptr(V1), dv1, 256 if V1 is None else _ld(V1),
-                                            N.ptr(O1), _ld(O1), N.ptr(V2), dv2, 0 if V2 is None else _ld(V2), N.ptr(O2),
-                                            0 if O2 is None else _ld(O2), N.ptr(scratch),
+    assert qpieces is not None or not (flags & ATTN_Q_PIECES)
+    N.check(N.lib().dcl_cross_attention_ws4(b, nq, nk, N.ptr(Q), _ld(Q), N.ptr(K), 64 if K is None else _ld(K), N.ptr(V1), dv1,
+                                            256 if V1 is None else _ld(V1), N.ptr(O1), _ld(O1), N.ptr(V2), dv2,
+                                            64 if V2 is None else _ld(V2), N.ptr(O2), 0 if O2 is None else _ld(O2), N.ptr(scratch),
                                             C.c_int64(0 if scratch is None else scratch.numel()), int(concurrent), N.ptr(planes),
-                                            C.c_int64(0 if planes is None else planes.numel()), N.stream()),
+                                            C.c_int64(0 if planes is None else planes.numel()), N.ptr(qpieces), int(flags),
+                                            N.stream()),
             "cross_attention")
     if ev is not None:
         ev[1].record()
@@ -832,6 +852,57 @@
     if ((M + 255) // 256) * ((sw.n + 127) // 128) < SPLIT_MIN_TILES or not linear_split_ok(x, sw.K):
         return None
     return sw
+
+
+_PREPARED64 = {}
+
+
+def prepare_linear64(Wt):
+    K, n = Wt.shape
+    if not Wt.is_cuda or n != 64 or K % 16 or K < 16:
+        return None
+    ent = _PREPARED64.get(id(Wt))
+    if ent is not None and ent[0]() is Wt:
+        return ent[1]
+    sw = SplitWeight(Wt)
+    sw.Wt = None
+    key = id(Wt)
+    _PREPARED64[key] = (weakref.ref(Wt, lambda _r, key=key: _PREPARED64.pop(key, None)), sw)
+    return sw
+
+
+def prepared64(Wt):
+    ent = _PREPARED64.get(id(Wt))
+    return ent[1] if ent is not None and ent[0]() is Wt else None
+
+
+def prepared_linear64(Wt, x):
+    if not GEMM_SPLIT:
+        return None
+    ent = _PREPARED64.get(id(Wt))
+    if ent is None or ent[0]() is not Wt or not linear_split_ok(x, ent[1].K):
+        return None
+    return ent[1]
+
+
+def linear_split64(x, sw, bias, relu=True, out=None, pieces=None, rows_per_crop=None, form=0):
+    N.need_cuda(x)
+    M, K, n = x.shape[0], sw.K, sw.n
+    assert x.shape[1] == K and n == 64 and form in (0, 1, 2)
+    if form < 2:
+        if out is None:
+            out = torch.empty((M, n), dtype=torch.float32, device=x.device)
+        assert out.shape == (M, n) and out.dtype == torch.float32 and out.is_cuda and out.stride(1) == 1
+    else:
+        out = None
+    if form:
+        N.need_cuda(pieces)
+        assert rows_per_crop % 256 == 0 and M % rows_per_crop == 0
+    pitch = lambda t: int(t.stride(0)) if t.shape[0] > 1 else max(int(t.stride(0)), int(t.shape[1]))
+    N.check(N.lib().dcl_linear_split64_fwd(N.ptr(x), C.c_int64(pitch(x)), N.ptr(sw.planes), N.ptr(bias), N.ptr(out),
+                                           C.c_int64(pitch(out) if out is not None else 0), N.ptr(pieces), int(rows_per_crop or 0), int(M),
+                                           int(n), int(K), int(bool(relu)), int(form), N.stream()), "linear_split64_fwd")
+    return out
 
 
 LINEAR_POOL_TILE = 128
diff --git a/include/dclnet_hip.h b/include/dclnet_hip.h
--- a/include/dclnet_hip.h
+++ b/include/dclnet_hip.h
@@ -201,6 +201,14 @@
                             int ldv2, float *O2, int ldo2, float *scratch, int64_t scratch_floats,
                             int concurrent_launches, void *planes, int64_t planes_bytes, dclStream_t stream);
 int dcl_cross_attention_scratch_floats(int b, int nq, int64_t *floats_host);
+#define DCL_ATTN_Q_PIECES 1
+#define DCL_ATTN_KV2_PIECES 2
+int64_t dcl_cross_attention_qpieces_bytes(int b, int nq);
+int dcl_cross_attention_ws4(int b, int nq, int nk, const float *Q, int ldq, const float *K, int ldk,
+                            const float *V1, int dv1, int ldv1, float *O1, int ldo1, const float *V2, int dv2,
+                            int ldv2, float *O2, int ldo2, float *scratch, int64_t scratch_floats,
+                            int concurrent_launches, void *planes, int64_t planes_bytes, void *qpieces, int flags,
+                            dclStream_t stream);
 
 int dcl_conf_pool(int b, int c, int n1, int n2, const float *logit1, const float *logit2,
                   const float *F1, int ld1, const float *F2, int ld2, float *conf, float *w_scratch,
@@ -239,6 +247,11 @@
                               dclStream_t stream);
 int dcl_linear_split_vpieces_fwd(const float *x, int64_t ldx, const void *planes, const float *bias, void *vplanes,
                                  int rows_per_crop, int M, int N, int K, int relu, dclStream_t stream);
+#define DCL_SPLIT64_PLAIN 0
+#define DCL_SPLIT64_Q 1
+#define DCL_SPLIT64_KV2 2
+int dcl_linear_split64_fwd(const float *x, int64_t ldx, const void *planes, const float *bias, float *y, int64_t ldy, void *pieces,
+                           int rows_per_crop, int M, int N, int K, int relu, int form, dclStream_t stream);
 int dcl_linear_split_rowdot_fwd(const float *x, int64_t ldx, const void *planes, const float *bias, const float *w3, int64_t ldw3,
                                 const float *b3, float *out, int M, int N, int K, dclStream_t stream);
 int dcl_conf_softmax(int b, int n1, int n2, const float *logit1, const float *logit2, float *conf, float *w, float *wsum,
```

Result: no change. 2108 (median of 6 runs) (+0.6%).
